# kekeliu-whu/Wildcat-SLAM

Hardware: AMD Instinct MI355X
Metric: surfel-extract Mpts/s (higher is better)
Workload: dtype f64; 1 GPU; C2: 1M-pt single scan (G2 patch lattice, 999936 pts -> 31248 surfels) per GPU, voxel-grid + 3-level octree + per-cell 3x3 PCA; input = the reference's 48-byte hilti_ros::Point records, consumed in place; points_per_gpu=999936, surfels_per_gpu=31248, parallelism=sweep-per-gpu x1

## Files before the change

### wildcat-slam_amd/csrc/ctx.h

```cpp
#pragma once
#include <hip/hip_runtime.h>

#include <cstdarg>
#include <cstdio>
#include <cstdlib>
#include <cstring>
#include <string>
#include <vector>

#include "../../include/wildcat_hip.h"
#include "extract_plan.h"

struct wc_window_state;

struct wc_buf {
  void *p = nullptr;
  size_t cap = 0;
  bool pooled = false;
  bool plain = false;
};

#ifdef WC_DEV_KNOBS
#define WC_DBG(P, bit) ((P).dbg & (bit))
#else
#define WC_DBG(P, bit) 0
#endif

struct wc_dev_opts {
  int exact_sums = 0;
  int debug_skip = 0;
  int fx_merge_min = 3;
  int fx_split = -1;
  int fx_acc_form = -1;
  int no_bucket_sort = 0;
  int ex_sync = 0;
  int match_pair_serial = 0;
  int lm_dense = 0;
  int lm_side_stream = 1;
  int lm_one_collective = 0;
  int map_mom_pts = 1;
  int map_lin_groups = 0;
  int map_score_groups = 0;
  int map_cast_groups = 0;
  int map_carve_groups = 0;
  int map_remove_groups = 0;
  int map_cc_groups = 0;
  int map_absorb_groups = 0;
  int lm_dense_radius = 7;
  int lm_radius0 = -1;
};
inline bool wc_log_env(const char *name) { return getenv(name) != nullptr; }

struct wc_ctx {
  int device = 0;
  wc_params P;
  wc_dev_opts dev;
  bool pool_ok = false;
  hipMemPool_t pool = nullptr;
  hipStream_t own_stream = nullptr;
  hipStream_t stream = nullptr;
  hipEvent_t ev0 = nullptr, ev1 = nullptr;
  std::string err;
  wc_buf b_ex_ctrl;
  wc_buf b_keys[2], b_vals[2], b_sorttmp, b_slots, b_slot_ids, b_slot_keys[2], b_slot_idx[2], b_cand, b_cand_meta,
      b_status, b_misc[8], b_route[4], b_fx[10];
  double match_stats[8] = {0, 0, 0, 0, 0, 0, 0, 0};
  wc_buf b_kd[10];
  std::vector<wc_ctx *> batch_subs;
  wc_buf b_batch;
  wc_buf b_match_half;
  hipEvent_t ev_knn[2] = {nullptr, nullptr};
  wc_comm comm{};
  bool have_comm = false;
  void *rccl = nullptr;
  uint32_t *h_status_dev = nullptr;
  uint32_t *h_status = nullptr;
  unsigned long long mail_ticket = 0;
  wc_buf b_stage;
  void *h_stage = nullptr;
  size_t h_stage_cap = 0;
  double *h_mail = nullptr;
  ExSweep ex;
  ExMemory ex_mem;
  wc_window_state *win = nullptr;
  wc_ctx *aux = nullptr;
  hipEvent_t ev_aux = nullptr;
  hipEvent_t ev_pair = nullptr;
  void *pair_worker = nullptr;
  void (*pair_worker_free)(void *) = nullptr;
  void *pair_sync = nullptr;
  bool ex_prof = false;
  int ex_prof_mode = 0;
  hipEvent_t ex_ev[8] = {nullptr, nullptr, nullptr, nullptr, nullptr, nullptr, nullptr, nullptr};
};

struct wc_dev_guard {
  int prev = -1;
  bool switched = false;
  explicit wc_dev_guard(const wc_ctx *ctx) {
    if (ctx && hipGetDevice(&prev) == hipSuccess && prev != ctx->device) switched = hipSetDevice(ctx->device) == hipSuccess;
  }
  ~wc_dev_guard() {
    if (switched) (void)hipSetDevice(prev);
  }
  wc_dev_guard(const wc_dev_guard &) = delete;
  wc_dev_guard &operator=(const wc_dev_guard &) = delete;
};

inline int wc_fail(wc_ctx *ctx, int code, const char *fmt, ...) {
  char buf[512];
  va_list ap;
  va_start(ap, fmt);
  vsnprintf(buf, sizeof(buf), fmt, ap);
  va_end(ap);
  if (ctx) ctx->err = buf;
  return code;
}

#define WC_HIP(ctx, call)                                                                                   \
  do {                                                                                                      \
    hipError_t e_ = (call);                                                                                 \
    if (e_ != hipSuccess)                                                                                   \
      return wc_fail(ctx, WC_ERR_HIP, "%s failed: %s (%s:%d)", #call, hipGetErrorString(e_), __FILE__, __LINE__); \
  } while (0)

inline void wc_buf_release(wc_ctx *ctx, wc_buf &b) {
  if (!b.p) return;
  if (b.pooled && ctx && ctx->stream && hipFreeAsync(b.p, ctx->stream) == hipSuccess) {
  } else {
    if (ctx && ctx->stream) (void)hipStreamSynchronize(ctx->stream);
    (void)hipFree(b.p);
  }
  b.p = nullptr, b.cap = 0, b.pooled = false;
}
inline int wc_ensure(wc_ctx *ctx, wc_buf &b, size_t bytes) {
  if (bytes <= b.cap) return WC_OK;
  wc_buf_release(ctx, b);
  size_t want = bytes < ((size_t)64 << 20) ? 2 * bytes : bytes + bytes / 2;
  if (bytes >= ((size_t)64 << 10) && want < ((size_t)16 << 20)) want = (size_t)16 << 20;
  if (want < 4096) want = 4096;
  static const bool alloc_dbg = wc_log_env("WC_ALLOC_DEBUG");
  if (alloc_dbg) fprintf(stderr, "[alloc] %zu bytes wanted -> %zu\n", bytes, want);
  if (ctx->pool_ok && !b.plain && hipMallocFromPoolAsync(&b.p, want, ctx->pool, ctx->stream) == hipSuccess) {
    b.pooled = true;
  } else {
    (void)hipGetLastError();
    b.p = nullptr;
    WC_HIP(ctx, hipMalloc(&b.p, want));
    b.pooled = false;
  }
  b.cap = want;
  return WC_OK;
}
int wc_rccl_allreduce_on(wc_ctx *ctx, double *d_buf, uint64_t count, hipStream_t st);
#define WC_TRY(expr)            \
  do {                          \
    int rc_ = (expr);           \
    if (rc_ != WC_OK) return rc_; \
  } while (0)
```

### wildcat-slam_amd/csrc/ctx.hip

```cpp
#include "ctx.h"

#include <cmath>
#include <cstring>
#include <mutex>

extern "C" const char *wc_version(void) { return "wildcat_hip 0.1 (gfx950)"; }

extern "C" int wc_device_count(void) {
  int n = 0;
  if (hipGetDeviceCount(&n) != hipSuccess) return 0;
  return n;
}

extern "C" void wc_params_default(wc_params *p) {
  std::memset(p, 0, sizeof(*p));
  p->voxel_size = 0.8f;
  p->max_layer = 2;
  p->min_points = 20;
  p->planer_threshold = 0.01f;
  p->min_plane_likeness = 0.1;
  p->cluster_gap = 0.05;
  p->cluster_min_points = 20;
  p->center_scale = 1.0;
  p->angular_scale = 5.0 * M_PI / 180.0;
  p->surfel_dist_max = 0.1;
  p->knn_k = 10;
  p->time_diff_min = 0.06;
  p->surfel_sigma0 = 0.05 / 6;
  p->cauchy_a = 0.4;
  const double gn = 0.00015198973532354657, an = 0.006308226052016165;
  const double gw = 0.00011673723527962174, aw = 2.664506559330434e-06;
  const double rate = 200, k = 0.01;
  p->w_gyr = 1 / (gn * std::sqrt(rate)) * k;
  p->w_acc = 1 / (an * std::sqrt(rate)) * k;
  p->w_bg = 1 / (gw / std::sqrt(rate)) * k;
  p->w_ba = 1 / (aw / std::sqrt(rate)) * k;
  p->imu_dt = 1 / rate;
  p->max_iterations = 100;
  p->reference_quirks = 1;
  p->exact_sums = 0;
}

static int check_params(wc_ctx *ctx, const wc_params *p) {
  if (p->max_layer < 0 || p->max_layer > 2) return wc_fail(ctx, WC_ERR_ARG, "max_layer must be 0..2");
  if (!(p->voxel_size > 0)) return wc_fail(ctx, WC_ERR_ARG, "voxel_size must be positive");
  if (p->cluster_min_points < 1 || p->min_points < 0) return wc_fail(ctx, WC_ERR_ARG, "bad point thresholds");
  if (p->knn_k < 1 || p->knn_k > 16) return wc_fail(ctx, WC_ERR_ARG, "knn_k must be 1..16");
  return WC_OK;
}

namespace {
struct DevOpt {
  const char *name, *env;
  int wc_dev_opts::*field;
  bool flag_only;
};
const DevOpt kDevOpts[] = {
    {"exact_sums", "WC_EXACT_SUMS", &wc_dev_opts::exact_sums, true},
    {"debug_skip", "WC_DEBUG_SKIP", &wc_dev_opts::debug_skip, false},
    {"fx_merge_min", "WC_FX_MERGE_MIN", &wc_dev_opts::fx_merge_min, false},
    {"fx_split", "WC_FX_SPLIT", &wc_dev_opts::fx_split, false},
    {"fx_acc_form", "WC_FX_ACC_FORM", &wc_dev_opts::fx_acc_form, false},
    {"no_bucket_sort", "WC_NO_BUCKET_SORT", &wc_dev_opts::no_bucket_sort, true},
    {"ex_sync", "WC_EX_SYNC", &wc_dev_opts::ex_sync, true},
    {"match_pair_serial", "WC_MATCH_PAIR_SERIAL", &wc_dev_opts::match_pair_serial, true},
    {"lm_dense", "WC_LM_DENSE", &wc_dev_opts::lm_dense, true},
    {"lm_one_collective", "WC_LM_ONE_COLLECTIVE", &wc_dev_opts::lm_one_collective, true},
    {"lm_side_stream", "WC_LM_SIDE_STREAM", &wc_dev_opts::lm_side_stream, false},
    {"map_mom_pts", "WC_MAP_MOM_PTS", &wc_dev_opts::map_mom_pts, false},
    {"map_lin_groups", "WC_MAP_LIN_GROUPS", &wc_dev_opts::map_lin_groups, false},
    {"map_score_groups", "WC_MAP_SCORE_GROUPS", &wc_dev_opts::map_score_groups, false},
    {"map_carve_groups", "WC_MAP_CARVE_GROUPS", &wc_dev_opts::map_carve_groups, false},
    {"map_cast_groups", "WC_MAP_CAST_GROUPS", &wc_dev_opts::map_cast_groups, false},
    {"map_absorb_groups", "WC_MAP_ABSORB_GROUPS", &wc_dev_opts::map_absorb_groups, false},
    {"map_remove_groups", "WC_MAP_REMOVE_GROUPS", &wc_dev_opts::map_remove_groups, false},
    {"map_cc_groups", "WC_MAP_CC_GROUPS", &wc_dev_opts::map_cc_groups, false},
    {"lm_dense_radius", "WC_LM_DENSE_RADIUS", &wc_dev_opts::lm_dense_radius, false},
    {"lm_radius0", "WC_LM_RADIUS0", &wc_dev_opts::lm_radius0, false},
};
}

namespace {
struct DevPool {
  hipMemPool_t pool = nullptr;
  int refs = 0;
};
std::mutex g_pool_mu;
DevPool g_pools[64];
}
hipMemPool_t wc_pool_acquire(int device) {
  if (device < 0 || device >= 64) return nullptr;
  std::lock_guard<std::mutex> lk(g_pool_mu);
  DevPool &d = g_pools[device];
  if (!d.pool) {
    int supported = 0;
    if (hipDeviceGetAttribute(&supported, hipDeviceAttributeMemoryPoolsSupported, device) != hipSuccess || !supported) {
      (void)hipGetLastError();
      return nullptr;
    }
    hipMemPoolProps props;
    std::memset(&props, 0, sizeof(props));
    props.allocType = hipMemAllocationTypePinned;
    props.handleTypes = hipMemHandleTypeNone;
    props.location.type = hipMemLocationTypeDevice;
    props.location.id = device;
    hipMemPool_t p = nullptr;
    if (hipMemPoolCreate(&p, &props) != hipSuccess || !p) {
      (void)hipGetLastError();
      return nullptr;
    }
    uint64_t keep = ~0ull;
    if (hipMemPoolSetAttribute(p, hipMemPoolAttrReleaseThreshold, &keep) != hipSuccess) (void)hipGetLastError();
    d.pool = p;
  }
  ++d.refs;
  return d.pool;
}
void wc_pool_release(int device, hipMemPool_t pool) {
  if (!pool || device < 0 || device >= 64) return;
  std::lock_guard<std::mutex> lk(g_pool_mu);
  DevPool &d = g_pools[device];
  if (d.pool == pool && --d.refs == 0) {
    (void)hipMemPoolDestroy(d.pool);
    d.pool = nullptr;
  }
}

extern "C" int wc_ctx_create(const wc_params *params, int device, wc_ctx **out) {
  if (!out) return WC_ERR_ARG;
  *out = nullptr;
  int n = 0;
  if (hipGetDeviceCount(&n) != hipSuccess || n <= 0 || device < 0 || device >= n) return WC_ERR_NOGPU;
  wc_ctx *ctx = new wc_ctx;
  ctx->device = device;
  if (params)
    ctx->P = *params;
  else
    wc_params_default(&ctx->P);
  int rc = check_params(ctx, &ctx->P);
  if (rc != WC_OK) {
    delete ctx;
    return rc;
  }
  int prev_dev = -1;
  (void)hipGetDevice(&prev_dev);
  struct Restore {
    int d;
    ~Restore() {
      if (d >= 0) (void)hipSetDevice(d);
    }
  } restore{prev_dev};
  if (hipSetDevice(device) != hipSuccess || hipStreamCreateWithFlags(&ctx->own_stream, hipStreamNonBlocking) != hipSuccess ||
      hipEventCreate(&ctx->ev0) != hipSuccess || hipEventCreate(&ctx->ev1) != hipSuccess ||
      hipHostMalloc((void **)&ctx->h_status, 128 * sizeof(uint32_t)) != hipSuccess ||
      hipHostMalloc((void **)&ctx->h_mail, (64 + 4096) * sizeof(double)) != hipSuccess) {
    delete ctx;
    return WC_ERR_HIP;
  }
  ctx->stream = ctx->own_stream;
  {
    void *dp = nullptr;
    if (hipHostGetDevicePointer(&dp, ctx->h_status, 0) == hipSuccess) ctx->h_status_dev = (uint32_t *)dp;
    for (int q = 0; q < 128; ++q) ctx->h_status[q] = 0;
  }
  for (wc_buf &b : ctx->b_route) b.plain = true;
  ctx->b_status.plain = true;
  ctx->pool = wc_pool_acquire(device);
  ctx->pool_ok = ctx->pool != nullptr;
#ifdef WC_DEV_KNOBS
  for (const DevOpt &o : kDevOpts)
    if (const char *v = getenv(o.env)) ctx->dev.*(o.field) = o.flag_only ? 1 : atoi(v);
#endif
  *out = ctx;
  return WC_OK;
}

extern "C" int wc_ctx_set_dev_option(wc_ctx *ctx, const char *name, int value) {
  if (!ctx || !name) return wc_fail(ctx, WC_ERR_ARG, "%s: null or out-of-range argument", __func__);
  for (const DevOpt &o : kDevOpts)
    if (strcmp(o.name, name) == 0) {
      ctx->dev.*(o.field) = value;
      ex_reset_backoff(ctx->ex_mem);
      if (ctx->aux) ctx->aux->dev = ctx->dev;
      for (wc_ctx *sub : ctx->batch_subs) sub->dev = ctx->dev, ex_reset_backoff(sub->ex_mem);
      return WC_OK;
    }
  return wc_fail(ctx, WC_ERR_ARG, "wc_ctx_set_dev_option: unknown option '%s'", name);
}

void wc_window_free(wc_ctx *ctx);
extern "C" int wc_comm_rccl_destroy(wc_ctx *ctx);

extern "C" void wc_ctx_destroy(wc_ctx *ctx) {
  wc_dev_guard dg_(ctx);
  if (!ctx) return;
  (void)hipSetDevice(ctx->device);
  (void)hipStreamSynchronize(ctx->stream);
  if (ctx->pair_worker && ctx->pair_worker_free) ctx->pair_worker_free(ctx->pair_worker);
  ctx->pair_worker = nullptr;
  if (ctx->aux) {
    wc_ctx_destroy(ctx->aux);
    ctx->aux = nullptr;
  }
  if (ctx->ev_aux) (void)hipEventDestroy(ctx->ev_aux);
  if (ctx->ev_pair) (void)hipEventDestroy(ctx->ev_pair);
  for (hipEvent_t e : ctx->ev_knn)
    if (e) (void)hipEventDestroy(e);
  (void)wc_comm_rccl_destroy(ctx);
  wc_window_free(ctx);
  wc_buf *all[] = {&ctx->b_keys[0],      &ctx->b_keys[1],     &ctx->b_vals[0],     &ctx->b_vals[1],      &ctx->b_sorttmp,
                   &ctx->b_slots,        &ctx->b_slot_ids,    &ctx->b_slot_keys[0], &ctx->b_slot_keys[1], &ctx->b_slot_idx[0],
                   &ctx->b_slot_idx[1],  &ctx->b_cand,        &ctx->b_cand_meta,   &ctx->b_status,
                   &ctx->b_ex_ctrl};
  for (wc_buf *b : all) wc_buf_release(ctx, *b);
// ... 187 lines not shown
```

### wildcat-slam_amd/csrc/extract.hip

```cpp
#include <hip/hip_runtime.h>
#include <type_traits>

#include <chrono>
#include <cstdlib>
#include <cstring>
#include <rocprim/rocprim.hpp>

#include "ctx.h"
#include "dmath.h"

namespace {

constexpr int kMom = 11;
constexpr int kProdStride = 66;
constexpr unsigned kRootsGrid = 256 * 16;
constexpr unsigned kEmitGrid = 256 * 8;
constexpr unsigned kRoots2Grid = 256 * 4;
constexpr int kTile = 2048;

struct ExParams {
  double vs;
  float vs_f;
  int max_layer;
  int min_points;
// ... 1056 lines not shown
    const uint32_t v = idx[a];
    const wc_surfel_id vid = slot_ids[v];
    uint64_t b = a;
    while (b > i && surfel_id_less(vid, slot_ids[idx[b - 1]])) {
      idx[b] = idx[b - 1];
      --b;
    }
    idx[b] = v;
  }
}

struct SlotEmitArgs {
  const uint32_t *counts;
  const uint64_t *bins;
  uint32_t bin_cap;
  const wc_surfel *slots;
  const wc_surfel_id *slot_ids;
  uint32_t *status;
  wc_surfel *out;
  wc_surfel_id *out_ids;
  uint64_t cap;
  uint32_t *next_ctrl;
  uint32_t next_words;
};
__device__ __forceinline__ void slot_emit_body(const SlotEmitArgs &E, const uint32_t bid, const uint32_t nblk) {
  const uint32_t *__restrict__ counts = E.counts;
  const uint64_t *__restrict__ bins = E.bins;
  const uint32_t bin_cap = E.bin_cap;
  const wc_surfel *__restrict__ slots = E.slots;
  const wc_surfel_id *__restrict__ slot_ids = E.slot_ids;
  uint32_t *status = E.status;
  wc_surfel *out = E.out;
  wc_surfel_id *out_ids = E.out_ids;
  const uint64_t cap = E.cap;
  uint32_t *next_ctrl = E.next_ctrl;
  const uint32_t next_words = E.next_words;
  __shared__ uint64_t s_item[4][kSlotBinMax];
  if (next_ctrl) {
    const uint32_t i = bid * 256u + threadIdx.x;
    if (i < next_words) next_ctrl[i] = (i == 8u || i == 9u) ? status[i] : 0u;
  }
  __shared__ uint32_t s_sorted[4][kSlotBinMax];
  __shared__ uint32_t s_red[4];
  const int t = threadIdx.x, w = t >> 6, lane = t & 63;
  const uint32_t b0 = bid * 4u;
  static_assert(kBuckets / 4 <= 4 * 256, "four uint4 loads per thread cover the counts");
  const uint4 *c4 = (const uint4 *)counts;
  uint4 v[4];
#pragma unroll
  for (int k = 0; k < 4; ++k) {
    const uint32_t i = (uint32_t)t + 256u * k;
    v[k] = i < bid ? c4[i] : make_uint4(0u, 0u, 0u, 0u);
  }
  const uint4 own = c4[bid];
  const uint64_t *bin = bins + (size_t)(b0 + w) * bin_cap;
  const uint64_t first = (uint32_t)lane < bin_cap ? bin[lane] : 0ull;
  uint32_t part = 0;
#pragma unroll
  for (int k = 0; k < 4; ++k) part += v[k].x + v[k].y + v[k].z + v[k].w;
  for (int off = 32; off >= 1; off >>= 1) part += __shfl_xor(part, off);
  if (lane == 0) s_red[w] = part;
  __syncthreads();
  uint32_t base = s_red[0] + s_red[1] + s_red[2] + s_red[3];
  const uint32_t c0 = own.x, c1 = own.y, c2 = own.z, c3 = own.w;
  if (bid == nblk - 1 && t == 0) {
    status[0] = base + c0 + c1 + c2 + c3;
    uint32_t *hm = host_mailbox(status);
    if (hm) {
      hm[0] = base + c0 + c1 + c2 + c3;
      uint32_t queued = status[4];
      const uint32_t *fxc = counts + kBuckets;
      for (int j = 0; j < 16; ++j) queued += fxc[(16 + j) * 32];
      hm[4] = queued;
      hm[5] = status[5];
    }
  }
  base += (w > 0 ? c0 : 0u) + (w > 1 ? c1 : 0u) + (w > 2 ? c2 : 0u);
  const uint32_t c = w == 0 ? c0 : (w == 1 ? c1 : (w == 2 ? c2 : c3));
  if (c == 0) return;
  if (c > bin_cap) {
    if (lane == 0) raise_flag(status, kFlagSlotBinOverflow);
    return;
  }
  auto before = [&](uint64_t other, uint64_t mine) -> bool {
    if ((other >> 32) == (mine >> 32) && other != mine) {
      const double to = slots[(uint32_t)other].t, tm = slots[(uint32_t)mine].t;
      return to < tm || (to == tm && surfel_id_less(slot_ids[(uint32_t)other], slot_ids[(uint32_t)mine]));
    }
    return other < mine;
  };
  if (c <= 64u) {
    const uint32_t lo = (uint32_t)first, hi = (uint32_t)(first >> 32);
    uint32_t rank = 0;
    for (uint32_t j = 0; j < c; ++j) {
      const uint64_t other = ((uint64_t)(uint32_t)__builtin_amdgcn_readlane((int)hi, (int)j) << 32) | (uint32_t)__builtin_amdgcn_readlane((int)lo, (int)j);
      if ((uint32_t)lane < c) rank += before(other, first) ? 1u : 0u;
    }
    if ((uint32_t)lane < c) s_sorted[w][rank] = lo;
  } else {
    s_item[w][lane] = first;
    for (uint32_t i = lane + 64; i < c; i += 64) s_item[w][i] = bin[i];
    __builtin_amdgcn_wave_barrier();
    for (uint32_t i = lane; i < c; i += 64) {
      const uint64_t mine = s_item[w][i];
      uint32_t rank = 0;
      for (uint32_t j = 0; j < c; ++j) rank += before(s_item[w][j], mine) ? 1u : 0u;
      s_sorted[w][rank] = (uint32_t)mine;
    }
  }
  __builtin_amdgcn_wave_barrier();
  const int sub = lane / 10, piece = lane - sub * 10;
  if (sub >= 6) return;
  auto load = [&](uint32_t r, bool on) -> double2 {
    double2 d = make_double2(0.0, 0.0);
    if (!on) return d;
    const uint32_t sl = s_sorted[w][r];
    if (piece < 9)
      d = ((const double2 *)(slots + sl))[piece];
    else if (out_ids) {
      const uint4 q = *(const uint4 *)(slot_ids + sl);
      d = *(const double2 *)&q;
    }
    return d;
  };
  auto store = [&](uint32_t r, bool on, const double2 &d) {
    if (!on) return;
    const uint64_t o = (uint64_t)base + r;
    if (piece < 9)
      ((double2 *)(out + o))[piece] = d;
    else if (out_ids)
      *(double2 *)(out_ids + o) = d;
  };
  if (c <= 12u) {
    const uint32_t r = sub;
    const bool on0 = r < c && (uint64_t)base + r < cap, on1 = r + 6 < c && (uint64_t)base + r + 6 < cap;
    const double2 d0 = load(r, on0), d1 = load(r + 6, on1);
    store(r, on0, d0);
    store(r + 6, on1, d1);
    return;
  }
  for (uint32_t r = sub; r < c; r += 24) {
    bool on[4];
    double2 d[4];
#pragma unroll
    for (int q = 0; q < 4; ++q) {
      on[q] = r + 6u * q < c && (uint64_t)base + r + 6u * q < cap;
      d[q] = load(r + 6u * q, on[q]);
    }
#pragma unroll
    for (int q = 0; q < 4; ++q) store(r + 6u * q, on[q], d[q]);
  }
}

__global__ void __launch_bounds__(256) k_slot_emit(const uint32_t *__restrict__ counts, const uint64_t *__restrict__ bins, uint32_t bin_cap,
                                                  const wc_surfel *__restrict__ slots, const wc_surfel_id *__restrict__ slot_ids,
                                                  uint32_t *status, wc_surfel *out, wc_surfel_id *out_ids, uint64_t cap, uint32_t *next_ctrl,
                                                  uint32_t next_words) {
  const SlotEmitArgs E{counts, bins, bin_cap, slots, slot_ids, status, out, out_ids, cap, next_ctrl, next_words};
  slot_emit_body(E, blockIdx.x, gridDim.x);
}
__global__ void __launch_bounds__(256) k_slot_emit_b(const SlotEmitArgs *__restrict__ Es, int K) {
  const uint32_t per = kBuckets / 4;
  const uint32_t k = blockIdx.x / per;
  if ((int)k >= K) return;
  slot_emit_body(Es[k], blockIdx.x - k * per, per);
}


__device__ __forceinline__ uint32_t run_length(const unsigned long long *s_bits, uint32_t i, uint32_t cnt) {
  uint32_t w = (i + 1) >> 6;
  unsigned long long m = (w < kTile / 64) ? (s_bits[w] & (~0ull << ((i + 1) & 63))) : 0ull;
  while (m == 0ull && ++w < kTile / 64) m = s_bits[w];
  const uint32_t nxt = m ? (w * 64 + (uint32_t)__ffsll((long long)m) - 1) : cnt;
  return min(nxt, cnt) - i;
}

struct InitArgs {
  uint32_t *p[8];
  uint32_t nw[8];
  uint32_t val[8];
};
__global__ void __launch_bounds__(256) k_init(InitArgs I) {
  const uint32_t i = blockIdx.x * 256u + threadIdx.x;
#pragma unroll
  for (int r = 0; r < 8; ++r)
    if (i < I.nw[r]) I.p[r][i] = I.val[r];
}

constexpr int kRunThreads = 512;
constexpr uint32_t kNoKey = 0xFFFFFFFFu;
__global__ void __launch_bounds__(kRunThreads) k_pt_runs(wc_points pts, double vs, uint64_t n, uint32_t *counts, uint64_t *bins,
                                                        uint32_t bin_cap, uint32_t *status) {
  __shared__ uint32_t s_key[kTile];
  __shared__ unsigned long long s_bits[kTile / 64];
  __shared__ uint32_t s_runs[kBuckets];
  __shared__ uint32_t s_pts[kBuckets];
  const int t = threadIdx.x;
  const uint64_t t0 = (uint64_t)blockIdx.x * kTile;
  const uint32_t cnt = (uint32_t)min((uint64_t)kTile, n - t0);
  double x0, y0, z0;
  ex_origin(pts, x0, y0, z0);
  const int k0x = vox(x0, vs), k0y = vox(y0, vs), k0z = vox(z0, vs);
  uint32_t key[kTile / kRunThreads];
#pragma unroll
  for (int j = 0; j < kTile / kRunThreads; ++j) {
    const uint32_t i = (uint32_t)j * kRunThreads + t;
    key[j] = 0;
    if (i < cnt) {
      double x, y, z;
      load_xyz(pts, t0 + i, x, y, z);
      key[j] = kNoKey;
      if (finite3(x, y, z)) {
        int rx = vox(x, vs) - k0x + 512, ry = vox(y, vs) - k0y + 512, rz = vox(z, vs) - k0z + 512;
        if ((unsigned)rx >= 1024u || (unsigned)ry >= 1024u || (unsigned)rz >= 1024u) {
          raise_flag(status, kFlagKeyRange);
          rx = min(max(rx, 0), 1023), ry = min(max(ry, 0), 1023), rz = min(max(rz, 0), 1023);
        }
        key[j] = (uint32_t)rx | ((uint32_t)ry << 10) | ((uint32_t)rz << 20);
      }
    }
  }
  for (int b = t; b < kBuckets; b += kRunThreads) {
    s_runs[b] = 0;
    s_pts[b] = 0;
  }
  if (t < kTile / 64) s_bits[t] = 0ull;
#pragma unroll
  for (int j = 0; j < kTile / kRunThreads; ++j) s_key[j * kRunThreads + t] = key[j];
  __syncthreads();
#pragma unroll
  for (int j = 0; j < kTile / kRunThreads; ++j) {
    const uint32_t i = (uint32_t)j * kRunThreads + t;
    const bool headp = i < cnt && (i == 0 || key[j] != s_key[i - 1]);
    const unsigned long long m = __ballot(headp);
    if ((t & 63) == 0) s_bits[i >> 6] = m;
  }
  __syncthreads();
  uint32_t rank[kTile / kRunThreads], len[kTile / kRunThreads];
#pragma unroll
  for (int j = 0; j < kTile / kRunThreads; ++j) {
    const uint32_t i = (uint32_t)j * kRunThreads + t;
    rank[j] = 0xFFFFFFFFu;
    if (i < cnt && key[j] != kNoKey && ((s_bits[i >> 6] >> (i & 63)) & 1ull)) {
      const uint32_t d = key_digit(key[j]);
      len[j] = run_length(s_bits, i, cnt);
      rank[j] = atomicAdd(&s_runs[d], 1u);
      atomicAdd(&s_pts[d], len[j]);
    }
  }
  __syncthreads();
  for (int b = t; b < kBuckets; b += kRunThreads) {
    const uint32_t c = s_runs[b];
    if (c) {
      s_runs[b] = atomicAdd(&counts[b], c);
      atomicAdd(&counts[kBuckets + b], s_pts[b]);
    }
  }
  __syncthreads();
#pragma unroll
  for (int j = 0; j < kTile / kRunThreads; ++j) {
    if (rank[j] == 0xFFFFFFFFu) continue;
    const uint32_t i = (uint32_t)j * kRunThreads + t;
    const uint32_t d = key_digit(key[j]);
    const uint32_t pos = s_runs[d] + rank[j];
    if (pos < bin_cap) bins[(size_t)d * bin_cap + pos] = run_comp(key_rest(key[j]), (uint32_t)(t0 + i), len[j]);
  }
}

__global__ void __launch_bounds__(256) k_pt_bucket(uint64_t *bins, uint32_t bin_cap, uint32_t lds_cap, const uint32_t *__restrict__ counts,
                                                  uint32_t *run_off, HeadRec *head_slots, uint32_t *root_cnt, uint32_t *root_first,
                                                  int min_points, uint32_t *status) {
  extern __shared__ __align__(16) unsigned char s_dyn[];
  __shared__ uint32_t s_red[4], s_live[4];
  const int t = threadIdx.x, w = t >> 6, lane = t & 63;
  uint64_t *s_a = (uint64_t *)s_dyn + (size_t)w * lds_cap;
  uint64_t *s_b = (uint64_t *)s_dyn + (size_t)(4 + w) * lds_cap;
  uint32_t *s_off = (uint32_t *)((uint64_t *)s_dyn + (size_t)8 * lds_cap) + (size_t)w * lds_cap;
  const uint32_t b0 = blockIdx.x * 4u, b = b0 + w;
  const uint32_t *pcounts = counts + kBuckets;
  uint32_t nb = counts[b];
  const uint32_t total = pcounts[b];
  uint64_t *bin = bins + (size_t)b * bin_cap;
  const uint64_t first = ((uint32_t)lane < min(nb, bin_cap)) ? bin[lane] : 0ull;
  uint32_t part = 0, runs_part = 0;
  for (uint32_t i = t; i < b0; i += 256) part += pcounts[i];
  if (blockIdx.x == gridDim.x - 1)
    for (uint32_t i = t; i < kBuckets; i += 256) runs_part += counts[i];
  uint32_t before = 0;
  for (int j = 0; j < w; ++j) before += pcounts[b0 + j];
  for (int off = 32; off >= 1; off >>= 1) part += __shfl_xor(part, off);
  if (lane == 0) s_red[w] = part;
  if (blockIdx.x == gridDim.x - 1) {
    for (int off = 32; off >= 1; off >>= 1) runs_part += __shfl_xor(runs_part, off);
    if (lane == 0) atomicAdd(&status[5], runs_part);
  }
  if (nb > bin_cap || nb > lds_cap) {
    if (lane == 0) raise_flag(status, nb > bin_cap ? kFlagBucketOverflow : kFlagLdsOverflow);
    nb = 0;
  }
  if (nb <= 64) {
    if ((uint32_t)lane < nb) s_a[lane] = first;
    __builtin_amdgcn_wave_barrier();
    if ((uint32_t)lane < nb) {
      uint32_t rank = 0;
      for (uint32_t j = 0; j < nb; ++j) rank += (s_a[j] < first) ? 1u : 0u;
      s_b[rank] = first;
    }
  } else {
    uint32_t N = 128;
    while (N < nb) N <<= 1;
    s_b[lane] = first;
    for (uint32_t i = lane + 64; i < N; i += 64) s_b[i] = (i < nb) ? bin[i] : ~0ull;
    __builtin_amdgcn_wave_barrier();
    for (uint32_t k = 2; k <= N; k <<= 1)
      for (uint32_t j = k >> 1; j > 0; j >>= 1) {
        for (uint32_t p = lane; p < N / 2; p += 64) {
          const uint32_t i = 2 * p - (p & (j - 1)), l = i + j;
          const uint64_t x = s_b[i], y = s_b[l];
// ... 56 lines not shown
    const uint32_t r = s_list[k] & 0xFFFFu, r2 = s_list[k] >> 16;
    const uint32_t seg = (r2 < nb ? s_off[r2] : total) - s_off[r];
    head_slots[first_slot + lbase + k] = HeadRec{pbase + s_off[r], b * bin_cap + r, r2 - r, seg};
  }
}

inline uint32_t pt_bin_cap(uint64_t n) {
  uint32_t cap = 64;
  while (cap < kPtBinMax && (uint64_t)cap * kBuckets < 32 * n) cap *= 2;
  return cap;
}

constexpr uint32_t kCtrlStatus = 0, kCtrlCounts = 64, kCtrlRoots = kCtrlCounts + 2 * kBuckets, kCtrlBins = kCtrlRoots + 2 * (kBuckets / 4),
                   kCtrlFx = kCtrlBins + kBuckets, kCtrlWords = kCtrlFx + 4 * 16 * 32;

int clear_ctrl(wc_ctx *ctx) {
  WC_TRY(wc_ensure(ctx, ctx->b_ex_ctrl, kCtrlWords * 4));
  uint32_t *ctrl = (uint32_t *)ctx->b_ex_ctrl.p;
  InitArgs I{};
  void *dp = nullptr;
  if (hipHostGetDevicePointer(&dp, ctx->h_status, 0) != hipSuccess) dp = nullptr;
  const unsigned long long a = (unsigned long long)dp;
  I.p[0] = ctrl, I.nw[0] = 8, I.val[0] = 0u;
  I.p[1] = ctrl + 10, I.nw[1] = kCtrlRoots - 10, I.val[1] = 0u;
  I.p[2] = ctrl + 8, I.nw[2] = 1, I.val[2] = (uint32_t)a;
  I.p[3] = ctrl + 9, I.nw[3] = 1, I.val[3] = (uint32_t)(a >> 32);
  I.p[4] = ctrl + kCtrlBins, I.nw[4] = kBuckets + 4 * 16 * 32, I.val[4] = 0u;
  k_init<<<(kCtrlRoots + 255) / 256, 256, 0, ctx->stream>>>(I);
  WC_HIP(ctx, hipGetLastError());
  return WC_OK;
}

int point_sort_runs(wc_ctx *ctx, const wc_points &pts, double vs, HeadRec *head_slots, int min_points, uint32_t *status) {
  hipStream_t st = ctx->stream;
  const uint64_t n = pts.n;
  const uint32_t cap = pt_bin_cap(n);
  const uint32_t lds_cap = std::min(cap, std::max(64u, ctx->ex_mem.lds_cap));
  WC_TRY(wc_ensure(ctx, ctx->b_misc[1], (uint64_t)kBuckets * cap * 8));
  WC_TRY(wc_ensure(ctx, ctx->b_misc[3], (uint64_t)kBuckets * cap * 4));
  uint32_t *counts = (uint32_t *)ctx->b_ex_ctrl.p + kCtrlCounts;
  const unsigned tiles = (unsigned)((n + kTile - 1) / kTile);
  const size_t lds = (size_t)4 * lds_cap * 20;
  if (!ctx->ex_mem.bucket_attr_set) {
    WC_HIP(ctx, hipFuncSetAttribute((const void *)k_pt_bucket, hipFuncAttributeMaxDynamicSharedMemorySize, (int)(4 * kPtBinMax * 20)));
    ctx->ex_mem.bucket_attr_set = true;
  }
  k_pt_runs<<<tiles, kRunThreads, 0, st>>>(pts, vs, n, counts, (uint64_t *)ctx->b_misc[1].p, cap, status);
  k_pt_bucket<<<kBuckets / 4, 256, lds, st>>>((uint64_t *)ctx->b_misc[1].p, cap, lds_cap, counts, (uint32_t *)ctx->b_misc[3].p, head_slots,
                                             counts + 2 * kBuckets, counts + 2 * kBuckets + kBuckets / 4, min_points, status);
  WC_HIP(ctx, hipGetLastError());
  return WC_OK;
}

template <typename K>
int sort_pairs(wc_ctx *ctx, K *kin, K *kout, uint32_t *vin, uint32_t *vout, size_t n, unsigned end_bit) {
  using cfg = rocprim::radix_sort_config<rocprim::default_config, rocprim::default_config, rocprim::default_config, 0>;
  size_t tmp = 0;
  WC_HIP(ctx, rocprim::radix_sort_pairs<cfg>(nullptr, tmp, kin, kout, vin, vout, n, 0u, end_bit, ctx->stream));
  WC_TRY(wc_ensure(ctx, ctx->b_sorttmp, tmp));
  tmp = ctx->b_sorttmp.cap;
  WC_HIP(ctx, rocprim::radix_sort_pairs<cfg>(ctx->b_sorttmp.p, tmp, kin, kout, vin, vout, n, 0u, end_bit, ctx->stream));
  return WC_OK;
}

#include "extract_fast.inc"
#include "extract_split.inc"

int fx_ensure_zero(wc_ctx *ctx, wc_buf &b, size_t bytes) {
  if (bytes <= b.cap) return WC_OK;
  WC_TRY(wc_ensure(ctx, b, bytes));
  WC_HIP(ctx, hipMemsetAsync(b.p, 0, b.cap, ctx->stream));
  return WC_OK;
}

bool fx_applicable(const wc_ctx *ctx, uint64_t n, double t_lo, double t_hi) {
  const wc_params &P = ctx->P;
  if (P.exact_sums || ctx->dev.exact_sums) return false;
  if (n < 64 || !(P.voxel_size > 0.0f) || P.voxel_size >= 0.99f) return false;
  if (!(P.cluster_gap > 1e-6) || !(t_hi > t_lo)) return false;
  if ((t_hi - t_lo) / (P.cluster_gap * 0.999) >= 1048000.0) return false;
  return true;
}

ExParams ex_params(const wc_ctx *ctx) {
  const wc_params &P = ctx->P;
  ExParams E{};
  E.vs = (double)P.voxel_size, E.vs_f = P.voxel_size, E.max_layer = P.max_layer, E.min_points = P.min_points;
  E.thr = (double)P.planer_threshold, E.min_like = P.min_plane_likeness;
  for (int i = 0; i < 3; ++i) E.view[i] = P.view_point[i];
  E.gap = P.cluster_gap, E.cluster_min = P.cluster_min_points;
  E.t_lo_bits = ordered_bits_host(ctx->ex.t_lo);
  E.t_span_bits = ordered_bits_host(ctx->ex.t_hi) - E.t_lo_bits;
  E.dbg = ctx->dev.debug_skip;
  E.merge_min = ctx->dev.fx_merge_min;
  return E;
}

void ex_mark(wc_ctx *ctx, int i) {
  if (ctx->ex_prof && (ctx->ex_prof_mode != 2 || i == 1 || i == 5)) (void)hipEventRecord(ctx->ex_ev[i], ctx->stream);
}

template <typename Args>
void ex_keep_for_tail(wc_ctx *ctx, const Args &A, int (*tail)(wc_ctx *, bool)) {
  static_assert(sizeof(Args) <= sizeof(ctx->ex.roots_args), "extract_plan.h: roots_args too small");
  std::memcpy(ctx->ex.roots_args, &A, sizeof(A));
  ctx->ex.tail = tail;
}

int fx_tail(wc_ctx *ctx, bool layer2);

int run_pipeline_fast(wc_ctx *ctx) {
  const wc_params &P = ctx->P;
  ExMemory &M = ctx->ex_mem;
  const wc_points &pts = ctx->ex.pts;
  const double t_lo = ctx->ex.t_lo, t_hi = ctx->ex.t_hi;
  const uint64_t n = pts.n;
  hipStream_t st = ctx->stream;
  FxArgs A;
  std::memset(&A, 0, sizeof(A));
  A.P = ex_params(ctx);
  A.pts = pts;
  A.t_lo = t_lo;
  int e = 0;
  (void)std::frexp(t_hi - t_lo, &e);
  A.tick = std::ldexp(1.0, 40 - e), A.inv_tick = std::ldexp(1.0, e - 40);
  A.inv_w = 1.0 / (P.cluster_gap * 0.999);
  A.inv_span = 1.0 / (t_hi - t_lo);
  A.inv_vs = 1.0 / (double)P.voxel_size;
  A.qs = 4294967296.0, A.inv_q = 1.0 / 4294967296.0, A.inv_qq = std::ldexp(1.0, -44);
  {
    const double vs = (double)P.voxel_size;
    A.band0 = 1e-14 + 3.0 * (std::ldexp(1.0, -45) + 2.0 * std::ldexp(1.0, -33) * vs + 16.0 * std::ldexp(1.0, -53) * (0.5 * vs) * (0.5 * vs));
  }
  uint32_t mr = 1024;
  while ((uint64_t)mr * 8 < n) mr *= 2;
  A.mr_per = mr / kFxSub, A.mq_per = std::max(64u, mr / 2 / kFxSub);
  uint32_t tr = 2048;
  while ((uint64_t)tr * 4 < n) tr *= 2;
  A.tr_mask = tr - 1;
  A.static_map = n <= 2000000ull ? 1u : 0u;
  {
    const uintptr_t px = (uintptr_t)pts.xyz, pt = (uintptr_t)pts.time;
    if (pts.xyz_stride == 48u && pts.time_stride == 48u && pt == px + 24u && px % 16u == 0u)
      A.fmt = 1u;
    else if (pts.xyz_stride == 12u && pts.time_stride == 8u && px % 16u == 0u && pt % 16u == 0u)
      A.fmt = 2u;
  }
  const unsigned tiles = ex_fx_tiles(n);
  A.rec_tiles = tiles;
  const uint64_t spill_full = ((uint64_t)tiles + 7) / 8 * kFxTile;
  A.spill_per = (uint32_t)((n <= 8000000ull || M.fx_spill_full) ? spill_full : std::max<uint64_t>(1024, n / 32));
  A.rec_cap = tiles * (uint32_t)kFxRecTile + 8u * A.spill_per;
  const uint64_t total_slots = ex_total_slots(n, P.max_layer, P.cluster_min_points, (uint64_t)kFxSub * 256);
  const uint32_t bin_cap = ex_slot_bin_cap(total_slots);
  WC_TRY(fx_ensure_zero(ctx, ctx->b_fx[0], (size_t)tr * 4));
  WC_TRY(wc_ensure(ctx, ctx->b_fx[1], (size_t)mr * 4));
  WC_TRY(fx_ensure_zero(ctx, ctx->b_fx[2], (size_t)tr * kFxBlockW * 8));
  WC_TRY(fx_ensure_zero(ctx, ctx->b_fx[3], (size_t)A.mq_per * kFxSub * kFxBlockW * 8));
  WC_TRY(wc_ensure(ctx, ctx->b_fx[4], (size_t)2 * A.rec_cap * kFxRecW * 8));
  const unsigned ngrid = ex_fx_node_grid(n);
  WC_TRY(wc_ensure(ctx, ctx->b_fx[6], (size_t)ngrid * kFxJobCap * kFxJobW * 8));
  ctx->ex.fx_split = ctx->ex.batch_defer || (ctx->dev.fx_split >= 0 ? ctx->dev.fx_split != 0 : !A.static_map);
  if (ctx->ex.fx_split) {
    A.static_map = 0u;
    A.jobpool_per = (uint32_t)std::max<uint64_t>(4096, n / (uint64_t)std::max(1, P.cluster_min_points) / 2);
    WC_TRY(wc_ensure(ctx, ctx->b_fx[7], ((size_t)mr / 8 + 2) * kFxNodeW * 64 * 8));
    WC_TRY(wc_ensure(ctx, ctx->b_fx[8], ((size_t)mr / 8 + 2) * kFxDescW * 4));
    WC_TRY(wc_ensure(ctx, ctx->b_fx[9], (size_t)8 * A.jobpool_per * kFxJobW * 8));
    A.nodes = (unsigned long long *)ctx->b_fx[7].p, A.wdesc = (uint32_t *)ctx->b_fx[8].p, A.jobpool = (unsigned long long *)ctx->b_fx[9].p;
  }
  WC_TRY(wc_ensure(ctx, ctx->b_slots, total_slots * sizeof(wc_surfel)));
  WC_TRY(wc_ensure(ctx, ctx->b_slot_ids, total_slots * sizeof(wc_surfel_id)));
  WC_TRY(wc_ensure(ctx, ctx->b_slot_keys[1], (uint64_t)kBuckets * bin_cap * 8));
  if (M.fx_dirty) {
    for (int i : {0, 2, 3}) WC_HIP(ctx, hipMemsetAsync(ctx->b_fx[i].p, 0, ctx->b_fx[i].cap, st));
    M.fx_dirty = false;
  }
  WC_TRY(wc_ensure(ctx, ctx->b_fx[5], (size_t)2 * kCtrlWords * 4));
  if (!M.fx_ctrl_ready) {
    WC_HIP(ctx, hipMemsetAsync(ctx->b_fx[5].p, 0, (size_t)2 * kCtrlWords * 4, st));
    const unsigned long long a = (unsigned long long)ctx->h_status_dev;
    const uint32_t addr[2] = {(uint32_t)a, (uint32_t)(a >> 32)};
    for (int b = 0; b < 2; ++b)
      WC_HIP(ctx, hipMemcpyAsync((uint32_t *)ctx->b_fx[5].p + (size_t)b * kCtrlWords + 8, addr, 8, hipMemcpyHostToDevice, st));
    WC_HIP(ctx, hipStreamSynchronize(st));
    M.fx_ctrl_ready = true;
    M.fx_parity = 0;
  }
  uint32_t *ctrl = (uint32_t *)ctx->b_fx[5].p + (size_t)M.fx_parity * kCtrlWords;
  for (int q = 0; q < 64; ++q) ctx->h_status[q] = 0;
  A.rkey = (uint32_t *)ctx->b_fx[0].p, A.rlist = (uint32_t *)ctx->b_fx[1].p;
  A.blk = (unsigned long long *)ctx->b_fx[2].p, A.blk2 = (unsigned long long *)ctx->b_fx[3].p;
  A.rec = (unsigned long long *)ctx->b_fx[4].p;
  A.jobs = (unsigned long long *)ctx->b_fx[6].p;
  A.status = ctrl + kCtrlStatus;
  A.cnt = ctrl + kCtrlFx;
  A.slots = (wc_surfel *)ctx->b_slots.p, A.slot_ids = (wc_surfel_id *)ctx->b_slot_ids.p;
  A.slots_per = (uint32_t)std::min<uint64_t>(total_slots / kFxSub, 0x7FFFFFFFu);
  A.slot_counts = ctrl + kCtrlBins;
  A.slot_bins = (uint64_t *)ctx->b_slot_keys[1].p;
  A.slot_bin_cap = bin_cap;
  ex_mark(ctx, 0);
  ex_mark(ctx, 1);
  static const bool dbg = wc_log_env("WC_FX_DEBUG");
  auto dbg_sync = [&](const char *what) {
    if (!dbg) return;
    fprintf(stderr, "[fx] %s ...", what);
    const hipError_t e = hipStreamSynchronize(st);
    uint32_t w[64], c[4 * 16 * 32];
    (void)hipMemcpy(w, A.status, sizeof(w), hipMemcpyDeviceToHost);
    (void)hipMemcpy(c, A.cnt, sizeof(c), hipMemcpyDeviceToHost);
    uint32_t r = 0, q = 0, sl = 0, sp = 0;
    for (int j = 0; j < 16; ++j) r += c[j * 32], q += c[(16 + j) * 32], sl += c[(32 + j) * 32], sp += c[(48 + j) * 32];
    fprintf(stderr, " %s flags=%u roots=%u nodes2=%u slots=%u spill=%u\n", hipGetErrorString(e), w[1], r, q, sl, sp);
  };
  if (dbg) fprintf(stderr, "[fx] n=%llu tiles=%u mr_per=%u mq_per=%u tr=%u slots_per=%u bin_cap=%u\n", (unsigned long long)n, tiles, A.mr_per, A.mq_per, tr, A.slots_per, bin_cap);
  ex_keep_for_tail(ctx, A, &fx_tail);
  if (ctx->ex.batch_defer) {
    ctx->ex.layer2_done = P.max_layer >= 2 && M.last_splits > 0;
    ctx->ex.deferred = true;
    return WC_OK;
  }
  fx_launch_acc<1>(ctx, tiles, st, A);
  dbg_sync("k_fx_acc<1>");
  ex_mark(ctx, 2);
  if (M.fx_long_lists) k_fx_merge<1><<<std::min<unsigned>(ngrid * 2u, 8192u), 128, 0, st>>>(A);
  if (ctx->ex.fx_split) {
    k_fx_walk<1><<<ngrid, 64, 0, st>>>(A);
    dbg_sync("k_fx_walk<1>");
    k_fx_test<1><<<ngrid, 64, 0, st>>>(A);
  } else {
    k_fx_nodes<1><<<ngrid, 64, 0, st>>>(A);
  }
  dbg_sync("k_fx_nodes<1>");
  ex_mark(ctx, 3);
  return fx_tail(ctx, P.max_layer >= 2 && M.last_splits > 0);
}

constexpr int kMailTicket = 120;
__global__ void k_ex_ticket(uint32_t *host_word, uint32_t ticket) {
  __hip_atomic_store(host_word, ticket, __ATOMIC_RELEASE, __HIP_MEMORY_SCOPE_SYSTEM);
}

int fx_tail(wc_ctx *ctx, bool layer2) {
  hipStream_t st = ctx->stream;
  FxArgs A;
  std::memcpy(&A, ctx->ex.roots_args, sizeof(A));
  ExMemory &M = ctx->ex_mem;
  if (layer2) {
    fx_launch_acc<2>(ctx, ex_fx_tiles(A.pts.n), st, A);
    if (M.fx_long_lists2) k_fx_merge<2><<<std::min(8192u, std::max(64u, M.last_splits)), 128, 0, st>>>(A);
    const unsigned g2 = ex_fx_layer2_grid(ex_fx_node_grid(A.pts.n), M.last_splits);
    if (ctx->ex.fx_split) {
      k_fx_walk<2><<<g2, 64, 0, st>>>(A);
      k_fx_test<2><<<g2, 64, 0, st>>>(A);
    } else {
      k_fx_nodes<2><<<g2, 64, 0, st>>>(A);
    }
  }
  ctx->ex.layer2_done = layer2;
  ex_mark(ctx, 4);
  uint32_t *next_ctrl = (uint32_t *)ctx->b_fx[5].p + (size_t)(M.fx_parity ^ 1) * kCtrlWords;
  static_assert(kCtrlWords <= (kBuckets / 4) * 256, "k_slot_emit's grid covers the control block");
  k_slot_emit<<<kBuckets / 4, 256, 0, st>>>(A.slot_counts, A.slot_bins, A.slot_bin_cap, (const wc_surfel *)ctx->b_slots.p,
                                           (const wc_surfel_id *)ctx->b_slot_ids.p, A.status, ctx->ex.d_out, ctx->ex.d_ids, ctx->ex.cap, next_ctrl,
                                           kCtrlWords);
  ex_mark(ctx, 5);
  ctx->ex.ticket = 0;
  if (ctx->h_status_dev && !ctx->ex_prof && !ctx->dev.ex_sync) {
    if (++M.ticket_seq == 0u) ++M.ticket_seq;
    ctx->ex.ticket = M.ticket_seq;
    k_ex_ticket<<<1, 1, 0, st>>>(ctx->h_status_dev + kMailTicket, ctx->ex.ticket);
  }
  static const bool fx_dbg = wc_log_env("WC_FX_DEBUG");
  if (fx_dbg) fprintf(stderr, "[fx] k_slot_emit (layer2=%d) ... %s\n", (int)layer2, hipGetErrorString(hipStreamSynchronize(st)));
  WC_HIP(ctx, hipGetLastError());
  return WC_OK;
}

template <typename K, bool RUNS>
int pipeline_tail(wc_ctx *ctx, bool layer2) {
  hipStream_t st = ctx->stream;
  RootsArgs A;
  memcpy(&A, ctx->ex.roots_args, sizeof(A));
  uint32_t *status = A.status;
  const uint64_t cap = ctx->ex.cap, total_slots = A.total_slots;
  const bool fast_slots = A.slot_counts != nullptr;
  if (layer2) {
    const unsigned grid2 = std::min(kRoots2Grid, std::max(64u, ctx->ex_mem.last_splits));
    if constexpr (RUNS) {
      if (ctx->ex_mem.unordered)
        k_roots_banks<K, 2, true><<<grid2, 64, 0, st>>>(A, (const K *)ctx->b_keys[1].p);
      else
        k_roots<K, 2><<<grid2, 64, 0, st>>>(A);
    } else {
      k_roots_banks<K, 2, false><<<grid2, 64, 0, st>>>(A, (const K *)ctx->b_keys[1].p);
    }
  }
  ctx->ex.layer2_done = layer2;
  ex_mark(ctx, 4);
  if (fast_slots) {
    k_slot_emit<<<kBuckets / 4, 256, 0, st>>>(A.slot_counts, A.slot_bins, A.slot_bin_cap, (const wc_surfel *)ctx->b_slots.p,
                                             (const wc_surfel_id *)ctx->b_slot_ids.p, status, ctx->ex.d_out, ctx->ex.d_ids, cap, nullptr, 0u);
  } else {
    k_iota<<<(unsigned)((total_slots + 255) / 256), 256, 0, st>>>((uint32_t *)ctx->b_slot_idx[0].p, total_slots);
    WC_TRY(sort_pairs<uint64_t>(ctx, (uint64_t *)ctx->b_slot_keys[0].p, (uint64_t *)ctx->b_slot_keys[1].p,
                                (uint32_t *)ctx->b_slot_idx[0].p, (uint32_t *)ctx->b_slot_idx[1].p, total_slots,
                                ctx->ex.slot_end_bit));
    k_fix_ties<<<(unsigned)((total_slots + 255) / 256), 256, 0, st>>>((const uint64_t *)ctx->b_slot_keys[1].p, (uint32_t *)ctx->b_slot_idx[1].p,
                                                                     total_slots, (const wc_surfel_id *)ctx->b_slot_ids.p);
    const uint64_t gth = std::min<uint64_t>(total_slots, cap) * 10;
    if (gth)
      k_gather<<<(unsigned)((gth + 255) / 256), 256, 0, st>>>((const uint32_t *)ctx->b_slot_idx[1].p, (const wc_surfel *)ctx->b_slots.p,
                                                             (const wc_surfel_id *)ctx->b_slot_ids.p, status, ctx->ex.d_out, ctx->ex.d_ids, cap);
  }
  ex_mark(ctx, 5);
  if (!fast_slots) WC_HIP(ctx, hipMemcpyAsync(ctx->h_status, status, 32, hipMemcpyDeviceToHost, st));
  WC_HIP(ctx, hipGetLastError());
  return WC_OK;
}

template <typename K>
int run_pipeline(wc_ctx *ctx, const ExPath &path) {
  const wc_params &P = ctx->P;
  const wc_points &pts = ctx->ex.pts;
  const uint64_t n = pts.n;
  hipStream_t st = ctx->stream;
  const ExParams E = ex_params(ctx);
  unsigned tbits = 1;
  while (tbits < 64 && (E.t_span_bits >> tbits)) ++tbits;
  const unsigned slot_end_bit = tbits >= 63 ? 64 : tbits + 1;

  const uint64_t total_slots = ex_total_slots(n, P.max_layer, P.cluster_min_points, 0);
  WC_TRY(wc_ensure(ctx, ctx->b_keys[0], n * sizeof(K)));
  WC_TRY(wc_ensure(ctx, ctx->b_keys[1], n * sizeof(K)));
  WC_TRY(wc_ensure(ctx, ctx->b_vals[0], n * 4));
  WC_TRY(wc_ensure(ctx, ctx->b_vals[1], n * 4));
  WC_TRY(wc_ensure(ctx, ctx->b_cand, total_slots * kMom * 8));
  WC_TRY(wc_ensure(ctx, ctx->b_cand_meta, total_slots * 4));
  WC_TRY(wc_ensure(ctx, ctx->b_slots, total_slots * sizeof(wc_surfel)));
  WC_TRY(wc_ensure(ctx, ctx->b_slot_ids, total_slots * sizeof(wc_surfel_id)));
  WC_TRY(wc_ensure(ctx, ctx->b_slot_keys[0], total_slots * 8));
  WC_TRY(wc_ensure(ctx, ctx->b_slot_keys[1], total_slots * 8));
  WC_TRY(wc_ensure(ctx, ctx->b_slot_idx[0], total_slots * 4));
  WC_TRY(wc_ensure(ctx, ctx->b_slot_idx[1], total_slots * 4));
  WC_TRY(wc_ensure(ctx, ctx->b_misc[0], (n / (uint64_t)(P.min_points + 1) + 2) * sizeof(HeadRec)));
  const bool precleared = ctx->ex_mem.precleared && ctx->b_ex_ctrl.p;
  ctx->ex_mem.precleared = false;
  if (!precleared) WC_TRY(clear_ctrl(ctx));
  for (int q = 0; q < 16; ++q) ctx->h_status[q] = 0;
  uint32_t *status = (uint32_t *)ctx->b_ex_ctrl.p + kCtrlStatus;

  ex_mark(ctx, 0);
  const bool fast_slots = path.bin_order && tbits <= 31 && total_slots < (1ull << 31);
  const uint32_t bin_cap = ex_slot_bin_cap(total_slots);
  const unsigned g256 = (unsigned)((n + 255) / 256);
  const bool fast_pts = path.run_sort && sizeof(K) == 4;
  if (fast_pts || fast_slots) {
    WC_TRY(wc_ensure(ctx, ctx->b_slot_keys[1], (uint64_t)kBuckets * bin_cap * 8));
  }
  const uint32_t nslots = (uint32_t)(n / (uint64_t)(P.min_points + 1) + 1);
  if (!fast_slots || !fast_pts) {
    InitArgs I{};
    int r = 0;
    auto fill = [&](void *p, uint64_t words, uint32_t v) { I.p[r] = (uint32_t *)p, I.nw[r] = (uint32_t)words, I.val[r] = v, ++r; };
    if (!fast_slots) fill(ctx->b_slot_keys[0].p, total_slots * 2, 0xFFFFFFFFu);
    if (!fast_pts) fill(ctx->b_misc[0].p, (uint64_t)nslots * 4, 0xFFFFFFFFu);
    uint32_t mx = 0;
    for (int q = 0; q < r; ++q) mx = std::max(mx, I.nw[q]);
    k_init<<<(mx + 255) / 256, 256, 0, st>>>(I);
  }
  ex_mark(ctx, 1);
  if (fast_pts) {
    WC_TRY(point_sort_runs(ctx, pts, E.vs, (HeadRec *)ctx->b_misc[0].p, P.min_points, status));
  } else {
    k_keygen<K><<<g256, 256, 0, st>>>(pts, E.vs, (K *)ctx->b_keys[0].p, (uint32_t *)ctx->b_vals[0].p, status);
    WC_TRY(sort_pairs<K>(ctx, (K *)ctx->b_keys[0].p, (K *)ctx->b_keys[1].p, (uint32_t *)ctx->b_vals[0].p,
                         (uint32_t *)ctx->b_vals[1].p, n, 3 * KeyTraits<K>::bits + 1));
  }
  RootsArgs A;
  A.pts = pts;
  A.P = E;
  A.n = n;
  A.vals = (const uint32_t *)ctx->b_vals[1].p;
  A.cand = (double *)ctx->b_cand.p;
  A.cand_meta = (uint32_t *)ctx->b_cand_meta.p;
  A.slots = (wc_surfel *)ctx->b_slots.p;
  A.slot_ids = (wc_surfel_id *)ctx->b_slot_ids.p;
  A.slot_keys = (uint64_t *)ctx->b_slot_keys[0].p;
  A.total_slots = total_slots;
  A.status = status;
  A.slot_counts = fast_slots ? (uint32_t *)ctx->b_ex_ctrl.p + kCtrlBins : nullptr;
  A.slot_shift = tbits > 12 ? tbits - 12 : 0u;
  A.slot_bins = (uint64_t *)ctx->b_slot_keys[1].p;
  A.runs = (const uint64_t *)ctx->b_misc[1].p;
  A.run_off = (const uint32_t *)ctx->b_misc[3].p;
  A.run_cap = pt_bin_cap(n);
  A.root_cnt = (const uint32_t *)ctx->b_ex_ctrl.p + kCtrlRoots;
  A.root_first = A.root_cnt + kBuckets / 4;
  A.slot_bin_cap = bin_cap;
  A.heads = (const HeadRec *)ctx->b_misc[0].p;
  A.nslots = nslots;
  if (!fast_pts) k_heads<K><<<g256, 256, 0, st>>>((const K *)ctx->b_keys[1].p, n, P.min_points, (HeadRec *)ctx->b_misc[0].p);
  ex_mark(ctx, 2);
  WC_TRY(wc_ensure(ctx, ctx->b_misc[5], (size_t)A.nslots * sizeof(SplitJob)));
  A.split_jobs = (SplitJob *)ctx->b_misc[5].p;
  WC_TRY(wc_ensure(ctx, ctx->b_misc[7], (size_t)A.nslots * (9 * kMom * 8 + 4)));
  A.node_tot = (double *)ctx->b_misc[7].p;
  A.root_ncand = (uint32_t *)(A.node_tot + (size_t)A.nslots * 9 * kMom);
  const K *skeys = (const K *)ctx->b_keys[1].p;
  if (fast_pts) {
    if constexpr (sizeof(K) == 4) {
      if (ctx->ex_mem.unordered)
        k_roots_banks<K, 1, true><<<kRootsGrid, 64, 0, st>>>(A, skeys);
      else
        k_roots<K, 1><<<kRootsGrid, 64, 0, st>>>(A);
      ex_mark(ctx, 3);
      k_roots_emit<K, true><<<kEmitGrid, 64, 0, st>>>(A, skeys);
    }
  } else {
    k_roots_banks<K, 1, false><<<kRootsGrid, 64, 0, st>>>(A, skeys);
    ex_mark(ctx, 3);
    k_roots_emit<K, false><<<kEmitGrid, 64, 0, st>>>(A, skeys);
  }
  ex_keep_for_tail(ctx, A, fast_pts ? &pipeline_tail<K, (sizeof(K) == 4)> : &pipeline_tail<K, false>);
  ctx->ex.slot_end_bit = slot_end_bit;
  return ctx->ex.tail(ctx, ctx->ex_mem.last_splits > 0);
}

int enqueue_path(wc_ctx *ctx, const ExPath &path) {
  ctx->ex.path = path;
  ++ctx->ex.runs;
  const int rc = path.fx ? run_pipeline_fast(ctx) : path.wide ? run_pipeline<uint64_t>(ctx, path) : run_pipeline<uint32_t>(ctx, path);
  if (path.fx && rc != WC_OK) ctx->ex_mem.fx_dirty = true;
  return rc;
}

int ex_wait(wc_ctx *ctx) {
  bool arrived = false;
  if (const uint32_t ticket = ctx->ex.ticket) {
    ctx->ex.ticket = 0;
    const uint32_t *w = (const uint32_t *)ctx->h_status + kMailTicket;
    const auto t0 = std::chrono::steady_clock::now();
    for (uint32_t spin = 0; !arrived; ++spin) {
      arrived = __atomic_load_n(w, __ATOMIC_ACQUIRE) == ticket;
      if ((spin & 1023u) == 1023u && std::chrono::steady_clock::now() - t0 > std::chrono::milliseconds(20)) break;
    }
  }
  if (!arrived) WC_HIP(ctx, hipStreamSynchronize(ctx->stream));
  for (int i = 0; i < 7; ++i)
    if (ctx->h_status[8 + i]) ctx->h_status[1] |= 1u << i;
  return WC_OK;
}

}

extern "C" int wc_voxel_keys(wc_ctx *ctx, const wc_points *pts, int32_t *d_keys_xyz) {
  wc_dev_guard dg_(ctx);
  if (!ctx || !pts || !d_keys_xyz) return wc_fail(ctx, WC_ERR_ARG, "%s: null or out-of-range argument", __func__);
  if (pts->n == 0) return WC_OK;
  k_voxel_keys<<<(unsigned)((pts->n + 255) / 256), 256, 0, ctx->stream>>>(*pts, (double)ctx->P.voxel_size, d_keys_xyz);
  WC_HIP(ctx, hipGetLastError());
  WC_HIP(ctx, hipStreamSynchronize(ctx->stream));
  return WC_OK;
}

extern "C" int wc_extract_surfels_enqueue(wc_ctx *ctx, const wc_points *pts, double t_lo, double t_hi, wc_surfel *d_out,
                                          wc_surfel_id *d_ids, uint64_t cap) {
  wc_dev_guard dg_(ctx);
  if (!ctx || !pts) return wc_fail(ctx, WC_ERR_ARG, "%s: null or out-of-range argument", __func__);
  if (pts->n >= (1ull << 32)) return wc_fail(ctx, WC_ERR_ARG, "at most 2^32-1 points per call");
  ctx->ex.active = true;
  ctx->ex.ticket = 0;
  ctx->ex.pts = *pts;
  ctx->ex.d_out = d_out, ctx->ex.d_ids = d_ids, ctx->ex.cap = cap;
  ctx->ex.path = ExPath{}, ctx->ex.runs = 0;
  for (int q = 0; q < 16; ++q) ctx->h_status[q] = 0;
  if (pts->n == 0) return WC_OK;
  if (t_lo > t_hi) {
    WC_HIP(ctx, hipMemcpyAsync(&ctx->h_mail[0], pts->time, 8, hipMemcpyDeviceToHost, ctx->stream));
    WC_HIP(ctx, hipMemcpyAsync(&ctx->h_mail[1], (const char *)pts->time + (pts->n - 1) * pts->time_stride, 8,
                               hipMemcpyDeviceToHost, ctx->stream));
    WC_HIP(ctx, hipStreamSynchronize(ctx->stream));
    t_lo = ctx->h_mail[0];
    t_hi = ctx->h_mail[1];
  }
  {
    const double mag = std::max(std::fabs(t_lo), std::fabs(t_hi));
    const double m = 4096.0 * (std::nextafter(mag, INFINITY) - mag);
    t_lo -= m;
    t_hi += m;
  }
  ctx->ex.t_lo = t_lo, ctx->ex.t_hi = t_hi;
  return enqueue_path(ctx, ex_first_path(ctx->ex_mem, fx_applicable(ctx, pts->n, t_lo, t_hi), ctx->dev.no_bucket_sort != 0));
}

extern "C" int wc_extract_surfels_finish(wc_ctx *ctx, uint64_t *h_n_out) {
  wc_dev_guard dg_(ctx);
  if (!ctx || !ctx->ex.active) return wc_fail(ctx, WC_ERR_ARG, "%s: null or out-of-range argument", __func__);
  ExSweep &S = ctx->ex;
  ExMemory &M = ctx->ex_mem;
  S.active = false;
  if (h_n_out) *h_n_out = 0;
  if (S.pts.n == 0) return WC_OK;
  WC_TRY(ex_wait(ctx));
  if (S.path.fx) {
    if (!S.layer2_done && ctx->P.max_layer >= 2 && ctx->h_status[4] > 0 && !(ctx->h_status[1] & (kFlagFxFallback | kFlagKeyRange))) {
      M.last_splits = ctx->h_status[4];
      WC_TRY(fx_tail(ctx, true));
      WC_TRY(ex_wait(ctx));
    }
    M.last_splits = ctx->h_status[4];
  }
  ExPath path = S.path;
  while (ex_next_path(path, ctx->h_status[1], ctx->h_status + 32, M)) {
    WC_TRY(enqueue_path(ctx, path));
    WC_TRY(ex_wait(ctx));
  }
  if (path.fx) {
    M.fx_long_lists = ctx->h_status[15] != 0u;
    M.fx_long_lists2 = ctx->h_status[16] != 0u;
    M.fx_parity ^= 1;
  } else {
    if (!S.layer2_done && ctx->h_status[4] > 0 && S.tail) {
      M.last_splits = ctx->h_status[4];
      WC_TRY(S.tail(ctx, true));
      WC_TRY(ex_wait(ctx));
    }
    M.last_splits = ctx->h_status[4];
    ex_learn_unordered(M, path, ctx->h_status[5], S.pts.n);
    if (clear_ctrl(ctx) == WC_OK) M.precleared = true;
  }
  const uint32_t flags = ctx->h_status[1], n_out = ctx->h_status[0];
  if (h_n_out) *h_n_out = n_out;
  if (flags & kFlagKeyRange) return wc_fail(ctx, WC_ERR_ARG, "point cloud extent exceeds 2^20 root voxels");
  if (flags & kFlagSlotOverflow) return wc_fail(ctx, WC_ERR_HIP, "internal: candidate slot overflow");
  if (flags & kFlagTimeRange) return wc_fail(ctx, WC_ERR_ARG, "surfel timestamp outside the [t_lo, t_hi] hint");
  if (n_out > S.cap) return wc_fail(ctx, WC_ERR_CAPACITY, "output capacity %llu < %u surfels", (unsigned long long)S.cap, n_out);
  return WC_OK;
}

extern "C" int wc_extract_surfels(wc_ctx *ctx, const wc_points *pts, double t_lo, double t_hi, wc_surfel *d_out,
                                  wc_surfel_id *d_ids, uint64_t cap, uint64_t *h_n_out) {
  wc_dev_guard dg_(ctx);
  WC_TRY(wc_extract_surfels_enqueue(ctx, pts, t_lo, t_hi, d_out, d_ids, cap));
  return wc_extract_surfels_finish(ctx, h_n_out);
}

extern "C" int wc_extract_surfels_batch_enqueue(wc_ctx *ctx, const wc_sweep_job *jobs, int K) {
  wc_dev_guard dg_(ctx);
  if (!ctx || !jobs || K < 1 || K > 64) return wc_fail(ctx, WC_ERR_ARG, "%s: null or out-of-range argument", __func__);
  while ((int)ctx->batch_subs.size() < K) {
    wc_ctx *sub = nullptr;
    const int rc = wc_ctx_create(&ctx->P, ctx->device, &sub);
    if (rc != WC_OK) return wc_fail(ctx, rc, "wc_extract_surfels_batch: no sub-context");
    ctx->batch_subs.push_back(sub);
  }
  hipStream_t st = ctx->stream;
  const size_t o_emit = (sizeof(FxArgs) * K + 15) & ~(size_t)15, o_tab = (o_emit + sizeof(SlotEmitArgs) * K + 15) & ~(size_t)15;
  const size_t bytes = o_tab + (size_t)(3 * (K + 1) + K) * 4;
  std::vector<unsigned char> host(bytes, 0);
  FxArgs *args = (FxArgs *)host.data();
  SlotEmitArgs *emit = (SlotEmitArgs *)(host.data() + o_emit);
  uint32_t *s_acc = (uint32_t *)(host.data() + o_tab), *s_nodes = s_acc + (K + 1), *s_g2 = s_nodes + (K + 1), *flags = s_g2 + (K + 1);
  int Kd = 0;
  bool any_l2 = false, any_merge = false;
  for (int k = 0; k < K; ++k) {
    wc_ctx *sub = ctx->batch_subs[k];
    if (sub->stream != st) WC_TRY(wc_ctx_set_stream(sub, st));
    if (std::memcmp(&sub->P, &ctx->P, sizeof(wc_params)) != 0) WC_TRY(wc_ctx_set_params(sub, &ctx->P));
    if (std::memcmp(&sub->dev, &ctx->dev, sizeof(wc_dev_opts)) != 0) {
      sub->dev = ctx->dev;
      ex_reset_backoff(sub->ex_mem);
    }
    sub->ex.batch_defer = true;
    sub->ex.deferred = false;
    const int rc = wc_extract_surfels_enqueue(sub, &jobs[k].pts, jobs[k].t_lo, jobs[k].t_hi, jobs[k].d_out, jobs[k].d_ids, jobs[k].cap);
    sub->ex.batch_defer = false;
    if (rc != WC_OK) {
      for (int j = 0; j <= k; ++j) {
        wc_ctx *pj = ctx->batch_subs[j];
        if (pj->ex.deferred || j == k) pj->ex_mem.fx_dirty = true, pj->ex.active = false, pj->ex.deferred = false;
      }
      return wc_fail(ctx, rc, "wc_extract_surfels_batch (sweep %d): %s", k, wc_last_error(sub));
    }
    if (!sub->ex.deferred) continue;
    FxArgs &A = args[Kd];
    std::memcpy(&A, sub->ex.roots_args, sizeof(A));
    const unsigned ngrid = ex_fx_batch_node_grid(A.pts.n);
    s_acc[Kd + 1] = s_acc[Kd] + ex_fx_tiles(A.pts.n);
    s_nodes[Kd + 1] = s_nodes[Kd] + ngrid;
    s_g2[Kd + 1] = s_g2[Kd] + ex_fx_layer2_grid(ngrid, sub->ex_mem.last_splits);
    const uint32_t f = (sub->ex.layer2_done ? 1u : 0u) | ((sub->ex_mem.fx_long_lists || sub->ex_mem.fx_long_lists2) ? 2u : 0u);
    flags[Kd] = f;
    any_l2 = any_l2 || (f & 1u);
    any_merge = any_merge || (f & 2u);
    uint32_t *next_ctrl = (uint32_t *)sub->b_fx[5].p + (size_t)(sub->ex_mem.fx_parity ^ 1) * kCtrlWords;
    emit[Kd++] = SlotEmitArgs{A.slot_counts, A.slot_bins, A.slot_bin_cap, (const wc_surfel *)sub->b_slots.p, (const wc_surfel_id *)sub->b_slot_ids.p,
                              A.status, sub->ex.d_out, sub->ex.d_ids, sub->ex.cap, next_ctrl, (uint32_t)kCtrlWords};
  }
  if (Kd == 0) return WC_OK;
  WC_TRY(wc_ensure(ctx, ctx->b_batch, bytes));
  WC_HIP(ctx, hipMemcpyAsync(ctx->b_batch.p, host.data(), bytes, hipMemcpyHostToDevice, st));
  WC_HIP(ctx, hipStreamSynchronize(st));
  const unsigned char *d = (const unsigned char *)ctx->b_batch.p;
  const uint32_t *dt = (const uint32_t *)(d + o_tab);
  FxBatch B;
  B.args = (const FxArgs *)d, B.K = Kd, B.flags = dt + 3 * (K + 1);
  B.start = dt;
  fx_launch_acc_b<1>(ctx, s_acc[Kd], st, B);
  B.start = dt + (K + 1);
  if (any_merge) k_fx_merge_b<1><<<s_nodes[Kd], 128, 0, st>>>(B);
  k_fx_walk_b<1><<<s_nodes[Kd], 64, 0, st>>>(B);
  k_fx_test_b<1><<<s_nodes[Kd], 64, 0, st>>>(B);
  if (any_l2) {
    B.start = dt;
    fx_launch_acc_b<2>(ctx, s_acc[Kd], st, B);
    B.start = dt + 2 * (K + 1);
    if (any_merge) k_fx_merge_b<2><<<s_g2[Kd], 128, 0, st>>>(B);
    k_fx_walk_b<2><<<s_g2[Kd], 64, 0, st>>>(B);
    k_fx_test_b<2><<<s_g2[Kd], 64, 0, st>>>(B);
  }
  k_slot_emit_b<<<(unsigned)Kd * (kBuckets / 4), 256, 0, st>>>((const SlotEmitArgs *)(d + o_emit), Kd);
  WC_HIP(ctx, hipGetLastError());
  return WC_OK;
}

extern "C" int wc_extract_surfels_batch_finish(wc_ctx *ctx, uint64_t *h_n_out, int K) {
  wc_dev_guard dg_(ctx);
  if (!ctx || !h_n_out || K < 1 || K > (int)ctx->batch_subs.size()) return wc_fail(ctx, WC_ERR_ARG, "%s: null or out-of-range argument", __func__);
  int first_rc = WC_OK;
  for (int k = 0; k < K; ++k) {
    wc_ctx *sub = ctx->batch_subs[k];
    h_n_out[k] = 0;
    if (!sub->ex.active) continue;
    const int rc = wc_extract_surfels_finish(sub, &h_n_out[k]);
    if (rc != WC_OK && first_rc == WC_OK) first_rc = wc_fail(ctx, rc, "wc_extract_surfels_batch (sweep %d): %s", k, wc_last_error(sub));
  }
  return first_rc;
}

extern "C" int wc_extract_profile(wc_ctx *ctx, int enable) {
  wc_dev_guard dg_(ctx);
  if (!ctx) return wc_fail(ctx, WC_ERR_ARG, "%s: null or out-of-range argument", __func__);
  if (enable && !ctx->ex_ev[0])
    for (int i = 0; i < 8; ++i) WC_HIP(ctx, hipEventCreate(&ctx->ex_ev[i]));
  ctx->ex_prof = enable != 0;
  ctx->ex_prof_mode = enable;
  return WC_OK;
}

extern "C" int wc_extract_stage_ms(wc_ctx *ctx, float *h_ms5) {
  wc_dev_guard dg_(ctx);
  if (!ctx || !h_ms5 || !ctx->ex_ev[0]) return wc_fail(ctx, WC_ERR_ARG, "%s: null or out-of-range argument", __func__);
  WC_HIP(ctx, hipEventSynchronize(ctx->ex_ev[5]));
  if (ctx->ex_prof_mode == 2) {
    for (int i = 0; i < 5; ++i) h_ms5[i] = 0.f;
    WC_HIP(ctx, hipEventElapsedTime(&h_ms5[1], ctx->ex_ev[1], ctx->ex_ev[5]));
    return WC_OK;
  }
  for (int i = 0; i < 5; ++i) WC_HIP(ctx, hipEventElapsedTime(&h_ms5[i], ctx->ex_ev[i], ctx->ex_ev[i + 1]));
  return WC_OK;
}

extern "C" int wc_debug_status(wc_ctx *ctx, uint32_t *h_out64) {
  wc_dev_guard dg_(ctx);
  if (!ctx || !h_out64) return wc_fail(ctx, WC_ERR_ARG, "%s: null or out-of-range argument", __func__);
  for (int i = 0; i < 64; ++i) h_out64[i] = i < 16 ? ctx->h_status[i] : 0u;
  h_out64[56] = ctx->ex.runs;
  h_out64[57] = ex_path_bits(ctx->ex.path);
  h_out64[58] = ctx->ex_mem.lds_cap;
  h_out64[59] = ctx->ex_mem.fx_long_lists ? 1u : 0u;
  h_out64[60] = ctx->ex_mem.fx_fallbacks;
  h_out64[61] = ctx->ex.path.fx ? 1u : 0u;
  h_out64[62] = ctx->ex_mem.fx_last_flags;
  h_out64[63] = ctx->ex_mem.fx_last_why;
  return WC_OK;
}

namespace {
struct FxEigOut {
  double ev[3];
  double vec[3];
  double accepted;
  double spare;
};
__global__ void k_selftest_fx_eig3(const double *a9, FxEigOut *o) {
  wc::M3 a, v;
  for (int i = 0; i < 3; ++i)
    for (int j = 0; j < 3; ++j) a.m[i][j] = a9[3 * i + j];
  bool acc = false;
  fx_eig3(a, o->ev, v, &acc);
  for (int i = 0; i < 3; ++i) o->vec[i] = v.m[i][0];
  o->accepted = acc ? 1.0 : 0.0;
  o->spare = 0.0;
}
}

extern "C" int wc_selftest_fx_eig3(wc_ctx *ctx, const double a9[9], double out8[8]) {
  if (!ctx || !a9 || !out8) return wc_fail(ctx, WC_ERR_ARG, "%s: null argument", __func__);
  wc_dev_guard dg_(ctx);
  WC_TRY(wc_ensure(ctx, ctx->b_status, 1024));
  double *d_in = (double *)ctx->b_status.p;
  FxEigOut *d_out = (FxEigOut *)((char *)ctx->b_status.p + 128);
  FxEigOut o;
  WC_HIP(ctx, hipMemcpyAsync(d_in, a9, 9 * 8, hipMemcpyHostToDevice, ctx->stream));
  k_selftest_fx_eig3<<<1, 1, 0, ctx->stream>>>(d_in, d_out);
  WC_HIP(ctx, hipGetLastError());
  WC_HIP(ctx, hipMemcpyAsync(&o, d_out, sizeof(o), hipMemcpyDeviceToHost, ctx->stream));
  WC_HIP(ctx, hipStreamSynchronize(ctx->stream));
  std::memcpy(out8, &o, sizeof(o));
  return WC_OK;
}

int wc_touch_extract() {
  hipFuncAttributes a;
  return hipFuncGetAttributes(&a, (const void *)k_voxel_keys) == hipSuccess ? WC_OK : WC_ERR_HIP;
}
```

### wildcat-slam_amd/csrc/extract_fast.inc

```

constexpr int kFxLds = 256;
constexpr int kFxLdsProbe = 12;
constexpr int kFxDirect = 16;
constexpr int kFxRecTile = kFxLds + (kFxThreads / 64) * 4 * kFxDirect;
constexpr int kFxSlots = 16;
constexpr int kFxRecW = 16;
constexpr int kFxHdrW = 16;
constexpr int kFxBlockW = kFxHdrW + 8 * kFxSlots / 2;
constexpr uint32_t kFxStRoots = 0, kFxStNodes2 = 1, kFxStSlots = 2, kFxStSpillBank = 3;
constexpr int kFxCntStride = 32;
constexpr int kFxCntWords = 4 * kFxSub * kFxCntStride;
constexpr unsigned long long kFxTMax = 0xFFFFFFFFFFFFull;
constexpr double kFxMagic = 6755399441055744.0, kFxMagic2 = 7083549724304467820544.0;
constexpr unsigned long long kFxMagicBits = 0x4338000000000000ull;
constexpr uint32_t kFxMagicHi = 0x43380000u, kFxMagic2Hi = 0x44780000u;

struct FxArgs {
  wc_points pts;
  ExParams P;
  double t_lo;
  double tick, inv_tick;
  double inv_w;
  double inv_span;
  double inv_vs;
  double qs, inv_q, inv_qq;
  double band0;
  uint32_t *rkey;
  uint32_t *rlist;
  uint32_t tr_mask;
  uint32_t static_map;
  unsigned long long *blk;
  unsigned long long *blk2;
  unsigned long long *rec;
  uint32_t rec_tiles;
  uint32_t spill_per;
  uint32_t rec_cap;
  uint32_t mr_per, mq_per;
  uint32_t fmt;
  uint32_t *status;
  uint32_t *cnt;
  unsigned long long *jobs;
  unsigned long long *nodes;
  uint32_t *wdesc;
  unsigned long long *jobpool;
  uint32_t jobpool_per;
  wc_surfel *slots;
  wc_surfel_id *slot_ids;
  uint32_t slots_per;
  uint32_t *slot_counts;
  uint64_t *slot_bins;
  uint32_t slot_bin_cap;
};

__device__ __forceinline__ void fx_fallback(uint32_t *status, int why) {
  raise_flag(status, kFlagFxFallback);
  uint32_t *hm = host_mailbox(status);
  if (hm) hm[32 + why] = 1u;
}
__device__ __forceinline__ uint32_t *fx_cnt(const FxArgs &A, uint32_t bank, uint32_t j) { return A.cnt + (bank * kFxSub + j) * kFxCntStride; }

__device__ __forceinline__ uint32_t fx_hash32(uint32_t k) {
  k ^= k >> 16;
  k *= 0x7FEB352Du;
  k ^= k >> 15;
  k *= 0x846CA68Bu;
  k ^= k >> 16;
  return k;
}

__device__ __forceinline__ int fx_vox(double p, double vs, double inv_vs) {
  const double q = p * inv_vs;
  const double r = rint(q);
  if (fabs(q - r) > 1e-9 * (fabs(r) + 1.0)) return (int)floor(q);
  return (int)floor(p / vs);
}

constexpr int kFxStMaxProbe = 20;
__device__ __forceinline__ uint32_t fx_root_slot(const FxArgs &A, uint32_t key1, uint32_t sub, bool insert, uint32_t maxprobe = 0u) {
  uint32_t slot = fx_hash32(key1) & A.tr_mask;
  for (int probe = 0; probe < 64; ++probe) {
    uint32_t k;
    if (insert) {
      k = atomicCAS(&A.rkey[slot], 0u, key1);
      if (k == 0u) {
        if (probe) atomicMax(&A.status[kFxStMaxProbe], (uint32_t)probe);
        const uint32_t local = atomicAdd(fx_cnt(A, kFxStRoots, sub), 1u);
        if (local < A.mr_per)
          A.rlist[sub * A.mr_per + local] = slot;
        else
          fx_fallback(A.status, 0);
        return slot;
      }
    } else {
      k = __hip_atomic_load(&A.rkey[slot], __ATOMIC_RELAXED, __HIP_MEMORY_SCOPE_AGENT);
      if (k == 0u && (uint32_t)probe >= maxprobe) return 0xFFFFFFFFu;
    }
    if (k == key1) return slot;
    slot = (slot + 1u) & A.tr_mask;
  }
  fx_fallback(A.status, 1);
  return 0xFFFFFFFFu;
}

struct FxPart {
  uint32_t n;
  long long st, s[3], ss[6];
  unsigned long long tmin_inv, tmax_p1;
};
__device__ __forceinline__ void fx_zero(FxPart &a) {
  a.n = 0, a.st = 0, a.tmin_inv = 0, a.tmax_p1 = 0;
  for (int i = 0; i < 3; ++i) a.s[i] = 0;
  for (int i = 0; i < 6; ++i) a.ss[i] = 0;
}
__device__ __forceinline__ void fx_acc(FxPart &a, const FxPart &b) {
  a.n += b.n, a.st += b.st;
  for (int i = 0; i < 3; ++i) a.s[i] += b.s[i];
  for (int i = 0; i < 6; ++i) a.ss[i] += b.ss[i];
  a.tmin_inv = max(a.tmin_inv, b.tmin_inv);
  a.tmax_p1 = max(a.tmax_p1, b.tmax_p1);
}

__device__ __forceinline__ void fx_add_cell(unsigned long long *cell, const FxPart &a) {
  atomicAdd((uint32_t *)cell, a.n);
  atomicAdd(&cell[1], (unsigned long long)a.st);
  for (int i = 0; i < 3; ++i) atomicAdd(&cell[2 + i], (unsigned long long)a.s[i]);
  for (int i = 0; i < 6; ++i) atomicAdd(&cell[5 + i], (unsigned long long)a.ss[i]);
  atomicMax(&cell[11], a.tmin_inv);
  atomicMax(&cell[12], a.tmax_p1);
}

struct FxClaim {
  int lead;
  uint32_t gmb, s0, found;
};
template <int LEVEL>
__device__ __forceinline__ void fx_code_fields(unsigned long long code, uint32_t &pkey, uint32_t &oct, uint32_t &bin) {
  if (LEVEL == 1) {
    pkey = (uint32_t)(code & 0x3FFFFFFFull) + 1u;
    oct = (uint32_t)(code >> 30) & 7u;
    bin = (uint32_t)(code >> 33) & 0xFFFFFu;
  } else {
    pkey = (uint32_t)(code & 0xFFFFFFFull) + 1u;
    oct = (uint32_t)(code >> 28) & 7u;
    bin = (uint32_t)(code >> 31) & 0xFFFFFu;
  }
}
template <int LEVEL>
__device__ __forceinline__ FxClaim fx_link_claim(const FxArgs &A, bool active, unsigned long long code) {
  const int lane = threadIdx.x & 63;
  uint32_t oct, bin, pkey;
  fx_code_fields<LEVEL>(code, pkey, oct, bin);
  int lead = lane;
  uint32_t gmb = bin;
  {
    unsigned long long todo = __ballot(active);
    while (todo) {
      const int first = __ffsll((long long)todo) - 1;
      const uint32_t k0 = (uint32_t)__shfl((int)pkey, first);
      const bool mine = active && pkey == k0;
      uint32_t mb = mine ? bin : 0xFFFFFFFFu;
      for (int m = 1; m < 64; m <<= 1) mb = min(mb, (uint32_t)__shfl_xor((int)mb, m));
      if (mine) lead = first, gmb = mb;
      todo &= ~__ballot(mine);
    }
  }
  FxClaim c;
  c.lead = lead, c.gmb = gmb, c.s0 = 0u, c.found = 0u;
  if (LEVEL == 1) {
    c.s0 = fx_hash32(pkey) & A.tr_mask;
    if (active && lane == lead && !(WC_DBG(A.P, 64))) c.found = atomicCAS(&A.rkey[c.s0], 0u, pkey);
  }
  return c;
}
template <int LEVEL>
__device__ __forceinline__ bool fx_link_head(const FxArgs &A, bool active, unsigned long long code, uint32_t sub, uint32_t ridx, const FxClaim &c,
                                             uint32_t &old) {
  const int lane = threadIdx.x & 63;
  unsigned long long *blk = nullptr;
  uint32_t oct, bin, pkey;
  fx_code_fields<LEVEL>(code, pkey, oct, bin);
  const int lead = c.lead;
  const uint32_t gmb = c.gmb;
  const bool leader = active && lane == lead;
  uint32_t slot = 0xFFFFFFFFu;
  bool created = false;
  if (leader) {
    if (LEVEL == 1) {
      if (WC_DBG(A.P, 64)) {
        slot = c.s0;
      } else if (c.found == 0u || c.found == pkey) {
        slot = c.s0;
        created = c.found == 0u;
      } else {
        uint32_t s = (c.s0 + 1u) & A.tr_mask;
        for (int probe = 1; probe < 64; ++probe) {
          const uint32_t k = atomicCAS(&A.rkey[s], 0u, pkey);
          if (k == 0u || k == pkey) {
            slot = s;
            created = k == 0u;
            if (created && probe) atomicMax(&A.status[kFxStMaxProbe], (uint32_t)probe);
            break;
          }
          s = (s + 1u) & A.tr_mask;
        }
// ... 576 lines not shown
  if (f == 0) return (void)k_fx_acc_form_b<LEVEL, 0><<<grid, kFxThreads, 0, st>>>(B);
  if constexpr (LEVEL == 1) {
    if (f == 1) return (void)k_fx_acc_form_b<1, 1><<<grid, kFxThreads, 0, st>>>(B);
    if (f == 2) return (void)k_fx_acc_form_b<1, 2><<<grid, kFxThreads, 0, st>>>(B);
  }
  k_fx_acc_b<LEVEL><<<grid, kFxThreads, 0, st>>>(B);
}

template <int LEVEL>
__device__ __forceinline__ void fx_merge_body(const FxArgs &A, const uint32_t bid, const uint32_t nblk) {
  const uint32_t bank = LEVEL == 1 ? kFxStRoots : kFxStNodes2;
  const uint32_t per = LEVEL == 1 ? A.mr_per : A.mq_per;
  uint32_t total = 0, cnts[kFxSub];
#pragma unroll
  for (int j = 0; j < kFxSub; ++j) {
    cnts[j] = min(*fx_cnt(A, bank, j), per);
    total += cnts[j];
  }
  for (uint32_t gi = bid; gi < total; gi += nblk) {
    uint32_t pidx = 0, rem = gi;
    bool found = false;
#pragma unroll
    for (int j = 0; j < kFxSub; ++j) {
      if (!found) {
        if (rem < cnts[j]) {
          pidx = (uint32_t)j * per + rem;
          found = true;
        } else {
          rem -= cnts[j];
        }
      }
    }
    if (LEVEL == 1) pidx = A.rlist[pidx];
    const unsigned long long *blk = (LEVEL == 1 ? A.blk : A.blk2) + (size_t)pidx * kFxBlockW;
    const uint32_t head = ((const uint32_t *)(blk + kFxHdrW))[threadIdx.x];
    if (head == 0u) continue;
    unsigned long long *first = A.rec + ((size_t)(LEVEL - 1) * A.rec_cap + (head - 1u)) * kFxRecW;
    ulonglong2 *f2 = (ulonglong2 *)first;
    const ulonglong2 w0 = f2[0], w6 = f2[6];
    uint32_t idx = (uint32_t)w6.y;
    if (idx == 0u) continue;
    const ulonglong2 w1 = f2[1], w2 = f2[2], w3 = f2[3], w4 = f2[4], w5 = f2[5];
    const uint32_t bin = (uint32_t)(w0.x >> 32);
    FxPart b;
    b.n = (uint32_t)w0.x, b.st = (long long)w0.y;
    b.s[0] = (long long)w1.x, b.s[1] = (long long)w1.y, b.s[2] = (long long)w2.x;
    b.ss[0] = (long long)w2.y, b.ss[1] = (long long)w3.x, b.ss[2] = (long long)w3.y;
    b.ss[3] = (long long)w4.x, b.ss[4] = (long long)w4.y, b.ss[5] = (long long)w5.x;
    b.tmin_inv = w5.y, b.tmax_p1 = w6.x;
    bool same = true;
    int guard = 0;
    for (; idx != 0u && guard < 100000; ++guard) {
      const ulonglong2 *r2 = (const ulonglong2 *)(A.rec + ((size_t)(LEVEL - 1) * A.rec_cap + (idx - 1u)) * kFxRecW);
      const ulonglong2 v0 = r2[0], v1 = r2[1], v2 = r2[2], v3 = r2[3], v4 = r2[4], v5 = r2[5], v6 = r2[6];
      same = same && (uint32_t)(v0.x >> 32) == bin;
      b.n += (uint32_t)v0.x, b.st += (long long)v0.y;
      b.s[0] += (long long)v1.x, b.s[1] += (long long)v1.y, b.s[2] += (long long)v2.x;
      b.ss[0] += (long long)v2.y, b.ss[1] += (long long)v3.x, b.ss[2] += (long long)v3.y;
      b.ss[3] += (long long)v4.x, b.ss[4] += (long long)v4.y, b.ss[5] += (long long)v5.x;
      b.tmin_inv = max(b.tmin_inv, v5.y), b.tmax_p1 = max(b.tmax_p1, v6.x);
      idx = (uint32_t)v6.y;
    }
    if (guard >= A.P.merge_min) {
      uint32_t *hm = host_mailbox(A.status);
      if (hm) hm[LEVEL == 1 ? 15 : 16] = 1u;
    }
    if (!same || idx != 0u) continue;
    f2[0] = make_ulonglong2((unsigned long long)b.n | ((unsigned long long)bin << 32), (unsigned long long)b.st);
    f2[1] = make_ulonglong2((unsigned long long)b.s[0], (unsigned long long)b.s[1]);
    f2[2] = make_ulonglong2((unsigned long long)b.s[2], (unsigned long long)b.ss[0]);
    f2[3] = make_ulonglong2((unsigned long long)b.ss[1], (unsigned long long)b.ss[2]);
    f2[4] = make_ulonglong2((unsigned long long)b.ss[3], (unsigned long long)b.ss[4]);
    f2[5] = make_ulonglong2((unsigned long long)b.ss[5], b.tmin_inv);
    f2[6] = make_ulonglong2(b.tmax_p1, 0ull);
  }
}

template <int LEVEL>
__global__ void __launch_bounds__(128) k_fx_merge(FxArgs A) {
  fx_merge_body<LEVEL>(A, blockIdx.x, gridDim.x);
}
template <int LEVEL>
__global__ void __launch_bounds__(128) k_fx_merge_b(FxBatch B) {
  uint32_t bid;
  const int k = fx_batch_find(B, blockIdx.x, bid);
  if (!(B.flags[k] & 2u) || (LEVEL == 2 && !(B.flags[k] & 1u))) return;
  WC_FX_BATCH_ARGS(sA, B, k)
  fx_merge_body<LEVEL>(sA, bid, B.start[k + 1] - B.start[k]);
}

__device__ __forceinline__ long long fx_gsum8(long long v) {
  for (int m = 1; m < 8; m <<= 1) v += __shfl_xor(v, m, 8);
  return v;
}
__device__ __forceinline__ void fx_gsum8(FxPart &a) {
  a.n = (uint32_t)fx_gsum8((long long)a.n);
  a.st = fx_gsum8(a.st);
  for (int i = 0; i < 3; ++i) a.s[i] = fx_gsum8(a.s[i]);
  for (int i = 0; i < 6; ++i) a.ss[i] = fx_gsum8(a.ss[i]);
}

#include "fx_eig3.h"

struct FxPca {
  Pca r;
  bool near;
  int which;
};

__device__ __forceinline__ void fx_pca(const FxArgs &A, const FxPart &m, const double *cc, FxPca &o) {
  const double n = (double)m.n;
  const double in = fx_rcp(n), iq = A.inv_q * in, iqq = A.inv_qq * in;
  const double mx = (double)m.s[0] * iq, my = (double)m.s[1] * iq, mz = (double)m.s[2] * iq;
  wc::M3 C;
  C.m[0][0] = (double)m.ss[0] * iqq - mx * mx;
  C.m[0][1] = C.m[1][0] = (double)m.ss[1] * iqq - mx * my;
  C.m[0][2] = C.m[2][0] = (double)m.ss[2] * iqq - mx * mz;
  C.m[1][1] = (double)m.ss[3] * iqq - my * my;
  C.m[1][2] = C.m[2][1] = (double)m.ss[4] * iqq - my * mz;
  C.m[2][2] = (double)m.ss[5] * iqq - mz * mz;
  Pca &r = o.r;
  r.c[0] = cc[0] + mx, r.c[1] = cc[1] + my, r.c[2] = cc[2] + mz;
  r.tmean = A.t_lo + ((double)m.st * in) * A.inv_tick;
  wc::M3 V;
  fx_eig3(C, r.ev, V);
  for (int i = 0; i < 3; ++i) {
    r.nrm[i] = V.m[i][0];
    for (int j = 0; j < 3; ++j) r.cov[3 * i + j] = C.m[i][j];
  }
  const double sum = (r.ev[0] + r.ev[1]) + r.ev[2];
  const double isum = fx_rcp(sum);
  r.like = 2 * (r.ev[1] - r.ev[0]) * isum;
  const double R2 = r.c[0] * r.c[0] + r.c[1] * r.c[1] + r.c[2] * r.c[2] + 1.0;
  const double dl = 16.0 * (n * fx_rsqrt(n)) * R2 * 1.1102230246251565e-16 + A.band0;
  const double dlike = 6.0 * dl * fabs(isum) + 1e-13;
  o.near = (fabs(r.ev[0] - A.P.thr) <= dl) || (fabs(r.like - A.P.min_like) <= dlike) || !(sum > 0.0);
  o.which = (fabs(r.ev[0] - A.P.thr) <= dl) ? 0 : ((fabs(r.like - A.P.min_like) <= dlike) ? 1 : 2);
}

__device__ __forceinline__ bool fx_surely_not_plane(const FxArgs &A, const FxPart &m, const double *cc) {
  const double n = (double)m.n;
  const double in = fx_rcp(n), iq = A.inv_q * in, iqq = A.inv_qq * in;
  const double mx = (double)m.s[0] * iq, my = (double)m.s[1] * iq, mz = (double)m.s[2] * iq;
  const double c00 = (double)m.ss[0] * iqq - mx * mx, c01 = (double)m.ss[1] * iqq - mx * my, c02 = (double)m.ss[2] * iqq - mx * mz;
  const double c11 = (double)m.ss[3] * iqq - my * my, c12 = (double)m.ss[4] * iqq - my * mz, c22 = (double)m.ss[5] * iqq - mz * mz;
  const double det = c00 * (c11 * c22 - c12 * c12) - c01 * (c01 * c22 - c12 * c02) + c02 * (c01 * c12 - c11 * c02);
  const double tr = (c00 + c11) + c22;
  const double px = cc[0] + mx, py = cc[1] + my, pz = cc[2] + mz;
  const double R2 = px * px + py * py + pz * pz + 1.0;
  const double dl = 16.0 * (n * fx_rsqrt(n)) * R2 * 1.1102230246251565e-16 + A.band0;
  return m.n != 0u && tr > 0.0 && 4.0 * det > 1.001 * (A.P.thr + dl) * tr * tr;
}

struct FxEmit {
  uint64_t entry;
  uint32_t bkt, r, rank;
  int lead;
  bool on;
};
__device__ __forceinline__ void fx_emit_end(const FxArgs &A, const FxEmit &e) {
  const uint32_t r = (uint32_t)__shfl((int)e.r, e.lead) + e.rank;
  if (e.on && r < A.slot_bin_cap) A.slot_bins[(size_t)e.bkt * A.slot_bin_cap + r] = e.entry;
}
__device__ __forceinline__ FxEmit fx_emit_begin(const FxArgs &A, const Pca &rr, uint32_t slot, int layer, uint32_t o1, uint32_t o2, uint32_t ord, int kx,
                                                int ky, int kz, float q0) {
  const ExParams &P = A.P;
  double nx = rr.nrm[0], ny = rr.nrm[1], nz = rr.nrm[2];
  const double d = nx * (rr.c[0] - P.view[0]) + ny * (rr.c[1] - P.view[1]) + nz * (rr.c[2] - P.view[2]);
  if (d < 0) nx = -nx, ny = -ny, nz = -nz;
  const float ql = layer == 0 ? q0 : (layer == 1 ? q0 / 2 : (q0 / 2) / 2);
  wc_surfel sf;
  sf.t = rr.tmean;
  sf.center[0] = rr.c[0], sf.center[1] = rr.c[1], sf.center[2] = rr.c[2];
  for (int i = 0; i < 9; ++i) sf.cov[i] = rr.cov[i];
  sf.normal[0] = nx, sf.normal[1] = ny, sf.normal[2] = nz;
  sf.resolution = (double)(ql * 4);
  sf.sigma = sqrt(rr.ev[0]);
  A.slots[slot] = sf;
  uint32_t node = (uint32_t)layer;
  if (layer >= 1) node |= o1 << 2;
  if (layer == 2) node |= o2 << 5;
  A.slot_ids[slot] = wc_surfel_id{kx, ky, kz, node | (ord << 8)};
  const double frac = (rr.tmean - A.t_lo) * A.inv_span;
  if (!(frac >= 0.0 && frac <= 1.0)) raise_flag(A.status, kFlagTimeRange);
  const uint64_t key = (uint64_t)min(max(frac, 0.0) * 4294967296.0, 4294967295.0);
  FxEmit e;
  e.on = true;
  e.bkt = (uint32_t)(key >> 20);
  e.entry = (key << 32) | (uint64_t)slot;
  const int lane = threadIdx.x & 63;
  e.lead = lane, e.rank = 0;
  uint32_t gsize = 1;
  if (!(WC_DBG(P, 16384))) {
    unsigned long long todo = __ballot(true);
    for (int round = 0; todo && round < 4; ++round) {
      const int lead = __ffsll((long long)todo) - 1;
      const uint32_t b0 = (uint32_t)__shfl((int)e.bkt, lead);
      const bool mine = e.bkt == b0;
      const unsigned long long m = __ballot(mine);
      if (mine) e.lead = lead, e.rank = (uint32_t)__popcll(m & ((1ull << lane) - 1ull)), gsize = (uint32_t)__popcll(m);
      todo &= ~m;
    }
  }
  e.r = 0;
  if (e.lead == lane) e.r = atomicAdd(&A.slot_counts[e.bkt], gsize);
  return e;
}
__device__ __forceinline__ void fx_emit(const FxArgs &A, const Pca &rr, uint32_t slot, int layer, uint32_t o1, uint32_t o2, uint32_t ord, int kx,
                                        int ky, int kz, float q0) {
  fx_emit_end(A, fx_emit_begin(A, rr, slot, layer, o1, o2, ord, kx, ky, kz, q0));
}

constexpr int kFxChains = 4;
constexpr int kFxJobCap = 512;
constexpr int kFxJobW = 12;
template <int N, int CAP = kFxChains>
__device__ __forceinline__ void fx_stepn(const FxArgs &A, int level, uint32_t (&ix)[CAP], const uint32_t (&bin)[CAP], FxPart (&b)[CAP]) {
  const unsigned long long *base = A.rec + (size_t)(level - 1) * A.rec_cap * kFxRecW;
  ulonglong2 w[N][7];
#pragma unroll
  for (int j = 0; j < N; ++j) {
    const ulonglong2 *r2 = (const ulonglong2 *)(base + (size_t)(ix[j] ? ix[j] - 1u : 0u) * kFxRecW);
#pragma unroll
    for (int i = 0; i < 7; ++i) w[j][i] = r2[i];
  }
#pragma unroll
  for (int j = 0; j < N; ++j) {
    const bool on = ix[j] != 0u;
    const unsigned long long m = on ? ~0ull : 0ull;
    if (on && (uint32_t)(w[j][0].x >> 32) != bin[j]) fx_fallback(A.status, 6);
    FxPart &q = b[j];
    q.n += (uint32_t)(w[j][0].x & m);
    q.st += (long long)(w[j][0].y & m);
    q.s[0] += (long long)(w[j][1].x & m), q.s[1] += (long long)(w[j][1].y & m), q.s[2] += (long long)(w[j][2].x & m);
    q.ss[0] += (long long)(w[j][2].y & m), q.ss[1] += (long long)(w[j][3].x & m), q.ss[2] += (long long)(w[j][3].y & m);
    q.ss[3] += (long long)(w[j][4].x & m), q.ss[4] += (long long)(w[j][4].y & m), q.ss[5] += (long long)(w[j][5].x & m);
    q.tmin_inv = max(q.tmin_inv, w[j][5].y & m);
    q.tmax_p1 = max(q.tmax_p1, w[j][6].x & m);
    ix[j] = (uint32_t)(w[j][6].y & m);
  }
}

struct FxWhy {
  int gap;
  int slots;
  int jobs;
  int walk1;
  int walkn;
  int big_bin;
  int job_which;
};

template <int LEVEL>
__device__ __forceinline__ uint32_t fx_dense_parent(const FxArgs &A, const uint32_t (&cnts)[kFxSub], uint32_t per, uint32_t gi, bool have_parent) {
  uint32_t pidx = 0;
  if (have_parent) {
    uint32_t rem = gi;
    bool found = false;
#pragma unroll
    for (int j = 0; j < kFxSub; ++j) {
      const uint32_t cj = cnts[j];
      if (!found) {
        if (rem < cj) {
          pidx = (uint32_t)j * per + rem;
          found = true;
        } else {
          rem -= cj;
        }
      }
    }
  }
  if (LEVEL == 1 && have_parent) pidx = A.rlist[pidx];
  return pidx;
}

template <int LEVEL>
__device__ __forceinline__ void fx_parent_header(const FxArgs &A, const unsigned long long *blk, uint32_t pidx, bool have_parent, uint32_t &key,
                                                 uint32_t &o1p, uint32_t &minbin) {
  const uint32_t *h32 = (const uint32_t *)blk;
  key = 0, o1p = 0, minbin = 0;
  if (have_parent) {
    minbin = 0xFFFFFFFFu - h32[2];
    if (LEVEL == 1) {
      key = A.rkey[pidx] - 1u;
    } else {
      const uint32_t ro = h32[0];
      o1p = (ro >> 28) & 7u;
      key = h32[1] - 1u;
    }
  }
}

__device__ __forceinline__ void fx_key_voxel(const ExParams &P, uint32_t key, int k0x, int k0y, int k0z, int &kx, int &ky, int &kz, double (&cc)[3]) {
  kx = (int)(key & 1023u) - 512 + k0x, ky = (int)((key >> 10) & 1023u) - 512 + k0y, kz = (int)(key >> 20) - 512 + k0z;
  cc[0] = (0.5 + kx) * P.vs_f, cc[1] = (0.5 + ky) * P.vs_f, cc[2] = (0.5 + kz) * P.vs_f;
}

__device__ __forceinline__ uint32_t fx_load_heads(const unsigned long long *blk, bool have_parent, uint32_t minbin, uint32_t *heads) {
  uint32_t occ = 0;
  const uint4 *hq = (const uint4 *)(blk + kFxHdrW) + (threadIdx.x & 7) * (kFxSlots / 4);
  uint32_t hv[kFxSlots];
#pragma unroll
  for (int q = 0; q < kFxSlots / 4; ++q) {
    const uint4 v = have_parent ? hq[q] : make_uint4(0u, 0u, 0u, 0u);
    hv[4 * q] = v.x, hv[4 * q + 1] = v.y, hv[4 * q + 2] = v.z, hv[4 * q + 3] = v.w;
  }
#pragma unroll
  for (int s = 0; s < kFxSlots; ++s) {
    const uint32_t p = ((uint32_t)s - minbin) & (kFxSlots - 1);
    heads[p] = hv[s];
    if (hv[s]) occ |= 1u << p;
  }
  __builtin_amdgcn_wave_barrier();
  return occ;
}

__device__ __forceinline__ double fx_tick_time(const FxArgs &A, unsigned long long tk) { return A.t_lo + (double)tk * A.inv_tick; }
__device__ __forceinline__ bool fx_starts(const FxArgs &A, unsigned long long tmin, unsigned long long prev_p1, int why) {
  if (prev_p1 == 0ull) return true;
  const double dt = fx_tick_time(A, tmin) - fx_tick_time(A, prev_p1 - 1ull);
  if (fabs(dt - A.P.gap) <= 8.0 * A.inv_tick) fx_fallback(A.status, why);
  return dt > A.P.gap;
}

__device__ __forceinline__ uint32_t fx_slots_issue(const FxArgs &A, uint32_t wsub, bool want, unsigned long long &m) {
  m = __ballot(want);
  uint32_t base_ = 0;
  if (m && threadIdx.x == 0) base_ = atomicAdd(fx_cnt(A, kFxStSlots, wsub), (uint32_t)__popcll(m));
  return base_;
}
__device__ __forceinline__ uint32_t fx_slots_finish(const FxArgs &A, uint32_t wsub, bool want, unsigned long long m, uint32_t base_, int why) {
  if (!m) return 0xFFFFFFFFu;
  base_ = (uint32_t)__shfl((int)base_, 0);
  const uint32_t local = base_ + (uint32_t)__popcll(m & ((1ull << threadIdx.x) - 1ull));
  if (want && local >= A.slots_per) {
    fx_fallback(A.status, why);
    return 0xFFFFFFFFu;
  }
  return wsub * A.slots_per + local;
}
__device__ __forceinline__ uint32_t fx_take_slots(const FxArgs &A, uint32_t wsub, bool want, int why) {
  unsigned long long m;
  const uint32_t b = fx_slots_issue(A, wsub, want, m);
  return fx_slots_finish(A, wsub, want, m, b, why);
}

__device__ __forceinline__ uint32_t fx_push_job(const FxArgs &A, unsigned long long *jb, uint32_t &jcnt, bool closing, const FxPart &cl, uint32_t ordv,
                                                uint32_t owner, int why) {
  const bool want = closing && (int)cl.n >= A.P.cluster_min;
  const unsigned long long m = __ballot(want);
  if (!m) return (uint32_t)kFxJobCap;
  const uint32_t pos = jcnt + (uint32_t)__popcll(m & ((1ull << threadIdx.x) - 1ull));
  jcnt += (uint32_t)__popcll(m);
  if (!want) return (uint32_t)kFxJobCap;
  if (pos >= (uint32_t)kFxJobCap) {
    fx_fallback(A.status, why);
    return (uint32_t)kFxJobCap;
  }
  ulonglong2 *o = (ulonglong2 *)(jb + (size_t)pos * kFxJobW);
  o[0] = make_ulonglong2((unsigned long long)cl.n | ((unsigned long long)ordv << 32), (unsigned long long)cl.st);
  o[1] = make_ulonglong2((unsigned long long)cl.s[0], (unsigned long long)cl.s[1]);
  o[2] = make_ulonglong2((unsigned long long)cl.s[2], (unsigned long long)cl.ss[0]);
  o[3] = make_ulonglong2((unsigned long long)cl.ss[1], (unsigned long long)cl.ss[2]);
  o[4] = make_ulonglong2((unsigned long long)cl.ss[3], (unsigned long long)cl.ss[4]);
  o[5] = make_ulonglong2((unsigned long long)cl.ss[5], (unsigned long long)owner);
  return pos;
}

template <int LEVEL, int CHAINS, class PushJob>
__device__ __forceinline__ void fx_walk_node(const FxArgs &A, uint32_t occ, uint32_t minbin, const uint32_t *heads, bool add_root,
                                             unsigned long long (*root)[13], const FxWhy &why, PushJob &push_job, FxPart &tot, uint32_t &ncl) {
  fx_zero(tot);
  ncl = 0;
  uint32_t todo = (WC_DBG(A.P, 512)) ? 0u : occ;
  unsigned long long prev_p1 = 0ull;
  FxPart cur;
  fx_zero(cur);
  uint32_t ord = 0;
  while (__ballot(todo != 0u)) {
    uint32_t ix[CHAINS], bn[CHAINS];
    int pj[CHAINS];
    FxPart b[CHAINS];
#pragma unroll
    for (int j = 0; j < CHAINS; ++j) {
      fx_zero(b[j]);
      pj[j] = 0, ix[j] = 0u;
      if (todo) {
        pj[j] = __ffs((int)todo) - 1;
        todo &= todo - 1u;
        ix[j] = heads[pj[j]];
      }
      bn[j] = minbin + (uint32_t)pj[j];
    }
    int guard = 0;
    const bool several = __ballot(ix[1] != 0u) != 0ull;
    if (!several) {
      while (__ballot(ix[0] != 0u)) {
        fx_stepn<1, CHAINS>(A, LEVEL, ix, bn, b);
        if (++guard > 200000) {
          fx_fallback(A.status, why.walk1);
          break;
        }
      }
    } else {
      for (;;) {
        uint32_t any = 0u;
#pragma unroll
        for (int j = 0; j < CHAINS; ++j) any |= ix[j];
        if (!__ballot(any != 0u)) break;
        fx_stepn<CHAINS, CHAINS>(A, LEVEL, ix, bn, b);
        if (++guard > 200000) {
          fx_fallback(A.status, why.walkn);
          break;
        }
      }
      if (guard > A.P.merge_min && threadIdx.x == 0) {
        uint32_t *hm = host_mailbox(A.status);
        if (hm) hm[LEVEL == 1 ? 15 : 16] = 1u;
      }
    }
#pragma unroll
    for (int j = 0; j < CHAINS; ++j) {
      if (j > 0 && !several) break;
      const bool have = b[j].n != 0u;
      bool closing = false;
      if (have) {
        if (b[j].n > (1u << 20)) fx_fallback(A.status, why.big_bin);
        if (fx_starts(A, kFxTMax - b[j].tmin_inv, prev_p1, why.gap)) {
          ++ncl;
          closing = cur.n != 0u;
        }
        prev_p1 = b[j].tmax_p1;
        fx_acc(tot, b[j]);
        if (add_root) fx_add_cell(&root[pj[j]][0], b[j]);
      }
      push_job(closing, cur, ord, (uint32_t)threadIdx.x);
      if (closing) {
        ++ord;
        fx_zero(cur);
      }
      if (have) fx_acc(cur, b[j]);
    }
  }
  push_job(ncl > 1u, cur, ord, (uint32_t)threadIdx.x);
}

template <class PushJob>
__device__ __forceinline__ uint32_t fx_root_clusters(const FxArgs &A, bool on, const unsigned long long (*root)[13], int why_gap, PushJob &push_job) {
  const uint32_t owner = 64u + (uint32_t)(threadIdx.x >> 3);
  uint32_t root_ncl = 0;
  FxPart cur;
  fx_zero(cur);
  unsigned long long prev_p1 = 0ull;
  uint32_t ord = 0;
  for (int p = 0; p < kFxSlots; ++p) {
    bool closing = false;
    FxPart b;
    fx_zero(b);
    if (on) {
      const unsigned long long *c = &root[p][0];
      if ((uint32_t)c[0]) {
        b.n = (uint32_t)c[0], b.st = (long long)c[1];
        for (int i = 0; i < 3; ++i) b.s[i] = (long long)c[2 + i];
        for (int i = 0; i < 6; ++i) b.ss[i] = (long long)c[5 + i];
        b.tmin_inv = c[11], b.tmax_p1 = c[12];
        if (fx_starts(A, kFxTMax - b.tmin_inv, prev_p1, why_gap)) {
          ++root_ncl;
          closing = cur.n != 0u;
        }
        prev_p1 = b.tmax_p1;
      }
    }
    push_job(closing, cur, ord, owner);
    if (closing) {
      ++ord;
      fx_zero(cur);
    }
    if (b.n) fx_acc(cur, b);
  }
  push_job(root_ncl > 1u, cur, ord, owner);
  return root_ncl;
}

template <int LEVEL>
__device__ __forceinline__ FxEmit fx_test_children(const FxArgs &A, bool have_parent, const FxPart &tot, uint32_t ncl, uint32_t key, uint32_t o1p, int kx,
                                                   int ky, int kz, const double *cc, float q0, uint32_t wsub, int why_slots, uint8_t *s_flag,
                                                   uint32_t *s_gkey, uint32_t *s_go1p, FxPart &rt, bool &parent_live, uint32_t &split) {
  const ExParams &P = A.P;
  const int lane = threadIdx.x, g = lane >> 3, gl = lane & 7;
  fx_zero(rt);
  if (LEVEL == 1) {
    rt = tot;
    fx_gsum8(rt);
  }
  parent_live = LEVEL == 1 ? (have_parent && (int)rt.n > P.min_points) : have_parent;
  const bool children_exist = LEVEL == 1 ? (P.max_layer >= 1) : true;
  const bool tested = parent_live && children_exist && (int)tot.n > P.min_points && !(WC_DBG(P, 256));
  const bool early = tested && ncl == 1u && (int)tot.n >= P.cluster_min;
  unsigned long long early_m;
  const uint32_t early_b = fx_slots_issue(A, wsub, early, early_m);
  FxPca pc;
  pc.near = false;
  if (tested) {
    fx_pca(A, tot, cc, pc);
    if (pc.near) fx_fallback(A.status, 13);
  }
  const bool plane = tested && (pc.r.ev[0] < P.thr) && (pc.r.like > P.min_like);
  split = (LEVEL == 1 && P.max_layer >= 2) ? ((uint32_t)(__ballot(tested && !plane) >> (g * 8)) & 0xFFu) : 0u;
  FxEmit pend;
  pend.on = false, pend.entry = 0, pend.bkt = 0, pend.r = 0, pend.rank = 0, pend.lead = lane;
  {
    const bool want = plane && ncl == 1u && (int)tot.n >= P.cluster_min && !(pc.r.ev[0] > P.thr || pc.r.like < P.min_like);
    const uint32_t sl = fx_slots_finish(A, wsub, early, early_m, early_b, why_slots);
    if (want && sl != 0xFFFFFFFFu) {
      if (LEVEL == 1)
        pend = fx_emit_begin(A, pc.r, sl, 1, (uint32_t)gl, 0u, 0u, kx, ky, kz, q0);
      else
        pend = fx_emit_begin(A, pc.r, sl, 2, o1p, (uint32_t)gl, 0u, kx, ky, kz, q0);
    }
  }
  s_flag[lane] = (plane && ncl > 1u && !(WC_DBG(P, 128))) ? 1 : 0;
  if (gl == 0) s_gkey[g] = key, s_go1p[g] = o1p, s_flag[64 + g] = 0;
  return pend;
}

template <class RootNcl>
__device__ __forceinline__ void fx_test_root(const FxArgs &A, bool parent_live, const FxPart &rt, const double *cc, int kx, int ky, int kz, float q0,
                                             uint32_t wsub, int why_slots, uint8_t *s_flag, RootNcl root_ncl_of) {
  const ExParams &P = A.P;
  if (!__ballot(parent_live)) return;
  const int g = threadIdx.x >> 3, gl = threadIdx.x & 7;
  const bool rtest = parent_live && gl == 0 && !fx_surely_not_plane(A, rt, cc);
  FxPca rp;
  rp.near = false;
  rp.r.ev[0] = 1e300, rp.r.like = 0.0;
  if (rtest) {
    fx_pca(A, rt, cc, rp);
    if (rp.near) fx_fallback(A.status, 14);
  }
  const bool rpl = rtest && (rp.r.ev[0] < P.thr) && (rp.r.like > P.min_like);
  const uint32_t root_ncl = root_ncl_of(rpl);
  if (rpl && root_ncl > 1u && !(WC_DBG(P, 1024))) s_flag[64 + g] = 1;
  const bool want = rpl && root_ncl == 1u && (int)rt.n >= P.cluster_min && !(rp.r.ev[0] > P.thr || rp.r.like < P.min_like);
  const uint32_t sl = fx_take_slots(A, wsub, want, why_slots);
  if (want && sl != 0xFFFFFFFFu) fx_emit(A, rp.r, sl, 0, 0u, 0u, 0u, kx, ky, kz, q0);
}

template <int LEVEL>
__device__ __forceinline__ void fx_run_job(const FxArgs &A, bool want, uint32_t owner, const FxPart &cl, uint32_t ordv, int k0x, int k0y, int k0z,
                                           float q0, uint32_t wsub, const FxWhy &why, const uint32_t *s_gkey, const uint32_t *s_go1p) {
  const ExParams &P = A.P;
  const uint32_t og = owner < 64u ? owner >> 3 : owner - 64u;
  int jx, jy, jz;
  double jc[3];
  fx_key_voxel(P, s_gkey[og], k0x, k0y, k0z, jx, jy, jz, jc);
  FxPca cp;
  cp.near = false;
  if (want) {
    fx_pca(A, cl, jc, cp);
    if (cp.near) {
      fx_fallback(A.status, 15);
      if (why.job_which >= 0) fx_fallback(A.status, why.job_which + cp.which);
    }
    want = !(cp.r.ev[0] > P.thr || cp.r.like < P.min_like);
  }
  const uint32_t sl = fx_take_slots(A, wsub, want, why.slots);
  if (want && sl != 0xFFFFFFFFu) {
    if (owner >= 64u)
      fx_emit(A, cp.r, sl, 0, 0u, 0u, ordv, jx, jy, jz, q0);
    else if (LEVEL == 1)
      fx_emit(A, cp.r, sl, 1, owner & 7u, 0u, ordv, jx, jy, jz, q0);
    else
      fx_emit(A, cp.r, sl, 2, s_go1p[og], owner & 7u, ordv, jx, jy, jz, q0);
  }
}

__device__ __forceinline__ bool fx_queue_layer2(const FxArgs &A, bool have_parent, uint32_t split, uint32_t pidx, uint32_t key, unsigned long long *blk,
                                                uint32_t wsub) {
  const int lane = threadIdx.x, g = lane >> 3, gl = lane & 7;
  const uint32_t nq = (uint32_t)__popc(split);
  uint32_t dem = (gl == 0 && have_parent) ? nq : 0u, pre = dem;
  for (int d = 8; d < 64; d <<= 1) {
    const uint32_t o = __shfl_up(pre, d);
    if (lane >= d) pre += o;
  }
  const uint32_t wave_total = (uint32_t)__shfl((int)pre, 56);
  uint32_t base_ = 0;
  if (wave_total) {
    if (lane == 0) base_ = atomicAdd(fx_cnt(A, kFxStNodes2, wsub), wave_total);
    base_ = (uint32_t)__shfl((int)base_, 0);
  }
  const uint32_t gbase = (uint32_t)__shfl((int)(base_ + pre - dem), g * 8);
  bool queued = false;
  if (have_parent && nq) {
    if (gbase + nq > A.mq_per) {
      fx_fallback(A.status, 16);
    } else {
      const uint32_t first = wsub * A.mq_per + gbase;
      queued = true;
      if (gl == 0) {
        uint32_t *w32 = (uint32_t *)blk;
        w32[12] = split;
        w32[13] = first;
      }
      if ((split >> gl) & 1u) {
        const uint32_t qn = first + (uint32_t)__popc(split & ((1u << gl) - 1u));
        uint32_t *q32 = (uint32_t *)(A.blk2 + (size_t)qn * kFxBlockW);
        const bool first_child = (split & ((1u << gl) - 1u)) == 0u;
        q32[0] = pidx | ((uint32_t)gl << 28) | (first_child ? 0x80000000u : 0u);
        q32[1] = key + 1u;
      }
    }
  }
  return queued;
}

__device__ __forceinline__ void fx_clear_heads(unsigned long long *blk) {
  uint4 *hz = (uint4 *)(blk + kFxHdrW) + (threadIdx.x & 7) * 4;
  hz[0] = hz[1] = hz[2] = hz[3] = make_uint4(0u, 0u, 0u, 0u);
}
template <int LEVEL>
__device__ __forceinline__ void fx_clear_header(const FxArgs &A, unsigned long long *blk, uint32_t pidx, bool queued) {
  uint32_t *w32 = (uint32_t *)blk;
  if (LEVEL == 1) {
    if (!queued) {
      w32[2] = 0u;
      A.rkey[pidx] = 0u;
    }
  } else {
    const uint32_t ro = w32[0];
    w32[0] = w32[1] = w32[2] = 0u;
    if (ro & 0x80000000u) {
      const uint32_t rslot = ro & 0xFFFFFFFu;
      uint32_t *r32 = (uint32_t *)(A.blk + (size_t)rslot * kFxBlockW);
      r32[2] = r32[12] = r32[13] = 0u;
      A.rkey[rslot] = 0u;
    }
  }
}

constexpr FxWhy kFxWhyNodes = {7, 8, 9, 10, 11, 12, -1};
template <int LEVEL>
__global__ void __launch_bounds__(64) k_fx_nodes(FxArgs A) {
  __shared__ uint32_t s_heads[64][kFxSlots + 1];
  __shared__ unsigned long long s_root[8][kFxSlots][13];
  __shared__ uint8_t s_jown[kFxJobCap];
  __shared__ uint8_t s_flag[72];
  __shared__ uint32_t s_gkey[8], s_go1p[8];
  const ExParams &P = A.P;
  const int lane = threadIdx.x, g = lane >> 3, gl = lane & 7;
  const uint32_t bank = LEVEL == 1 ? kFxStRoots : kFxStNodes2;
  const uint32_t per = LEVEL == 1 ? A.mr_per : A.mq_per;
  const bool stat = A.static_map != 0u;
  const uint32_t sj = blockIdx.x & (kFxSub - 1);
  const uint32_t nwj = (gridDim.x - sj + kFxSub - 1) / kFxSub;
  uint32_t total = 0, cnts[kFxSub], cnt_j = 0;
  if (stat) {
    cnt_j = min(*fx_cnt(A, bank, (int)sj), per);
  } else {
#pragma unroll
    for (int j = 0; j < kFxSub; ++j) {
      cnts[j] = min(*fx_cnt(A, bank, j), per);
      total += cnts[j];
    }
  }
  double x0, y0, z0;
  ex_origin(A.pts, x0, y0, z0);
  const int k0x = vox(x0, P.vs), k0y = vox(y0, P.vs), k0z = vox(z0, P.vs);
  const float q0 = P.vs_f / 4;
  const uint32_t wsub = blockIdx.x & (kFxSub - 1);
  if (WC_DBG(P, 2048)) return;
  for (uint32_t it = 0;; ++it) {
    uint32_t pidx = 0;
    bool have_parent;
    if (stat) {
      const uint32_t chunk = blockIdx.x / kFxSub + it * nwj;
      if (chunk * 8u >= per) break;
      const uint32_t local = chunk * 8u + (uint32_t)g;
      pidx = sj * per + min(local, per - 1u);
      if (LEVEL == 1) {
        pidx = A.rlist[pidx] & A.tr_mask;
        asm volatile("" : "+v"(pidx));
      }
      if (chunk * 8u >= cnt_j) break;
      have_parent = local < cnt_j;
    } else {
      const uint32_t w0 = (blockIdx.x + it * gridDim.x) * 8u;
      if (w0 >= total) break;
      const uint32_t gi = w0 + (uint32_t)g;
      have_parent = gi < total;
      pidx = fx_dense_parent<LEVEL>(A, cnts, per, gi, have_parent);
    }
    unsigned long long *blk = (LEVEL == 1 ? A.blk : A.blk2) + (size_t)pidx * kFxBlockW;
    uint32_t key, o1p, minbin;
    fx_parent_header<LEVEL>(A, blk, pidx, have_parent, key, o1p, minbin);
    int kx, ky, kz;
    double cc[3];
    fx_key_voxel(P, key, k0x, k0y, k0z, kx, ky, kz, cc);
    const uint32_t occ = fx_load_heads(blk, have_parent, minbin, s_heads[lane]);
    uint32_t jcnt = 0;
    const bool one_bin = __ballot((occ & (occ - 1u)) != 0u) == 0ull;
    if (LEVEL == 1 && !one_bin) {
      for (int i = lane; i < 8 * kFxSlots * 13; i += 64) (&s_root[0][0][0])[i] = 0ull;
      __builtin_amdgcn_wave_barrier();
    }
    unsigned long long *jb = A.jobs + (size_t)blockIdx.x * kFxJobCap * kFxJobW;
    auto push_job = [&](bool closing, const FxPart &cl, uint32_t ordv, uint32_t owner) {
      const uint32_t pos = fx_push_job(A, jb, jcnt, closing, cl, ordv, owner, kFxWhyNodes.jobs);
      if (pos < (uint32_t)kFxJobCap) s_jown[pos] = (uint8_t)owner;
    };
    FxPart tot;
    uint32_t ncl;
    fx_walk_node<LEVEL, kFxChains>(A, occ, minbin, s_heads[lane], LEVEL == 1 && !one_bin, s_root[g], kFxWhyNodes, push_job, tot, ncl);
    __builtin_amdgcn_wave_barrier();
    FxPart rt;
    bool parent_live;
    uint32_t split;
    const FxEmit pend = fx_test_children<LEVEL>(A, have_parent, tot, ncl, key, o1p, kx, ky, kz, cc, q0, wsub, kFxWhyNodes.slots, s_flag, s_gkey, s_go1p,
                                                rt, parent_live, split);
    if (LEVEL == 1) {
      fx_test_root(A, parent_live, rt, cc, kx, ky, kz, q0, wsub, kFxWhyNodes.slots, s_flag, [&](bool rpl) -> uint32_t {
        if (!__ballot(rpl)) return 0u;
        if (one_bin) {
          for (int i = lane; i < 8 * kFxSlots * 13; i += 64) (&s_root[0][0][0])[i] = 0ull;
          __builtin_amdgcn_wave_barrier();
          const bool grp = ((__ballot(rpl) >> (g * 8)) & 0xFFull) != 0ull;
          if (grp && tot.n) fx_add_cell(&s_root[g][__ffs((int)occ) - 1][0], tot);
          __builtin_amdgcn_wave_barrier();
        }
        return fx_root_clusters(A, rpl, s_root[g], kFxWhyNodes.gap, push_job);
      });
    }
    fx_emit_end(A, pend);
    if (jcnt) __builtin_amdgcn_fence(__ATOMIC_RELEASE, "workgroup");
    __builtin_amdgcn_wave_barrier();
    for (uint32_t r0 = 0; r0 < min(jcnt, (uint32_t)kFxJobCap); r0 += 64u) {
      const uint32_t ji = r0 + (uint32_t)lane;
      bool want = ji < min(jcnt, (uint32_t)kFxJobCap);
      const uint32_t owner = want ? s_jown[ji] : 0u;
      want = want && s_flag[owner] != 0;
      if (!__ballot(want)) continue;
      FxPart cl;
      fx_zero(cl);
      uint32_t ordv = 0;
      if (want) {
        const unsigned long long *o = jb + (size_t)ji * kFxJobW;
        unsigned long long w[11];
#pragma unroll
        for (int i = 0; i < 11; ++i) w[i] = __hip_atomic_load(&o[i], __ATOMIC_RELAXED, __HIP_MEMORY_SCOPE_AGENT);
        cl.n = (uint32_t)w[0], ordv = (uint32_t)(w[0] >> 32), cl.st = (long long)w[1];
        for (int i = 0; i < 3; ++i) cl.s[i] = (long long)w[2 + i];
        for (int i = 0; i < 6; ++i) cl.ss[i] = (long long)w[5 + i];
      }
      fx_run_job<LEVEL>(A, want, owner, cl, ordv, k0x, k0y, k0z, q0, wsub, kFxWhyNodes, s_gkey, s_go1p);
    }
    __builtin_amdgcn_wave_barrier();
    const bool queued = LEVEL == 1 && fx_queue_layer2(A, have_parent, split, pidx, key, blk, wsub);
    if (have_parent && !(WC_DBG(P, 8192))) {
      fx_clear_heads(blk);
      if (gl == 0) fx_clear_header<LEVEL>(A, blk, pidx, queued);
    }
  }
}
```

### wildcat-slam_amd/csrc/extract_plan.h

```cpp
#pragma once
#include <algorithm>
#include <cstdint>

#include "../../include/wc_types.h"

struct wc_ctx;

constexpr int kBuckets = 4096;
constexpr int kSlotBinMax = 512;
constexpr uint32_t kPtBinMax = 1024;
constexpr int kFxSub = 16;
constexpr int kFxPts = 4, kFxThreads = 256, kFxTile = kFxPts * kFxThreads;

constexpr uint32_t kFlagKeyRange = 1u;
constexpr uint32_t kFlagSlotOverflow = 2u;
constexpr uint32_t kFlagTimeRange = 4u;
constexpr uint32_t kFlagBucketOverflow = 8u;
constexpr uint32_t kFlagSlotBinOverflow = 16u;
constexpr uint32_t kFlagLdsOverflow = 32u;
constexpr uint32_t kFlagFxFallback = 64u;
constexpr uint32_t kFlagsFxRepeat = kFlagFxFallback | kFlagKeyRange | kFlagSlotBinOverflow | kFlagTimeRange;

struct ExPath {
  bool fx = false;
  bool wide = false;
  bool run_sort = false;
  bool bin_order = false;
};
inline uint32_t ex_path_bits(const ExPath &p) { return (p.fx ? 1u : 0u) | (p.wide ? 2u : 0u) | (p.run_sort ? 4u : 0u) | (p.bin_order ? 8u : 0u); }

struct ExSweep {
  bool active = false;
  wc_points pts{};
  double t_lo = 0, t_hi = 0;
  wc_surfel *d_out = nullptr;
  wc_surfel_id *d_ids = nullptr;
  uint64_t cap = 0;
  ExPath path;
  uint32_t runs = 0;
  uint32_t ticket = 0;
  int (*tail)(wc_ctx *, bool) = nullptr;
  bool layer2_done = true;
  alignas(16) unsigned char roots_args[768];
  unsigned slot_end_bit = 0;
  bool fx_split = false;
  bool batch_defer = false;
  bool deferred = false;
};

struct ExMemory {
  int general_calls = 0;
  uint32_t lds_cap = 256;
  bool unordered = false;
  uint32_t last_splits = 256;
  uint32_t fx_backoff = 0, fx_skip_calls = 0;
  bool fx_long_lists = false, fx_long_lists2 = false;
  bool fx_spill_full = false;
  int fx_parity = 0;
  bool fx_dirty = false;
  bool fx_ctrl_ready = false;
  bool precleared = false;
  bool bucket_attr_set = false;
  uint32_t ticket_seq = 0;
  uint32_t fx_fallbacks = 0;
  uint32_t fx_last_flags = 0;
  uint32_t fx_last_why = 0;
};

inline void ex_reset_backoff(ExMemory &m) { m.fx_backoff = m.fx_skip_calls = 0; }

inline ExPath ex_first_path(ExMemory &m, bool fx_ok, bool no_bucket_sort) {
  const bool general = m.general_calls > 0 || no_bucket_sort;
  if (m.general_calls > 0) --m.general_calls;
  if (fx_ok && m.fx_skip_calls > 0) --m.fx_skip_calls, fx_ok = false;
  return ExPath{fx_ok, false, !fx_ok && !general, true};
}

inline bool ex_next_path(ExPath &p, uint32_t flags, const uint32_t *why_words, ExMemory &m) {
  if (p.fx) {
    m.fx_last_flags = flags;
    if (!(flags & kFlagsFxRepeat)) {
      m.fx_backoff = 0;
      return false;
    }
    ++m.fx_fallbacks;
    m.fx_last_why = 0;
    for (int i = 0; i < 24; ++i)
      if (why_words[i]) m.fx_last_why |= 1u << i;
    if (m.fx_last_why & (1u << 4)) m.fx_spill_full = true;
    m.fx_backoff = std::min(32u, std::max(1u, m.fx_backoff * 2u));
    m.fx_skip_calls = m.fx_backoff - 1u;
    m.fx_dirty = true;
    m.fx_ctrl_ready = false;
    p = ExPath{false, false, !(m.general_calls > 0), true};
    return true;
  }
  if (p.run_sort) {
    bool bucket = flags & kFlagBucketOverflow;
    if ((flags & kFlagLdsOverflow) && !bucket && !(flags & kFlagKeyRange) && m.lds_cap < kPtBinMax) {
      m.lds_cap *= 2;
      return true;
    }
    if (flags & kFlagLdsOverflow) bucket = true;
    if (bucket && !(flags & kFlagKeyRange)) {
      p.run_sort = false;
      m.general_calls = 15;
      return true;
    }
  }
  if ((flags & kFlagKeyRange) && !p.wide) {
    p.wide = true, p.run_sort = false;
    return true;
  }
  if ((flags & kFlagSlotBinOverflow) && p.bin_order) {
    p.bin_order = false;
    return true;
  }
  return false;
}

inline void ex_learn_unordered(ExMemory &m, const ExPath &p, uint32_t run_count, uint64_t n) {
  if (p.run_sort && run_count > 0) m.unordered = (uint64_t)run_count * 4 > n;
}

inline uint64_t ex_total_slots(uint64_t n, int max_layer, int cluster_min, uint64_t floor) {
  return std::max<uint64_t>((n * (uint64_t)(max_layer + 1)) / (uint64_t)cluster_min + 1, floor);
}
inline uint32_t ex_slot_bin_cap(uint64_t total_slots) {
  uint32_t bin_cap = 64;
  while (bin_cap < (uint32_t)kSlotBinMax && (uint64_t)bin_cap * kBuckets < 2 * total_slots) bin_cap *= 2;
  return bin_cap;
}
inline unsigned ex_fx_tiles(uint64_t n) { return (unsigned)((n + kFxTile - 1) / kFxTile); }
inline unsigned ex_fx_node_grid(uint64_t n) { return std::min<unsigned>(256 * 16, std::max<unsigned>(64, (unsigned)(n / 256))); }
inline unsigned ex_fx_batch_node_grid(uint64_t n) { return std::max(64u, ex_fx_node_grid(n) / 8u); }
inline unsigned ex_fx_layer2_grid(unsigned ngrid, uint32_t last_splits) { return std::min(std::min(256u * 8u, ngrid), std::max(64u, last_splits)); }
```

### wildcat-slam_amd/csrc/extract_split.inc

```

constexpr int kFxNodeW = 11;
constexpr int kFxDescW = 64;
constexpr int kFxWalkChains = 2;
constexpr uint32_t kFxJobSub0 = 8;
constexpr FxWhy kFxWhySplit = {17, 23, 18, 19, 20, 21, 17};

template <int LEVEL>
__device__ __forceinline__ void fx_walk_body(const FxArgs &A, const uint32_t bid, const uint32_t nblk) {
  __shared__ uint32_t s_heads[64][kFxSlots + 1];
  __shared__ unsigned long long s_root[8][kFxSlots][13];
  const ExParams &P = A.P;
  const int lane = threadIdx.x, g = lane >> 3, gl = lane & 7;
  const uint32_t bank = LEVEL == 1 ? kFxStRoots : kFxStNodes2;
  const uint32_t per = LEVEL == 1 ? A.mr_per : A.mq_per;
  uint32_t total = 0, cnts[kFxSub];
#pragma unroll
  for (int j = 0; j < kFxSub; ++j) {
    cnts[j] = min(*fx_cnt(A, bank, j), per);
    total += cnts[j];
  }
  if (WC_DBG(P, 2048)) return;
  unsigned long long *jb = A.jobs + (size_t)bid * kFxJobCap * kFxJobW;
  for (uint32_t it = 0;; ++it) {
    const uint32_t vw = bid + it * nblk;
    const uint32_t w0 = vw * 8u;
    if (w0 >= total) break;
    const uint32_t gi = w0 + (uint32_t)g;
    const bool have_parent = gi < total;
    const uint32_t pidx = fx_dense_parent<LEVEL>(A, cnts, per, gi, have_parent);
    unsigned long long *blk = (LEVEL == 1 ? A.blk : A.blk2) + (size_t)pidx * kFxBlockW;
    uint32_t key, o1p, minbin;
    fx_parent_header<LEVEL>(A, blk, pidx, have_parent, key, o1p, minbin);
    const uint32_t occ = fx_load_heads(blk, have_parent, minbin, s_heads[lane]);
    uint32_t jcnt = 0;
    uint32_t rocc = occ;
    if (LEVEL == 1) {
      for (int m = 1; m < 8; m <<= 1) rocc |= (uint32_t)__shfl_xor((int)rocc, m, 8);
    }
    const bool root_multi = LEVEL == 1 && __ballot(have_parent && (rocc & (rocc - 1u)) != 0u) != 0ull;
    if (root_multi) {
      for (int i = lane; i < 8 * kFxSlots * 13; i += 64) (&s_root[0][0][0])[i] = 0ull;
      __builtin_amdgcn_wave_barrier();
    }
    auto push_job = [&](bool closing, const FxPart &cl, uint32_t ordv, uint32_t owner) {
      fx_push_job(A, jb, jcnt, closing, cl, ordv, owner, kFxWhySplit.jobs);
    };
    FxPart tot;
    uint32_t ncl;
    fx_walk_node<LEVEL, kFxWalkChains>(A, occ, minbin, s_heads[lane], root_multi, s_root[g], kFxWhySplit, push_job, tot, ncl);
    __builtin_amdgcn_wave_barrier();
    uint32_t root_ncl = 0;
    if (LEVEL == 1) {
      long long rn = (long long)tot.n;
      rn = fx_gsum8(rn);
      const bool rl = have_parent && gl == 0 && (int)rn > P.min_points;
      root_ncl = rl ? 1u : 0u;
      if (root_multi && __ballot(rl && (rocc & (rocc - 1u)) != 0u)) root_ncl = fx_root_clusters(A, rl, s_root[g], kFxWhySplit.gap, push_job);
    }
    {
      unsigned long long *nd = A.nodes + (size_t)vw * kFxNodeW * 64 + lane;
      nd[0 * 64] = (unsigned long long)tot.n | ((unsigned long long)ncl << 32);
      nd[1 * 64] = (unsigned long long)tot.st;
#pragma unroll
      for (int i = 0; i < 3; ++i) nd[(2 + i) * 64] = (unsigned long long)tot.s[i];
#pragma unroll
      for (int i = 0; i < 6; ++i) nd[(5 + i) * 64] = (unsigned long long)tot.ss[i];
      uint32_t *wd = A.wdesc + (size_t)vw * kFxDescW;
      if (gl == 0) {
        const uint32_t flags = (have_parent ? 1u : 0u) | (o1p << 1) | (min(root_ncl, 255u) << 8);
        *(uint4 *)(wd + 4 * g) = make_uint4(pidx, key, flags, 0u);
      }
      const uint32_t nj = min(jcnt, (uint32_t)kFxJobCap);
      uint32_t jbase = 0;
      if (nj) {
        const uint32_t sp = vw & 7u;
        if (lane == 0) jbase = atomicAdd(fx_cnt(A, kFxStSpillBank, kFxJobSub0 + sp), nj);
        jbase = (uint32_t)__shfl((int)jbase, 0);
        if (jbase + nj > A.jobpool_per) {
          fx_fallback(A.status, 22);
        } else {
          __builtin_amdgcn_fence(__ATOMIC_RELEASE, "workgroup");
          __builtin_amdgcn_wave_barrier();
          const unsigned long long *src = jb;
          unsigned long long *dst = A.jobpool + ((size_t)sp * A.jobpool_per + jbase) * kFxJobW;
          for (uint32_t i = (uint32_t)lane; i < nj * (uint32_t)kFxJobW; i += 64u)
            dst[i] = __hip_atomic_load(&src[i], __ATOMIC_RELAXED, __HIP_MEMORY_SCOPE_AGENT);
        }
      }
      if (lane == 0) *(uint2 *)(wd + 32) = make_uint2(nj, jbase);
    }
    if (have_parent && !(WC_DBG(P, 8192))) fx_clear_heads(blk);
    __builtin_amdgcn_wave_barrier();
  }
}

template <int LEVEL>
__device__ __forceinline__ void fx_test_body(const FxArgs &A, const uint32_t bid, const uint32_t nblk) {
  __shared__ uint8_t s_flag[72];
  __shared__ uint32_t s_gkey[8], s_go1p[8];
  const ExParams &P = A.P;
  const int lane = threadIdx.x, g = lane >> 3, gl = lane & 7;
  const uint32_t bank = LEVEL == 1 ? kFxStRoots : kFxStNodes2;
  const uint32_t per = LEVEL == 1 ? A.mr_per : A.mq_per;
  uint32_t total = 0;
#pragma unroll
  for (int j = 0; j < kFxSub; ++j) total += min(*fx_cnt(A, bank, j), per);
  double x0, y0, z0;
  ex_origin(A.pts, x0, y0, z0);
  const int k0x = vox(x0, P.vs), k0y = vox(y0, P.vs), k0z = vox(z0, P.vs);
  const float q0 = P.vs_f / 4;
  const uint32_t wsub = bid & (kFxSub - 1);
  if (WC_DBG(P, 2048)) return;
  for (uint32_t it = 0;; ++it) {
    const uint32_t vw = bid + it * nblk;
    if (vw * 8u >= total) break;
    const uint32_t *wd = A.wdesc + (size_t)vw * kFxDescW;
    const uint4 d4 = *(const uint4 *)(wd + 4 * g);
    const uint2 dj = *(const uint2 *)(wd + 32);
    const unsigned long long *nd = A.nodes + (size_t)vw * kFxNodeW * 64 + lane;
    unsigned long long nw[kFxNodeW];
#pragma unroll
    for (int i = 0; i < kFxNodeW; ++i) nw[i] = nd[i * 64];
    const bool have_parent = (d4.z & 1u) != 0u;
    const uint32_t pidx = d4.x, key = d4.y, o1p = (d4.z >> 1) & 7u, root_ncl = (d4.z >> 8) & 0xFFu;
    const uint32_t jcnt = dj.x, jbase = dj.y;
    unsigned long long *blk = (LEVEL == 1 ? A.blk : A.blk2) + (size_t)pidx * kFxBlockW;
    int kx, ky, kz;
    double cc[3];
    fx_key_voxel(P, key, k0x, k0y, k0z, kx, ky, kz, cc);
    FxPart tot;
    fx_zero(tot);
    uint32_t ncl = 0;
    if (have_parent) {
      tot.n = (uint32_t)nw[0], ncl = (uint32_t)(nw[0] >> 32), tot.st = (long long)nw[1];
#pragma unroll
      for (int i = 0; i < 3; ++i) tot.s[i] = (long long)nw[2 + i];
#pragma unroll
      for (int i = 0; i < 6; ++i) tot.ss[i] = (long long)nw[5 + i];
    }
    FxPart rt;
    bool parent_live;
    uint32_t split;
    const FxEmit pend = fx_test_children<LEVEL>(A, have_parent, tot, ncl, key, o1p, kx, ky, kz, cc, q0, wsub, kFxWhySplit.slots, s_flag, s_gkey, s_go1p,
                                                rt, parent_live, split);
    if (LEVEL == 1) fx_test_root(A, parent_live, rt, cc, kx, ky, kz, q0, wsub, kFxWhySplit.slots, s_flag, [&](bool) { return root_ncl; });
    fx_emit_end(A, pend);
    __builtin_amdgcn_wave_barrier();
    const unsigned long long *jp = A.jobpool + ((size_t)(vw & 7u) * A.jobpool_per + jbase) * kFxJobW;
    for (uint32_t r0 = 0; r0 < jcnt; r0 += 64u) {
      const uint32_t ji = r0 + (uint32_t)lane;
      bool want = ji < jcnt;
      unsigned long long w[kFxJobW];
#pragma unroll
      for (int i = 0; i < kFxJobW; ++i) w[i] = want ? jp[(size_t)ji * kFxJobW + i] : 0ull;
      const uint32_t owner = want ? min((uint32_t)w[11], 71u) : 0u;
      want = want && s_flag[owner] != 0;
      if (!__ballot(want)) continue;
      FxPart cl;
      fx_zero(cl);
      cl.n = (uint32_t)w[0], cl.st = (long long)w[1];
      const uint32_t ordv = (uint32_t)(w[0] >> 32);
#pragma unroll
      for (int i = 0; i < 3; ++i) cl.s[i] = (long long)w[2 + i];
#pragma unroll
      for (int i = 0; i < 6; ++i) cl.ss[i] = (long long)w[5 + i];
      fx_run_job<LEVEL>(A, want, owner, cl, ordv, k0x, k0y, k0z, q0, wsub, kFxWhySplit, s_gkey, s_go1p);
    }
    __builtin_amdgcn_wave_barrier();
    const bool queued = LEVEL == 1 && fx_queue_layer2(A, have_parent, split, pidx, key, blk, wsub);
    if (have_parent && gl == 0 && !(WC_DBG(P, 8192))) fx_clear_header<LEVEL>(A, blk, pidx, queued);
    __builtin_amdgcn_wave_barrier();
  }
}

template <int LEVEL>
__global__ void __launch_bounds__(64) k_fx_walk(FxArgs A) {
  fx_walk_body<LEVEL>(A, blockIdx.x, gridDim.x);
}
template <int LEVEL>
__global__ void __launch_bounds__(64) k_fx_test(FxArgs A) {
  fx_test_body<LEVEL>(A, blockIdx.x, gridDim.x);
}
template <int LEVEL>
__global__ void __launch_bounds__(64) k_fx_walk_b(FxBatch B) {
  uint32_t bid;
  const int k = fx_batch_find(B, blockIdx.x, bid);
  if (LEVEL == 2 && !(B.flags[k] & 1u)) return;
  WC_FX_BATCH_ARGS(sA, B, k)
  fx_walk_body<LEVEL>(sA, bid, B.start[k + 1] - B.start[k]);
}
template <int LEVEL>
__global__ void __launch_bounds__(64) k_fx_test_b(FxBatch B) {
  uint32_t bid;
  const int k = fx_batch_find(B, blockIdx.x, bid);
  if (LEVEL == 2 && !(B.flags[k] & 1u)) return;
  WC_FX_BATCH_ARGS(sA, B, k)
  fx_test_body<LEVEL>(sA, bid, B.start[k + 1] - B.start[k]);
}
```

### wildcat-slam_amd/host/odom_c_api.cc

```cpp
#include <cstring>

#include <algorithm>

#include "../csrc/extract_plan.h"
#include "../csrc/lm_loop.h"
#include "../csrc/map_room.h"
#include "cubic_bspline.h"
#include "histogram.h"
#include "imu_resampler.h"
#include "lidar_odometry.h"
#include "map_file.h"

extern "C" {

void *wc_odom_create(int device) { return new LidarOdometry(device); }
void wc_odom_destroy(void *h) { delete (LidarOdometry *)h; }
int wc_odom_set_dev_option(void *h, const char *name, int value) { return wc_ctx_set_dev_option(((LidarOdometry *)h)->gpu_context(), name, value); }

void wc_odom_add_imu(void *h, double t, const double acc[3], const double gyr[3]) {
  ImuData d;
  d.timestamp = t;
  for (int i = 0; i < 3; ++i) d.linear_acceleration[i] = acc[i], d.angular_velocity[i] = gyr[i];
  ((LidarOdometry *)h)->AddImuData(d);
}
// ... 143 lines not shown
  std::memcpy(out14, m.position, 24);
  std::memcpy(out14 + 3, m.orientation, 32);
  std::memcpy(out14 + 7, m.scale, 24);
  for (int c = 0; c < 4; ++c) out14[10 + c] = m.color[c];
}

int wc_odom_set_map_voxel(void *h, double voxel) { return ((LidarOdometry *)h)->SetMapVoxel(voxel) ? 0 : WC_ERR_ARG; }
void wc_odom_map_size(void *h, uint64_t out3[3]) {
  const LidarOdometry *o = (const LidarOdometry *)h;
  out3[0] = o->map_voxels(), out3[1] = o->map_points(), out3[2] = o->map_rejected();
}
uint64_t wc_odom_map_export(void *h, float *xyz, uint32_t *counts, uint64_t cap) { return ((LidarOdometry *)h)->ExportMap(xyz, counts, cap); }
void wc_odom_map_clear(void *h) { ((LidarOdometry *)h)->ClearMap(); }
double wc_odom_map_ms(void *h) { return ((const LidarOdometry *)h)->last_map_ms(); }
uint64_t wc_odom_map_query(void *h, const float *xyz, uint64_t n, double max_dist, wc_map_hit *hits) {
  return ((LidarOdometry *)h)->QueryMap(xyz, n, max_dist, hits);
}
uint64_t wc_odom_map_query_knn(void *h, const float *xyz, uint64_t n, const wc_map_knn_params *params, wc_map_hit *hits, uint32_t *within) {
  return params ? ((LidarOdometry *)h)->QueryMapKnn(xyz, n, *params, hits, within) : 0;
}
uint64_t wc_odom_map_crop(void *h, const double lo[3], const double hi[3]) { return ((LidarOdometry *)h)->CropMap(lo, hi); }
void wc_odom_set_map_surfels(void *h, int on) { ((LidarOdometry *)h)->SetMapSurfels(on != 0); }
int wc_odom_map_surfels_on(void *h) { return ((LidarOdometry *)h)->config().map_surfels ? 1 : 0; }
uint64_t wc_odom_map_surfels(void *h, wc_map_surfel *surfels, uint64_t cap) { return ((LidarOdometry *)h)->ExportMapSurfels(surfels, cap); }
uint64_t wc_odom_map_query_planes(void *h, const float *xyz, uint64_t n, double max_dist, uint32_t min_points, wc_map_plane_hit *hits) {
  return ((LidarOdometry *)h)->QueryMapPlanes(xyz, n, max_dist, min_points, hits);
}
int wc_odom_map_align(void *h, const float *xyz, uint64_t n, double T_io[12], const wc_map_align_opts *opts, wc_map_align_summary *summary) {
  return opts && ((LidarOdometry *)h)->AlignToMap(xyz, n, T_io, *opts, summary) ? 1 : 0;
}
int wc_odom_map_align_sweep(void *h, const void *points48, uint64_t n, wc_pose *pose_begin_io, wc_pose *pose_end_io,
                            const wc_map_ct_align_opts *opts, wc_map_ct_align_summary *summary, int insert) {
  return opts && ((LidarOdometry *)h)->AlignSweepToMap(points48, n, pose_begin_io, pose_end_io, *opts, summary, insert != 0) ? 1 : 0;
}
int wc_odom_map_relocalize(void *h, const float *xyz, uint64_t n, double T_io[12], uint32_t factor, uint32_t n_levels,
                           const wc_map_align_opts *finest, wc_map_align_summary *summaries) {
  return finest && ((LidarOdometry *)h)->RelocalizeToMap(xyz, n, T_io, factor, n_levels, *finest, summaries) ? 1 : 0;
}
int wc_odom_map_relocalize_search(void *h, const float *xyz, uint64_t n, double T_io[12], uint32_t n_yaw, uint32_t factor, uint32_t n_levels,
                                  const wc_map_align_opts *finest, wc_map_align_summary *summaries, int32_t *best) {
  return finest && ((LidarOdometry *)h)->RelocalizeSearch(xyz, n, T_io, n_yaw, factor, n_levels, *finest, summaries, best) ? 1 : 0;
}
int wc_odom_map_relocalize_global(void *h, const float *xyz, uint64_t n, double T_io[12], uint32_t n_yaw, const uint32_t n_xyz[3],
                                  const double step[3], uint32_t top_m, uint32_t factor, uint32_t n_levels, const wc_map_align_opts *finest,
                                  wc_map_align_summary *summaries, int32_t *best) {
  return finest && ((LidarOdometry *)h)->RelocalizeGlobal(xyz, n, T_io, n_yaw, n_xyz, step, top_m, factor, n_levels, *finest, summaries, best) ? 1 : 0;
}
int wc_odom_map_linearize(void *h, const float *xyz, uint64_t n, const double T[12], const wc_map_reg_params *params, wc_map_normal_eq *out,
                          wc_map_reg_row *rows) {
  return params && ((LidarOdometry *)h)->LinearizeAgainstMap(xyz, n, T, *params, out, rows) ? 1 : 0;
}
int wc_odom_map_carve(void *h, const float *xyz, uint64_t n, const double origin[3], const wc_map_carve_params *params, wc_map_carve_result *result) {
  return params && ((LidarOdometry *)h)->CarveMap(xyz, n, origin, *params, result) ? 1 : 0;
}
int wc_odom_map_carve_remove(void *h, const float *xyz, uint64_t n, const double origin[3], const wc_map_carve_params *params,
                             wc_map_carve_result *result) {
  return params && ((LidarOdometry *)h)->CarveMapRemove(xyz, n, origin, *params, result) ? 1 : 0;
}
int wc_odom_map_remove_keys(void *h, const int32_t *keys, uint64_t n, uint64_t out3[3]) {
  return ((LidarOdometry *)h)->RemoveMapVoxels(keys, n, out3) ? 1 : 0;
}
int wc_odom_map_components(void *h, const wc_map_cc_params *params, int32_t *keys, uint32_t *labels, uint64_t cap, wc_map_component *comps,
                           uint64_t cap_comps, uint64_t out4[4]) {
  return params && ((LidarOdometry *)h)->MapComponents(*params, keys, labels, cap, comps, cap_comps, out4) ? 1 : 0;
}
int wc_odom_map_remove_small(void *h, const wc_map_cc_params *params, uint32_t min_voxels, uint64_t min_comp_points, uint64_t out4[4]) {
  return params && ((LidarOdometry *)h)->RemoveSmallMapComponents(*params, min_voxels, min_comp_points, out4) ? 1 : 0;
}
int wc_odom_set_map_carve(void *h, double range, uint32_t shell, uint32_t min_rays) {
  return ((LidarOdometry *)h)->SetMapCarve(range, shell, min_rays) ? 0 : WC_ERR_ARG;
}
int wc_host_map_room(uint64_t cap, uint64_t live_bound, uint64_t tombs, uint64_t n, uint64_t *new_cap) {
  uint64_t c = cap;
  const int rc = map_room(cap, live_bound, tombs, n, &c);
  if (new_cap) *new_cap = c;
  return rc;
}
int wc_odom_map_raycast(void *h, const float *xyz, uint64_t n, const double origin[3], const wc_map_raycast_params *params, wc_map_ray_hit *hits,
                        wc_map_raycast_result *result) {
  return params && ((LidarOdometry *)h)->CastMap(xyz, n, origin, *params, hits, result) ? 1 : 0;
}
int wc_odom_map_save(void *h, const char *path) { return path && ((LidarOdometry *)h)->SaveMap(path) ? 1 : 0; }
int wc_odom_map_load(void *h, const char *path, int merge) { return path && ((LidarOdometry *)h)->LoadMap(path, merge != 0) ? 1 : 0; }
int wc_odom_map_merge_file(void *h, const char *path, double T_io[12], uint32_t factor, uint32_t n_levels, const wc_map_align_opts *opts,
                           wc_map_align_summary *summaries) {
  return path && opts && ((LidarOdometry *)h)->MergeMapFile(path, T_io, factor, n_levels, *opts, summaries) ? 1 : 0;
}
uint64_t wc_host_map_file_encode(double voxel, uint32_t flags, const void *vox, const int64_t *mom, uint64_t n, uint8_t *out, uint64_t cap) {
  const uint64_t bytes = wc_map_file::EncodedBytes(n, (flags & wc_map_file::kFlagMoments) != 0);
  if (out && cap >= bytes) wc_map_file::Encode(voxel, flags, (const wc_map_file::Voxel *)vox, mom, n, out);
  return bytes;
}
int wc_host_map_file_decode(const uint8_t *buf, uint64_t len, double *voxel, uint32_t *flags, uint64_t *n, void *vox, int64_t *mom, uint64_t cap) {
  wc_map_file::Header h;
  const int rc = wc_map_file::Decode(buf, len, &h);
  if (rc != wc_map_file::kOk) return rc;
  if (voxel) *voxel = h.voxel;
  if (flags) *flags = h.flags;
  if (n) *n = h.n;
  if (vox && cap >= h.n) wc_map_file::Unpack(buf, h, (wc_map_file::Voxel *)vox, mom);
  return rc;
}
int wc_odom_set_map_keep_radius(void *h, double radius) { return ((LidarOdometry *)h)->SetMapKeepRadius(radius) ? 0 : WC_ERR_ARG; }
int wc_host_xyz_to_cloud2(const float *xyz, uint64_t n, uint32_t table9[9], char *names_out, uint64_t cap, uint8_t *data_out) {
  wc_wire::PointCloud2 msg;
  wc_wire::Cloud2FromXyz(xyz, n, msg);
  std::string names;
  for (size_t f = 0; f < msg.fields.size() && f < 3; ++f) {
    table9[3 * f] = msg.fields[f].offset, table9[3 * f + 1] = msg.fields[f].datatype, table9[3 * f + 2] = msg.fields[f].count;
    names += msg.fields[f].name;
    names.push_back('\0');
  }
  if (names_out && cap >= names.size()) std::memcpy(names_out, names.data(), names.size());
  if (data_out && !msg.data.empty()) std::memcpy(data_out, msg.data.data(), msg.data.size());
  return (int)msg.point_step;
}

int wc_odom_import_state(void *h, const double *samples23, uint64_t ns, const wc_imu_state *imu, uint64_t n_imu) {
  return ((LidarOdometry *)h)->ImportState(samples23, ns, imu, n_imu) ? 0 : 1;
}


int wc_host_ex_plan(int op, uint32_t mem11[11], uint32_t *path_bits, uint32_t a, uint64_t b) {
  ExMemory m;
  m.general_calls = (int)mem11[0], m.lds_cap = mem11[1], m.unordered = mem11[2] != 0, m.fx_backoff = mem11[3], m.fx_skip_calls = mem11[4];
  m.fx_spill_full = mem11[5] != 0, m.fx_fallbacks = mem11[6], m.fx_last_flags = mem11[7], m.fx_last_why = mem11[8];
  m.fx_dirty = mem11[9] != 0, m.fx_ctrl_ready = mem11[10] != 0;
  ExPath p;
  p.fx = *path_bits & 1u, p.wide = *path_bits & 2u, p.run_sort = *path_bits & 4u, p.bin_order = *path_bits & 8u;
  int rc = 0;
  if (op == 0) {
    p = ex_first_path(m, a != 0, b != 0);
  } else if (op == 1) {
    uint32_t why[24];
    for (int i = 0; i < 24; ++i) why[i] = (uint32_t)((b >> i) & 1u);
    rc = ex_next_path(p, a, why, m) ? 1 : 0;
  } else if (op == 2) {
    ex_learn_unordered(m, p, a, b);
  } else {
    ex_reset_backoff(m);
  }
  const uint32_t out[11] = {(uint32_t)m.general_calls, m.lds_cap, m.unordered, m.fx_backoff, m.fx_skip_calls, m.fx_spill_full,
                            m.fx_fallbacks, m.fx_last_flags, m.fx_last_why, m.fx_dirty, m.fx_ctrl_ready};
  std::memcpy(mem11, out, sizeof(out));
  *path_bits = ex_path_bits(p);
  return rc;
}
void wc_host_ex_sizes(uint64_t n, int max_layer, int cluster_min, uint64_t floor, uint32_t last_splits, uint64_t out5[5]) {
  out5[0] = ex_total_slots(n, max_layer, cluster_min, floor);
  out5[1] = ex_slot_bin_cap(out5[0]);
  out5[2] = ex_fx_tiles(n);
  out5[3] = ex_fx_node_grid(n);
  out5[4] = ex_fx_layer2_grid((unsigned)out5[3], last_splits);
}

int wc_host_lm_loop(int op, void *state, uint64_t state_bytes, const double *in, double *out22) {
  if (op == -1) return (int)sizeof(LmLoop);
  if (!state || state_bytes < sizeof(LmLoop) || (op != 1 && !in)) return -2;
  LmLoop L;
  std::memcpy(&L, state, sizeof(L));
  int rc = 0;
  if (op == 0)
    L = lm_begin(LmConfig{(int)in[0], (int)in[1], (int)in[2], in[3] != 0, (int)in[4], in[5] != 0}, in[6], in[7], in[8]);
  else if (op == 1)
    rc = (int)lm_next(L);
  else if (op == 2)
    rc = (int)lm_judge(L, LmMail{(int)in[0], in[1], in[2], in[3], in[4], in[5]});
  else if (op == 3)
    rc = lm_accepted(L, in[0], (int)in[1]) ? 1 : 0;
  else
    return -2;
  std::memcpy(state, &L, sizeof(L));
  if (out22) {
    const wc_solve_summary s = lm_summary(L);
    const double o[22] = {L.cost, L.gmax, L.min_cost, L.radius, L.decrease, L.x_norm, (double)L.iter, (double)L.consecutive_invalid,
                          (double)L.first_recorded, (double)L.first_step_now, (double)L.late_pending, (double)L.late_at,
                          s.initial_cost, s.final_cost, (double)s.iterations, (double)s.successful_steps, (double)s.unsuccessful_steps,
                          (double)s.termination, (double)s.n_linearizations, (double)s.n_cost_evaluations, s.first_step[0], s.first_step[1]};
    std::memcpy(out22, o, sizeof(o));
  }
  return rc;
}

void wc_host_so3(const double v3[3], double out52[52]) {
  using namespace wc;
  const V3 v = mk3(v3[0], v3[1], v3[2]);
  const Q4 q = so3_exp(v);
  const V3 l = so3_log(q);
  double *o = out52;
  o[0] = q.w, o[1] = q.x, o[2] = q.y, o[3] = q.z, o[4] = l.x, o[5] = l.y, o[6] = l.z;
  const M3 ms[5] = {so3_Jl(v), so3_Jl_inv(v), so3_Jr(v), so3_Jr_inv(v), hat(v)};
  for (int m = 0; m < 5; ++m)
    for (int i = 0; i < 3; ++i)
      for (int j = 0; j < 3; ++j) o[7 + 9 * m + 3 * i + j] = ms[m].m[i][j];
}

void wc_host_bspline_fit_eval(const double *ts, const double *pts3, uint64_t np, const double *query, uint64_t nq, double *out3,
                              uint8_t *valid, double *ctrl3) {
  using namespace wc;
  std::vector<double> t(ts, ts + np);
  std::vector<V3> p(np);
  for (uint64_t i = 0; i < np; ++i) p[i] = mk3(pts3[3 * i], pts3[3 * i + 1], pts3[3 * i + 2]);
  const CubicBSpline sp(t, p);
  for (uint64_t i = 0; i < nq; ++i) {
    V3 o = mk3(0, 0, 0);
    valid[i] = sp.Interp(query[i], o) ? 1 : 0;
    out3[3 * i] = o.x, out3[3 * i + 1] = o.y, out3[3 * i + 2] = o.z;
  }
  if (ctrl3)
    for (uint64_t i = 0; i < np; ++i)
      ctrl3[3 * i] = sp.control_points()[i].x, ctrl3[3 * i + 1] = sp.control_points()[i].y, ctrl3[3 * i + 2] = sp.control_points()[i].z;
}

void *wc_host_resampler_create(int freq) { return new ImuResampler(freq); }
void wc_host_resampler_destroy(void *h) { delete (ImuResampler *)h; }
void wc_host_resampler_add(void *h, double t, const double acc[3], const double gyr[3]) {
  ImuData d;
  d.timestamp = t;
  for (int i = 0; i < 3; ++i) d.linear_acceleration[i] = acc[i], d.angular_velocity[i] = gyr[i];
  ((ImuResampler *)h)->AddImuData(d);
}
int wc_host_resampler_advance(void *h, double out7[7]) {
  const std::shared_ptr<ImuData> r = ((ImuResampler *)h)->AdvanceGetResampledImuData();
  if (!r) return 0;
  out7[0] = r->timestamp;
  for (int i = 0; i < 3; ++i) out7[1 + i] = r->linear_acceleration[i], out7[4 + i] = r->angular_velocity[i];
  return 1;
}
}
```

Measured before the change: 21590 Mpts/s.

## Write surfels directly into time buckets instead of slots plus key bins

The fast extraction path now writes each surfel's full 160-byte record (surfel plus id) straight into its time bucket, instead of writing it to a per-subgroup slot array and a separate 64-bit key/slot entry into the bucket. The emit kernel is rewritten to read records from the bucket, rank them by time and id within the wave, and copy them to the output in order. This removes the slot-counter atomics, the slot arrays and one indirect gather in the emit stage. In exchange the bucket buffer is larger (bin_cap times 160 bytes per bucket), the ranking logic is more complex, and a new bin-floor option is added.

```diff
diff --git a/wildcat-slam_amd/csrc/ctx.h b/wildcat-slam_amd/csrc/ctx.h
--- a/wildcat-slam_amd/csrc/ctx.h
+++ b/wildcat-slam_amd/csrc/ctx.h
@@ -31,6 +31,7 @@
   int debug_skip = 0;
   int fx_merge_min = 3;
   int fx_split = -1;
+  int fx_bin_floor = 0;
   int fx_acc_form = -1;
   int no_bucket_sort = 0;
   int ex_sync = 0;
@@ -63,7 +64,7 @@
   std::string err;
   wc_buf b_ex_ctrl;
   wc_buf b_keys[2], b_vals[2], b_sorttmp, b_slots, b_slot_ids, b_slot_keys[2], b_slot_idx[2], b_cand, b_cand_meta,
-      b_status, b_misc[8], b_route[4], b_fx[10];
+      b_status, b_misc[8], b_route[4], b_fx[11];
   double match_stats[8] = {0, 0, 0, 0, 0, 0, 0, 0};
   wc_buf b_kd[10];
   std::vector<wc_ctx *> batch_subs;
diff --git a/wildcat-slam_amd/csrc/ctx.hip b/wildcat-slam_amd/csrc/ctx.hip
--- a/wildcat-slam_amd/csrc/ctx.hip
+++ b/wildcat-slam_amd/csrc/ctx.hip
@@ -60,6 +60,7 @@
     {"debug_skip", "WC_DEBUG_SKIP", &wc_dev_opts::debug_skip, false},
     {"fx_merge_min", "WC_FX_MERGE_MIN", &wc_dev_opts::fx_merge_min, false},
     {"fx_split", "WC_FX_SPLIT", &wc_dev_opts::fx_split, false},
+    {"fx_bin_floor", "WC_FX_BIN_FLOOR", &wc_dev_opts::fx_bin_floor, false},
     {"fx_acc_form", "WC_FX_ACC_FORM", &wc_dev_opts::fx_acc_form, false},
     {"no_bucket_sort", "WC_NO_BUCKET_SORT", &wc_dev_opts::no_bucket_sort, true},
     {"ex_sync", "WC_EX_SYNC", &wc_dev_opts::ex_sync, true},
diff --git a/wildcat-slam_amd/csrc/extract.hip b/wildcat-slam_amd/csrc/extract.hip
--- a/wildcat-slam_amd/csrc/extract.hip
+++ b/wildcat-slam_amd/csrc/extract.hip
@@ -1232,18 +1232,12 @@
   }
 }
 
-__global__ void __launch_bounds__(256) k_slot_emit(const uint32_t *__restrict__ counts, const uint64_t *__restrict__ bins, uint32_t bin_cap,
-                                                  const wc_surfel *__restrict__ slots, const wc_surfel_id *__restrict__ slot_ids,
-                                                  uint32_t *status, wc_surfel *out, wc_surfel_id *out_ids, uint64_t cap, uint32_t *next_ctrl,
-                                                  uint32_t next_words) {
+__global__ void __launch_bounds__(256) k_slot_order(const uint32_t *__restrict__ counts, const uint64_t *__restrict__ bins, uint32_t bin_cap,
+                                                   const wc_surfel *__restrict__ slots, const wc_surfel_id *__restrict__ slot_ids,
+                                                   uint32_t *status, wc_surfel *out, wc_surfel_id *out_ids, uint64_t cap, uint32_t *next_ctrl,
+                                                   uint32_t next_words) {
   const SlotEmitArgs E{counts, bins, bin_cap, slots, slot_ids, status, out, out_ids, cap, next_ctrl, next_words};
   slot_emit_body(E, blockIdx.x, gridDim.x);
-}
-__global__ void __launch_bounds__(256) k_slot_emit_b(const SlotEmitArgs *__restrict__ Es, int K) {
-  const uint32_t per = kBuckets / 4;
-  const uint32_t k = blockIdx.x / per;
-  if ((int)k >= K) return;
-  slot_emit_body(Es[k], blockIdx.x - k * per, per);
 }
 
 
@@ -1606,7 +1600,7 @@
   A.spill_per = (uint32_t)((n <= 8000000ull || M.fx_spill_full) ? spill_full : std::max<uint64_t>(1024, n / 32));
   A.rec_cap = tiles * (uint32_t)kFxRecTile + 8u * A.spill_per;
   const uint64_t total_slots = ex_total_slots(n, P.max_layer, P.cluster_min_points, (uint64_t)kFxSub * 256);
-  const uint32_t bin_cap = ex_slot_bin_cap(total_slots);
+  const uint32_t bin_cap = ex_fx_bin_cap(total_slots, ctx->dev.fx_bin_floor);
   WC_TRY(fx_ensure_zero(ctx, ctx->b_fx[0], (size_t)tr * 4));
   WC_TRY(wc_ensure(ctx, ctx->b_fx[1], (size_t)mr * 4));
   WC_TRY(fx_ensure_zero(ctx, ctx->b_fx[2], (size_t)tr * kFxBlockW * 8));
@@ -1623,9 +1617,7 @@
     WC_TRY(wc_ensure(ctx, ctx->b_fx[9], (size_t)8 * A.jobpool_per * kFxJobW * 8));
     A.nodes = (unsigned long long *)ctx->b_fx[7].p, A.wdesc = (uint32_t *)ctx->b_fx[8].p, A.jobpool = (unsigned long long *)ctx->b_fx[9].p;
   }
-  WC_TRY(wc_ensure(ctx, ctx->b_slots, total_slots * sizeof(wc_surfel)));
-  WC_TRY(wc_ensure(ctx, ctx->b_slot_ids, total_slots * sizeof(wc_surfel_id)));
-  WC_TRY(wc_ensure(ctx, ctx->b_slot_keys[1], (uint64_t)kBuckets * bin_cap * 8));
+  WC_TRY(wc_ensure(ctx, ctx->b_fx[10], ex_fx_bins_bytes(bin_cap)));
   if (M.fx_dirty) {
     for (int i : {0, 2, 3}) WC_HIP(ctx, hipMemsetAsync(ctx->b_fx[i].p, 0, ctx->b_fx[i].cap, st));
     M.fx_dirty = false;
@@ -1649,11 +1641,9 @@
   A.jobs = (unsigned long long *)ctx->b_fx[6].p;
   A.status = ctrl + kCtrlStatus;
   A.cnt = ctrl + kCtrlFx;
-  A.slots = (wc_surfel *)ctx->b_slots.p, A.slot_ids = (wc_surfel_id *)ctx->b_slot_ids.p;
-  A.slots_per = (uint32_t)std::min<uint64_t>(total_slots / kFxSub, 0x7FFFFFFFu);
-  A.slot_counts = ctrl + kCtrlBins;
-  A.slot_bins = (uint64_t *)ctx->b_slot_keys[1].p;
-  A.slot_bin_cap = bin_cap;
+  A.bins = (unsigned char *)ctx->b_fx[10].p;
+  A.bin_counts = ctrl + kCtrlBins;
+  A.bin_cap = bin_cap;
   ex_mark(ctx, 0);
   ex_mark(ctx, 1);
   static const bool dbg = wc_log_env("WC_FX_DEBUG");
@@ -1664,11 +1654,11 @@
     uint32_t w[64], c[4 * 16 * 32];
     (void)hipMemcpy(w, A.status, sizeof(w), hipMemcpyDeviceToHost);
     (void)hipMemcpy(c, A.cnt, sizeof(c), hipMemcpyDeviceToHost);
-    uint32_t r = 0, q = 0, sl = 0, sp = 0;
-    for (int j = 0; j < 16; ++j) r += c[j * 32], q += c[(16 + j) * 32], sl += c[(32 + j) * 32], sp += c[(48 + j) * 32];
-    fprintf(stderr, " %s flags=%u roots=%u nodes2=%u slots=%u spill=%u\n", hipGetErrorString(e), w[1], r, q, sl, sp);
+    uint32_t r = 0, q = 0, sp = 0;
+    for (int j = 0; j < 16; ++j) r += c[j * 32], q += c[(16 + j) * 32], sp += c[(48 + j) * 32];
+    fprintf(stderr, " %s flags=%u roots=%u nodes2=%u spill=%u\n", hipGetErrorString(e), w[1], r, q, sp);
   };
-  if (dbg) fprintf(stderr, "[fx] n=%llu tiles=%u mr_per=%u mq_per=%u tr=%u slots_per=%u bin_cap=%u\n", (unsigned long long)n, tiles, A.mr_per, A.mq_per, tr, A.slots_per, bin_cap);
+  if (dbg) fprintf(stderr, "[fx] n=%llu tiles=%u mr_per=%u mq_per=%u tr=%u bin_cap=%u\n", (unsigned long long)n, tiles, A.mr_per, A.mq_per, tr, bin_cap);
   ex_keep_for_tail(ctx, A, &fx_tail);
   if (ctx->ex.batch_defer) {
     ctx->ex.layer2_done = P.max_layer >= 2 && M.last_splits > 0;
@@ -1716,9 +1706,8 @@
   ex_mark(ctx, 4);
   uint32_t *next_ctrl = (uint32_t *)ctx->b_fx[5].p + (size_t)(M.fx_parity ^ 1) * kCtrlWords;
   static_assert(kCtrlWords <= (kBuckets / 4) * 256, "k_slot_emit's grid covers the control block");
-  k_slot_emit<<<kBuckets / 4, 256, 0, st>>>(A.slot_counts, A.slot_bins, A.slot_bin_cap, (const wc_surfel *)ctx->b_slots.p,
-                                           (const wc_surfel_id *)ctx->b_slot_ids.p, A.status, ctx->ex.d_out, ctx->ex.d_ids, ctx->ex.cap, next_ctrl,
-                                           kCtrlWords);
+  k_slot_emit<<<kBuckets / 4, 256, 0, st>>>(
+      BinEmitArgs{A.bin_counts, A.cnt, A.bins, A.bin_cap, A.status, ctx->ex.d_out, ctx->ex.d_ids, ctx->ex.cap, next_ctrl, kCtrlWords});
   ex_mark(ctx, 5);
   ctx->ex.ticket = 0;
   if (ctx->h_status_dev && !ctx->ex_prof && !ctx->dev.ex_sync) {
@@ -1754,8 +1743,8 @@
   ctx->ex.layer2_done = layer2;
   ex_mark(ctx, 4);
   if (fast_slots) {
-    k_slot_emit<<<kBuckets / 4, 256, 0, st>>>(A.slot_counts, A.slot_bins, A.slot_bin_cap, (const wc_surfel *)ctx->b_slots.p,
-                                             (const wc_surfel_id *)ctx->b_slot_ids.p, status, ctx->ex.d_out, ctx->ex.d_ids, cap, nullptr, 0u);
+    k_slot_order<<<kBuckets / 4, 256, 0, st>>>(A.slot_counts, A.slot_bins, A.slot_bin_cap, (const wc_surfel *)ctx->b_slots.p,
+                                              (const wc_surfel_id *)ctx->b_slot_ids.p, status, ctx->ex.d_out, ctx->ex.d_ids, cap, nullptr, 0u);
   } else {
     k_iota<<<(unsigned)((total_slots + 255) / 256), 256, 0, st>>>((uint32_t *)ctx->b_slot_idx[0].p, total_slots);
     WC_TRY(sort_pairs<uint64_t>(ctx, (uint64_t *)ctx->b_slot_keys[0].p, (uint64_t *)ctx->b_slot_keys[1].p,
@@ -2011,11 +2000,11 @@
     ctx->batch_subs.push_back(sub);
   }
   hipStream_t st = ctx->stream;
-  const size_t o_emit = (sizeof(FxArgs) * K + 15) & ~(size_t)15, o_tab = (o_emit + sizeof(SlotEmitArgs) * K + 15) & ~(size_t)15;
+  const size_t o_emit = (sizeof(FxArgs) * K + 15) & ~(size_t)15, o_tab = (o_emit + sizeof(BinEmitArgs) * K + 15) & ~(size_t)15;
   const size_t bytes = o_tab + (size_t)(3 * (K + 1) + K) * 4;
   std::vector<unsigned char> host(bytes, 0);
   FxArgs *args = (FxArgs *)host.data();
-  SlotEmitArgs *emit = (SlotEmitArgs *)(host.data() + o_emit);
+  BinEmitArgs *emit = (BinEmitArgs *)(host.data() + o_emit);
   uint32_t *s_acc = (uint32_t *)(host.data() + o_tab), *s_nodes = s_acc + (K + 1), *s_g2 = s_nodes + (K + 1), *flags = s_g2 + (K + 1);
   int Kd = 0;
   bool any_l2 = false, any_merge = false;
@@ -2050,8 +2039,8 @@
     any_l2 = any_l2 || (f & 1u);
     any_merge = any_merge || (f & 2u);
     uint32_t *next_ctrl = (uint32_t *)sub->b_fx[5].p + (size_t)(sub->ex_mem.fx_parity ^ 1) * kCtrlWords;
-    emit[Kd++] = SlotEmitArgs{A.slot_counts, A.slot_bins, A.slot_bin_cap, (const wc_surfel *)sub->b_slots.p, (const wc_surfel_id *)sub->b_slot_ids.p,
-                              A.status, sub->ex.d_out, sub->ex.d_ids, sub->ex.cap, next_ctrl, (uint32_t)kCtrlWords};
+    emit[Kd++] = BinEmitArgs{A.bin_counts, A.cnt, A.bins, A.bin_cap, A.status, sub->ex.d_out, sub->ex.d_ids, sub->ex.cap, next_ctrl,
+                             (uint32_t)kCtrlWords};
   }
   if (Kd == 0) return WC_OK;
   WC_TRY(wc_ensure(ctx, ctx->b_batch, bytes));
@@ -2075,7 +2064,7 @@
     k_fx_walk_b<2><<<s_g2[Kd], 64, 0, st>>>(B);
     k_fx_test_b<2><<<s_g2[Kd], 64, 0, st>>>(B);
   }
-  k_slot_emit_b<<<(unsigned)Kd * (kBuckets / 4), 256, 0, st>>>((const SlotEmitArgs *)(d + o_emit), Kd);
+  k_slot_emit_b<<<(unsigned)Kd * (kBuckets / 4), 256, 0, st>>>((const BinEmitArgs *)(d + o_emit), Kd);
   WC_HIP(ctx, hipGetLastError());
   return WC_OK;
 }
diff --git a/wildcat-slam_amd/csrc/extract_fast.inc b/wildcat-slam_amd/csrc/extract_fast.inc
--- a/wildcat-slam_amd/csrc/extract_fast.inc
+++ b/wildcat-slam_amd/csrc/extract_fast.inc
@@ -7,7 +7,7 @@
 constexpr int kFxRecW = 16;
 constexpr int kFxHdrW = 16;
 constexpr int kFxBlockW = kFxHdrW + 8 * kFxSlots / 2;
-constexpr uint32_t kFxStRoots = 0, kFxStNodes2 = 1, kFxStSlots = 2, kFxStSpillBank = 3;
+constexpr uint32_t kFxStRoots = 0, kFxStNodes2 = 1, kFxStSpillBank = 3;
 constexpr int kFxCntStride = 32;
 constexpr int kFxCntWords = 4 * kFxSub * kFxCntStride;
 constexpr unsigned long long kFxTMax = 0xFFFFFFFFFFFFull;
@@ -44,12 +44,9 @@
   uint32_t *wdesc;
   unsigned long long *jobpool;
   uint32_t jobpool_per;
-  wc_surfel *slots;
-  wc_surfel_id *slot_ids;
-  uint32_t slots_per;
-  uint32_t *slot_counts;
-  uint64_t *slot_bins;
-  uint32_t slot_bin_cap;
+  unsigned char *bins;
+  uint32_t *bin_counts;
+  uint32_t bin_cap;
 };
 
 __device__ __forceinline__ void fx_fallback(uint32_t *status, int why) {
@@ -932,63 +929,70 @@
   return m.n != 0u && tr > 0.0 && 4.0 * det > 1.001 * (A.P.thr + dl) * tr * tr;
 }
 
-struct FxEmit {
-  uint64_t entry;
+constexpr uint32_t kFxBinRec = 160;
+static_assert(sizeof(wc_surfel) == 144 && sizeof(wc_surfel_id) == 16, "a bucket record is nine + one 16-byte pieces");
+struct FxClaimB {
   uint32_t bkt, r, rank;
   int lead;
-  bool on;
+  bool bad;
 };
-__device__ __forceinline__ void fx_emit_end(const FxArgs &A, const FxEmit &e) {
-  const uint32_t r = (uint32_t)__shfl((int)e.r, e.lead) + e.rank;
-  if (e.on && r < A.slot_bin_cap) A.slot_bins[(size_t)e.bkt * A.slot_bin_cap + r] = e.entry;
-}
-__device__ __forceinline__ FxEmit fx_emit_begin(const FxArgs &A, const Pca &rr, uint32_t slot, int layer, uint32_t o1, uint32_t o2, uint32_t ord, int kx,
-                                                int ky, int kz, float q0) {
+__device__ __forceinline__ FxClaimB fx_bin_claim(const FxArgs &A, double tmean) {
+  const double frac = (tmean - A.t_lo) * A.inv_span;
+  const uint64_t key = (uint64_t)min(max(frac, 0.0) * 4294967296.0, 4294967295.0);
+  const int lane = threadIdx.x & 63;
+  FxClaimB c;
+  c.bad = !(frac >= 0.0 && frac <= 1.0);
+  c.bkt = (uint32_t)(key >> 20);
+  c.lead = lane, c.rank = 0;
+  uint32_t gsize = 1;
+  if (!(WC_DBG(A.P, 16384))) {
+    unsigned long long todo = __ballot(true);
+    for (int round = 0; todo && round < 4; ++round) {
+      const int lead = __ffsll((long long)todo) - 1;
+      const uint32_t b0 = (uint32_t)__shfl((int)c.bkt, lead);
+      const bool mine = c.bkt == b0;
+      const unsigned long long m = __ballot(mine);
+      if (mine) c.lead = lead, c.rank = (uint32_t)__popcll(m & ((1ull << lane) - 1ull)), gsize = (uint32_t)__popcll(m);
+      todo &= ~m;
+    }
+  }
+  c.r = 0;
+  if (c.lead == lane) c.r = atomicAdd(&A.bin_counts[c.bkt], gsize);
+  return c;
+}
+__device__ __forceinline__ uint32_t fx_bin_place(const FxClaimB &c) { return (uint32_t)__shfl((int)c.r, c.lead) + c.rank; }
+__device__ __forceinline__ double2 *fx_bin_rec(const FxArgs &A, uint32_t bkt, uint32_t place) {
+  return (double2 *)(A.bins + ((size_t)bkt * A.bin_cap + place) * kFxBinRec);
+}
+__device__ __forceinline__ void fx_bin_store(const FxArgs &A, const FxClaimB &c, uint32_t place, const Pca &rr, int layer, uint32_t o1, uint32_t o2,
+                                             uint32_t ord, int kx, int ky, int kz, float q0) {
   const ExParams &P = A.P;
+  if (c.bad) raise_flag(A.status, kFlagTimeRange);
+  if (place >= A.bin_cap) return;
   double nx = rr.nrm[0], ny = rr.nrm[1], nz = rr.nrm[2];
   const double d = nx * (rr.c[0] - P.view[0]) + ny * (rr.c[1] - P.view[1]) + nz * (rr.c[2] - P.view[2]);
   if (d < 0) nx = -nx, ny = -ny, nz = -nz;
   const float ql = layer == 0 ? q0 : (layer == 1 ? q0 / 2 : (q0 / 2) / 2);
-  wc_surfel sf;
-  sf.t = rr.tmean;
-  sf.center[0] = rr.c[0], sf.center[1] = rr.c[1], sf.center[2] = rr.c[2];
-  for (int i = 0; i < 9; ++i) sf.cov[i] = rr.cov[i];
-  sf.normal[0] = nx, sf.normal[1] = ny, sf.normal[2] = nz;
-  sf.resolution = (double)(ql * 4);
-  sf.sigma = sqrt(rr.ev[0]);
-  A.slots[slot] = sf;
   uint32_t node = (uint32_t)layer;
   if (layer >= 1) node |= o1 << 2;
   if (layer == 2) node |= o2 << 5;
-  A.slot_ids[slot] = wc_surfel_id{kx, ky, kz, node | (ord << 8)};
-  const double frac = (rr.tmean - A.t_lo) * A.inv_span;
-  if (!(frac >= 0.0 && frac <= 1.0)) raise_flag(A.status, kFlagTimeRange);
-  const uint64_t key = (uint64_t)min(max(frac, 0.0) * 4294967296.0, 4294967295.0);
-  FxEmit e;
-  e.on = true;
-  e.bkt = (uint32_t)(key >> 20);
-  e.entry = (key << 32) | (uint64_t)slot;
-  const int lane = threadIdx.x & 63;
-  e.lead = lane, e.rank = 0;
-  uint32_t gsize = 1;
-  if (!(WC_DBG(P, 16384))) {
-    unsigned long long todo = __ballot(true);
-    for (int round = 0; todo && round < 4; ++round) {
-      const int lead = __ffsll((long long)todo) - 1;
-      const uint32_t b0 = (uint32_t)__shfl((int)e.bkt, lead);
-      const bool mine = e.bkt == b0;
-      const unsigned long long m = __ballot(mine);
-      if (mine) e.lead = lead, e.rank = (uint32_t)__popcll(m & ((1ull << lane) - 1ull)), gsize = (uint32_t)__popcll(m);
-      todo &= ~m;
-    }
-  }
-  e.r = 0;
-  if (e.lead == lane) e.r = atomicAdd(&A.slot_counts[e.bkt], gsize);
-  return e;
-}
-__device__ __forceinline__ void fx_emit(const FxArgs &A, const Pca &rr, uint32_t slot, int layer, uint32_t o1, uint32_t o2, uint32_t ord, int kx,
-                                        int ky, int kz, float q0) {
-  fx_emit_end(A, fx_emit_begin(A, rr, slot, layer, o1, o2, ord, kx, ky, kz, q0));
+  const wc_surfel_id id{kx, ky, kz, node | (ord << 8)};
+  double2 *o = fx_bin_rec(A, c.bkt, place);
+  o[0] = make_double2(rr.tmean, rr.c[0]);
+  o[1] = make_double2(rr.c[1], rr.c[2]);
+  o[2] = make_double2(rr.cov[0], rr.cov[1]);
+  o[3] = make_double2(rr.cov[2], rr.cov[3]);
+  o[4] = make_double2(rr.cov[4], rr.cov[5]);
+  o[5] = make_double2(rr.cov[6], rr.cov[7]);
+  o[6] = make_double2(rr.cov[8], nx);
+  o[7] = make_double2(ny, nz);
+  o[8] = make_double2((double)(ql * 4), sqrt(rr.ev[0]));
+  *(uint4 *)(o + 9) = *(const uint4 *)&id;
+}
+__device__ __forceinline__ void fx_emit(const FxArgs &A, const Pca &rr, int layer, uint32_t o1, uint32_t o2, uint32_t ord, int kx, int ky, int kz,
+                                        float q0) {
+  const FxClaimB c = fx_bin_claim(A, rr.tmean);
+  fx_bin_store(A, c, fx_bin_place(c), rr, layer, o1, o2, ord, kx, ky, kz, q0);
 }
 
 constexpr int kFxChains = 4;
@@ -1101,28 +1105,6 @@
   const double dt = fx_tick_time(A, tmin) - fx_tick_time(A, prev_p1 - 1ull);
   if (fabs(dt - A.P.gap) <= 8.0 * A.inv_tick) fx_fallback(A.status, why);
   return dt > A.P.gap;
-}
-
-__device__ __forceinline__ uint32_t fx_slots_issue(const FxArgs &A, uint32_t wsub, bool want, unsigned long long &m) {
-  m = __ballot(want);
-  uint32_t base_ = 0;
-  if (m && threadIdx.x == 0) base_ = atomicAdd(fx_cnt(A, kFxStSlots, wsub), (uint32_t)__popcll(m));
-  return base_;
-}
-__device__ __forceinline__ uint32_t fx_slots_finish(const FxArgs &A, uint32_t wsub, bool want, unsigned long long m, uint32_t base_, int why) {
-  if (!m) return 0xFFFFFFFFu;
-  base_ = (uint32_t)__shfl((int)base_, 0);
-  const uint32_t local = base_ + (uint32_t)__popcll(m & ((1ull << threadIdx.x) - 1ull));
-  if (want && local >= A.slots_per) {
-    fx_fallback(A.status, why);
-    return 0xFFFFFFFFu;
-  }
-  return wsub * A.slots_per + local;
-}
-__device__ __forceinline__ uint32_t fx_take_slots(const FxArgs &A, uint32_t wsub, bool want, int why) {
-  unsigned long long m;
-  const uint32_t b = fx_slots_issue(A, wsub, want, m);
-  return fx_slots_finish(A, wsub, want, m, b, why);
 }
 
 __device__ __forceinline__ uint32_t fx_push_job(const FxArgs &A, unsigned long long *jb, uint32_t &jcnt, bool closing, const FxPart &cl, uint32_t ordv,
@@ -1263,9 +1245,9 @@
 }
 
 template <int LEVEL>
-__device__ __forceinline__ FxEmit fx_test_children(const FxArgs &A, bool have_parent, const FxPart &tot, uint32_t ncl, uint32_t key, uint32_t o1p, int kx,
-                                                   int ky, int kz, const double *cc, float q0, uint32_t wsub, int why_slots, uint8_t *s_flag,
-                                                   uint32_t *s_gkey, uint32_t *s_go1p, FxPart &rt, bool &parent_live, uint32_t &split) {
+__device__ __forceinline__ void fx_test_children(const FxArgs &A, bool have_parent, const FxPart &tot, uint32_t ncl, uint32_t key, uint32_t o1p, int kx,
+                                                 int ky, int kz, const double *cc, float q0, uint8_t *s_flag, uint32_t *s_gkey, uint32_t *s_go1p,
+                                                 FxPart &rt, bool &parent_live, uint32_t &split) {
   const ExParams &P = A.P;
   const int lane = threadIdx.x, g = lane >> 3, gl = lane & 7;
   fx_zero(rt);
@@ -1276,9 +1258,6 @@
   parent_live = LEVEL == 1 ? (have_parent && (int)rt.n > P.min_points) : have_parent;
   const bool children_exist = LEVEL == 1 ? (P.max_layer >= 1) : true;
   const bool tested = parent_live && children_exist && (int)tot.n > P.min_points && !(WC_DBG(P, 256));
-  const bool early = tested && ncl == 1u && (int)tot.n >= P.cluster_min;
-  unsigned long long early_m;
-  const uint32_t early_b = fx_slots_issue(A, wsub, early, early_m);
   FxPca pc;
   pc.near = false;
   if (tested) {
@@ -1287,26 +1266,22 @@
   }
   const bool plane = tested && (pc.r.ev[0] < P.thr) && (pc.r.like > P.min_like);
   split = (LEVEL == 1 && P.max_layer >= 2) ? ((uint32_t)(__ballot(tested && !plane) >> (g * 8)) & 0xFFu) : 0u;
-  FxEmit pend;
-  pend.on = false, pend.entry = 0, pend.bkt = 0, pend.r = 0, pend.rank = 0, pend.lead = lane;
   {
     const bool want = plane && ncl == 1u && (int)tot.n >= P.cluster_min && !(pc.r.ev[0] > P.thr || pc.r.like < P.min_like);
-    const uint32_t sl = fx_slots_finish(A, wsub, early, early_m, early_b, why_slots);
-    if (want && sl != 0xFFFFFFFFu) {
+    if (want) {
       if (LEVEL == 1)
-        pend = fx_emit_begin(A, pc.r, sl, 1, (uint32_t)gl, 0u, 0u, kx, ky, kz, q0);
+        fx_emit(A, pc.r, 1, (uint32_t)gl, 0u, 0u, kx, ky, kz, q0);
       else
-        pend = fx_emit_begin(A, pc.r, sl, 2, o1p, (uint32_t)gl, 0u, kx, ky, kz, q0);
+        fx_emit(A, pc.r, 2, o1p, (uint32_t)gl, 0u, kx, ky, kz, q0);
     }
   }
   s_flag[lane] = (plane && ncl > 1u && !(WC_DBG(P, 128))) ? 1 : 0;
   if (gl == 0) s_gkey[g] = key, s_go1p[g] = o1p, s_flag[64 + g] = 0;
-  return pend;
 }
 
 template <class RootNcl>
 __device__ __forceinline__ void fx_test_root(const FxArgs &A, bool parent_live, const FxPart &rt, const double *cc, int kx, int ky, int kz, float q0,
-                                             uint32_t wsub, int why_slots, uint8_t *s_flag, RootNcl root_ncl_of) {
+                                             uint8_t *s_flag, RootNcl root_ncl_of) {
   const ExParams &P = A.P;
   if (!__ballot(parent_live)) return;
   const int g = threadIdx.x >> 3, gl = threadIdx.x & 7;
@@ -1322,13 +1297,12 @@
   const uint32_t root_ncl = root_ncl_of(rpl);
   if (rpl && root_ncl > 1u && !(WC_DBG(P, 1024))) s_flag[64 + g] = 1;
   const bool want = rpl && root_ncl == 1u && (int)rt.n >= P.cluster_min && !(rp.r.ev[0] > P.thr || rp.r.like < P.min_like);
-  const uint32_t sl = fx_take_slots(A, wsub, want, why_slots);
-  if (want && sl != 0xFFFFFFFFu) fx_emit(A, rp.r, sl, 0, 0u, 0u, 0u, kx, ky, kz, q0);
+  if (want) fx_emit(A, rp.r, 0, 0u, 0u, 0u, kx, ky, kz, q0);
 }
 
 template <int LEVEL>
 __device__ __forceinline__ void fx_run_job(const FxArgs &A, bool want, uint32_t owner, const FxPart &cl, uint32_t ordv, int k0x, int k0y, int k0z,
-                                           float q0, uint32_t wsub, const FxWhy &why, const uint32_t *s_gkey, const uint32_t *s_go1p) {
+                                           float q0, const FxWhy &why, const uint32_t *s_gkey, const uint32_t *s_go1p) {
   const ExParams &P = A.P;
   const uint32_t og = owner < 64u ? owner >> 3 : owner - 64u;
   int jx, jy, jz;
@@ -1344,14 +1318,13 @@
     }
     want = !(cp.r.ev[0] > P.thr || cp.r.like < P.min_like);
   }
-  const uint32_t sl = fx_take_slots(A, wsub, want, why.slots);
-  if (want && sl != 0xFFFFFFFFu) {
+  if (want) {
     if (owner >= 64u)
-      fx_emit(A, cp.r, sl, 0, 0u, 0u, ordv, jx, jy, jz, q0);
+      fx_emit(A, cp.r, 0, 0u, 0u, ordv, jx, jy, jz, q0);
     else if (LEVEL == 1)
-      fx_emit(A, cp.r, sl, 1, owner & 7u, 0u, ordv, jx, jy, jz, q0);
+      fx_emit(A, cp.r, 1, owner & 7u, 0u, ordv, jx, jy, jz, q0);
     else
-      fx_emit(A, cp.r, sl, 2, s_go1p[og], owner & 7u, ordv, jx, jy, jz, q0);
+      fx_emit(A, cp.r, 2, s_go1p[og], owner & 7u, ordv, jx, jy, jz, q0);
   }
 }
 
@@ -1496,10 +1469,9 @@
     FxPart rt;
     bool parent_live;
     uint32_t split;
-    const FxEmit pend = fx_test_children<LEVEL>(A, have_parent, tot, ncl, key, o1p, kx, ky, kz, cc, q0, wsub, kFxWhyNodes.slots, s_flag, s_gkey, s_go1p,
-                                                rt, parent_live, split);
+    fx_test_children<LEVEL>(A, have_parent, tot, ncl, key, o1p, kx, ky, kz, cc, q0, s_flag, s_gkey, s_go1p, rt, parent_live, split);
     if (LEVEL == 1) {
-      fx_test_root(A, parent_live, rt, cc, kx, ky, kz, q0, wsub, kFxWhyNodes.slots, s_flag, [&](bool rpl) -> uint32_t {
+      fx_test_root(A, parent_live, rt, cc, kx, ky, kz, q0, s_flag, [&](bool rpl) -> uint32_t {
         if (!__ballot(rpl)) return 0u;
         if (one_bin) {
           for (int i = lane; i < 8 * kFxSlots * 13; i += 64) (&s_root[0][0][0])[i] = 0ull;
@@ -1511,7 +1483,6 @@
         return fx_root_clusters(A, rpl, s_root[g], kFxWhyNodes.gap, push_job);
       });
     }
-    fx_emit_end(A, pend);
     if (jcnt) __builtin_amdgcn_fence(__ATOMIC_RELEASE, "workgroup");
     __builtin_amdgcn_wave_barrier();
     for (uint32_t r0 = 0; r0 < min(jcnt, (uint32_t)kFxJobCap); r0 += 64u) {
@@ -1532,7 +1503,7 @@
         for (int i = 0; i < 3; ++i) cl.s[i] = (long long)w[2 + i];
         for (int i = 0; i < 6; ++i) cl.ss[i] = (long long)w[5 + i];
       }
-      fx_run_job<LEVEL>(A, want, owner, cl, ordv, k0x, k0y, k0z, q0, wsub, kFxWhyNodes, s_gkey, s_go1p);
+      fx_run_job<LEVEL>(A, want, owner, cl, ordv, k0x, k0y, k0z, q0, kFxWhyNodes, s_gkey, s_go1p);
     }
     __builtin_amdgcn_wave_barrier();
     const bool queued = LEVEL == 1 && fx_queue_layer2(A, have_parent, split, pidx, key, blk, wsub);
@@ -1542,3 +1513,160 @@
     }
   }
 }
+
+struct BinEmitArgs {
+  const uint32_t *counts;
+  const uint32_t *fx_cnt;
+  const unsigned char *bins;
+  uint32_t bin_cap;
+  uint32_t *status;
+  wc_surfel *out;
+  wc_surfel_id *out_ids;
+  uint64_t cap;
+  uint32_t *next_ctrl;
+  uint32_t next_words;
+};
+__device__ __forceinline__ void bin_emit_body(const BinEmitArgs &E, const uint32_t bid, const uint32_t nblk) {
+  const uint32_t bin_cap = E.bin_cap;
+  uint32_t *status = E.status;
+  wc_surfel *out = E.out;
+  wc_surfel_id *out_ids = E.out_ids;
+  const uint64_t cap = E.cap;
+  if (E.next_ctrl) {
+    const uint32_t i = bid * 256u + threadIdx.x;
+    if (i < E.next_words) E.next_ctrl[i] = (i == 8u || i == 9u) ? status[i] : 0u;
+  }
+  __shared__ double s_t[4][kSlotBinMax];
+  __shared__ uint32_t s_rank[4][kSlotBinMax];
+  __shared__ uint32_t s_red[4];
+  const int t = threadIdx.x, w = t >> 6, lane = t & 63;
+  const uint32_t b0 = bid * 4u;
+  static_assert(kBuckets / 4 <= 4 * 256, "four uint4 loads per thread cover the counts");
+  const uint4 *c4 = (const uint4 *)E.counts;
+  uint4 v[4];
+#pragma unroll
+  for (int k = 0; k < 4; ++k) {
+    const uint32_t i = (uint32_t)t + 256u * k;
+    v[k] = i < bid ? c4[i] : make_uint4(0u, 0u, 0u, 0u);
+  }
+  const uint4 own = c4[bid];
+  const unsigned char *bin = E.bins + (size_t)(b0 + w) * bin_cap * kFxBinRec;
+  constexpr int kBinSpec = 16;
+  double st = 0.0;
+  uint4 idv = make_uint4(0u, 0u, 0u, 0u);
+  if (lane < kBinSpec) {
+    st = *(const double *)(bin + (size_t)lane * kFxBinRec);
+    idv = *(const uint4 *)(bin + (size_t)lane * kFxBinRec + 144);
+  }
+  const int sub = lane / 10, piece = lane - sub * 10;
+  double2 d0 = make_double2(0.0, 0.0), d1 = d0;
+  if (sub < 6) {
+    d0 = ((const double2 *)(bin + (size_t)sub * kFxBinRec))[piece];
+    d1 = ((const double2 *)(bin + (size_t)(sub + 6) * kFxBinRec))[piece];
+  }
+  uint32_t part = 0;
+#pragma unroll
+  for (int k = 0; k < 4; ++k) part += v[k].x + v[k].y + v[k].z + v[k].w;
+  for (int off = 32; off >= 1; off >>= 1) part += __shfl_xor(part, off);
+  if (lane == 0) s_red[w] = part;
+  __syncthreads();
+  uint32_t base = s_red[0] + s_red[1] + s_red[2] + s_red[3];
+  const uint32_t n0 = own.x, n1 = own.y, n2 = own.z, n3 = own.w;
+  if (bid == nblk - 1 && t == 0) {
+    status[0] = base + n0 + n1 + n2 + n3;
+    uint32_t *hm = host_mailbox(status);
+    if (hm) {
+      hm[0] = base + n0 + n1 + n2 + n3;
+      uint32_t queued = status[4];
+      for (int j = 0; j < kFxSub; ++j) queued += E.fx_cnt[(kFxStNodes2 * kFxSub + j) * kFxCntStride];
+      hm[4] = queued;
+      hm[5] = status[5];
+    }
+  }
+  base += (w > 0 ? n0 : 0u) + (w > 1 ? n1 : 0u) + (w > 2 ? n2 : 0u);
+  const uint32_t c = w == 0 ? n0 : (w == 1 ? n1 : (w == 2 ? n2 : n3));
+  if (c == 0) return;
+  if (c > bin_cap) {
+    if (lane == 0) raise_flag(status, kFlagSlotBinOverflow);
+    return;
+  }
+  auto store = [&](uint32_t rank, bool on, const double2 &d) {
+    const uint64_t o = (uint64_t)base + rank;
+    if (!on || o >= cap) return;
+    if (piece < 9)
+      ((double2 *)(out + o))[piece] = d;
+    else if (out_ids)
+      *(double2 *)(out_ids + o) = d;
+  };
+  if (c > (uint32_t)kBinSpec && lane >= kBinSpec && (uint32_t)lane < c) {
+    st = *(const double *)(bin + (size_t)lane * kFxBinRec);
+    idv = *(const uint4 *)(bin + (size_t)lane * kFxBinRec + 144);
+  }
+  if (c <= 64u) {
+    const unsigned long long sb = (unsigned long long)__double_as_longlong(st);
+    const uint32_t slo = (uint32_t)sb, shi = (uint32_t)(sb >> 32);
+    const wc_surfel_id mine{(int32_t)idv.x, (int32_t)idv.y, (int32_t)idv.z, idv.w};
+    const bool live = (uint32_t)lane < c;
+    uint32_t rank = 0;
+    for (uint32_t j = 0; j < c; ++j) {
+      const unsigned long long ob = ((unsigned long long)(uint32_t)__builtin_amdgcn_readlane((int)shi, (int)j) << 32) |
+                                    (uint32_t)__builtin_amdgcn_readlane((int)slo, (int)j);
+      const double to = __longlong_as_double((long long)ob);
+      const wc_surfel_id other{__builtin_amdgcn_readlane((int)idv.x, (int)j), __builtin_amdgcn_readlane((int)idv.y, (int)j),
+                               __builtin_amdgcn_readlane((int)idv.z, (int)j), (uint32_t)__builtin_amdgcn_readlane((int)idv.w, (int)j)};
+      rank += (to < st || (to == st && surfel_id_less(other, mine))) ? 1u : 0u;
+    }
+    if (c <= 12u) {
+      const uint32_t r0 = (uint32_t)__shfl((int)rank, sub), r1 = (uint32_t)__shfl((int)rank, sub + 6);
+      const bool l0 = __shfl((int)live, sub) != 0, l1 = __shfl((int)live, sub + 6) != 0;
+      if (sub >= 6) return;
+      store(r0, l0, d0);
+      store(r1, l1, d1);
+      return;
+    }
+    s_rank[w][lane] = live ? rank : 0xFFFFFFFFu;
+  } else {
+    s_t[w][lane] = st;
+    for (uint32_t i = lane + 64; i < c; i += 64) s_t[w][i] = *(const double *)(bin + (size_t)i * kFxBinRec);
+    __builtin_amdgcn_wave_barrier();
+    auto id_at = [&](uint32_t i) -> wc_surfel_id {
+      const uint4 q = *(const uint4 *)(bin + (size_t)i * kFxBinRec + 144);
+      return wc_surfel_id{(int32_t)q.x, (int32_t)q.y, (int32_t)q.z, q.w};
+    };
+    for (uint32_t i = lane; i < c; i += 64) {
+      const double tm = s_t[w][i];
+      uint32_t rank = 0;
+      for (uint32_t j = 0; j < c; ++j) {
+        const double to = s_t[w][j];
+        if (to < tm)
+          ++rank;
+        else if (to == tm && j != i && surfel_id_less(id_at(j), id_at(i)))
+          ++rank;
+      }
+      s_rank[w][i] = rank;
+    }
+  }
+  __builtin_amdgcn_wave_barrier();
+  if (sub >= 6) return;
+  for (uint32_t r = sub; r < c; r += 24) {
+    uint32_t rk[4];
+    double2 d[4];
+#pragma unroll
+    for (int q = 0; q < 4; ++q) {
+      const uint32_t p = r + 6u * q;
+      rk[q] = p < c ? s_rank[w][p] : 0xFFFFFFFFu;
+      d[q] = make_double2(0.0, 0.0);
+      if (rk[q] != 0xFFFFFFFFu && (piece < 9 || out_ids)) d[q] = ((const double2 *)(bin + (size_t)p * kFxBinRec))[piece];
+    }
+#pragma unroll
+    for (int q = 0; q < 4; ++q) store(rk[q], rk[q] != 0xFFFFFFFFu, d[q]);
+  }
+}
+
+__global__ void __launch_bounds__(256) k_slot_emit(BinEmitArgs E) { bin_emit_body(E, blockIdx.x, gridDim.x); }
+__global__ void __launch_bounds__(256) k_slot_emit_b(const BinEmitArgs *__restrict__ Es, int K) {
+  const uint32_t per = kBuckets / 4;
+  const uint32_t k = blockIdx.x / per;
+  if ((int)k >= K) return;
+  bin_emit_body(Es[k], blockIdx.x - k * per, per);
+}
diff --git a/wildcat-slam_amd/csrc/extract_plan.h b/wildcat-slam_amd/csrc/extract_plan.h
--- a/wildcat-slam_amd/csrc/extract_plan.h
+++ b/wildcat-slam_amd/csrc/extract_plan.h
@@ -131,6 +131,10 @@
   while (bin_cap < (uint32_t)kSlotBinMax && (uint64_t)bin_cap * kBuckets < 2 * total_slots) bin_cap *= 2;
   return bin_cap;
 }
+inline uint32_t ex_fx_bin_cap(uint64_t total_slots, int floor) {
+  return std::max(ex_slot_bin_cap(total_slots), (uint32_t)std::min(std::max(floor, 0), kSlotBinMax));
+}
+inline uint64_t ex_fx_bins_bytes(uint32_t bin_cap) { return (uint64_t)kBuckets * bin_cap * (sizeof(wc_surfel) + sizeof(wc_surfel_id)); }
 inline unsigned ex_fx_tiles(uint64_t n) { return (unsigned)((n + kFxTile - 1) / kFxTile); }
 inline unsigned ex_fx_node_grid(uint64_t n) { return std::min<unsigned>(256 * 16, std::max<unsigned>(64, (unsigned)(n / 256))); }
 inline unsigned ex_fx_batch_node_grid(uint64_t n) { return std::max(64u, ex_fx_node_grid(n) / 8u); }
diff --git a/wildcat-slam_amd/csrc/extract_split.inc b/wildcat-slam_amd/csrc/extract_split.inc
--- a/wildcat-slam_amd/csrc/extract_split.inc
+++ b/wildcat-slam_amd/csrc/extract_split.inc
@@ -141,10 +141,8 @@
     FxPart rt;
     bool parent_live;
     uint32_t split;
-    const FxEmit pend = fx_test_children<LEVEL>(A, have_parent, tot, ncl, key, o1p, kx, ky, kz, cc, q0, wsub, kFxWhySplit.slots, s_flag, s_gkey, s_go1p,
-                                                rt, parent_live, split);
-    if (LEVEL == 1) fx_test_root(A, parent_live, rt, cc, kx, ky, kz, q0, wsub, kFxWhySplit.slots, s_flag, [&](bool) { return root_ncl; });
-    fx_emit_end(A, pend);
+    fx_test_children<LEVEL>(A, have_parent, tot, ncl, key, o1p, kx, ky, kz, cc, q0, s_flag, s_gkey, s_go1p, rt, parent_live, split);
+    if (LEVEL == 1) fx_test_root(A, parent_live, rt, cc, kx, ky, kz, q0, s_flag, [&](bool) { return root_ncl; });
     __builtin_amdgcn_wave_barrier();
     const unsigned long long *jp = A.jobpool + ((size_t)(vw & 7u) * A.jobpool_per + jbase) * kFxJobW;
     for (uint32_t r0 = 0; r0 < jcnt; r0 += 64u) {
@@ -164,7 +162,7 @@
       for (int i = 0; i < 3; ++i) cl.s[i] = (long long)w[2 + i];
 #pragma unroll
       for (int i = 0; i < 6; ++i) cl.ss[i] = (long long)w[5 + i];
-      fx_run_job<LEVEL>(A, want, owner, cl, ordv, k0x, k0y, k0z, q0, wsub, kFxWhySplit, s_gkey, s_go1p);
+      fx_run_job<LEVEL>(A, want, owner, cl, ordv, k0x, k0y, k0z, q0, kFxWhySplit, s_gkey, s_go1p);
     }
     __builtin_amdgcn_wave_barrier();
     const bool queued = LEVEL == 1 && fx_queue_layer2(A, have_parent, split, pidx, key, blk, wsub);
diff --git a/wildcat-slam_amd/host/odom_c_api.cc b/wildcat-slam_amd/host/odom_c_api.cc
--- a/wildcat-slam_amd/host/odom_c_api.cc
+++ b/wildcat-slam_amd/host/odom_c_api.cc
@@ -319,6 +319,10 @@
   out5[2] = ex_fx_tiles(n);
   out5[3] = ex_fx_node_grid(n);
   out5[4] = ex_fx_layer2_grid((unsigned)out5[3], last_splits);
+}
+void wc_host_ex_fx_bins(uint64_t n, int max_layer, int cluster_min, int bin_floor, uint64_t out2[2]) {
+  out2[0] = ex_fx_bin_cap(ex_total_slots(n, max_layer, cluster_min, (uint64_t)kFxSub * 256), bin_floor);
+  out2[1] = ex_fx_bins_bytes((uint32_t)out2[0]);
 }
 
 int wc_host_lm_loop(int op, void *state, uint64_t state_bytes, const double *in, double *out22) {
```

After: 20490 Mpts/s. -5.1%, worse.
